# qianyizh/ElasticReconstruction

Measured on AMD Instinct MI355X. Metric: depth frames/sec into 512^3 TSDF (640x480), higher is better.
Workload: dtype f32; 1 GPU; configs[1]; frames_per_gpu=91800, volume_units_touched=122, warp=True, inputs=hbm_resident, parallelism=single GPU

## Files before the change

### elasticreconstruction_amd/_ffi.py

```python
import ctypes as C
import os

_HERE = os.path.dirname(os.path.abspath(__file__))
LIB_PATH = os.environ.get("ER_HIP_LIB") or os.path.join(_HERE, "liber_hip.so")

SYMBOLS = [
    "er_last_error", "er_device_count", "er_abi_version", "er_request_hw_queues", "er_host_alloc", "er_host_free", "er_host_copy_h2d", "er_device_alloc", "er_device_free", "er_device_copy_d2h",
    "er_tsdf_create", "er_tsdf_destroy", "er_tsdf_set_stream", "er_tsdf_synchronize",
    "er_tsdf_wait_event", "er_tsdf_reset", "er_tsdf_status", "er_tsdf_set_unit_shard", "er_unit_owner",
    "er_tsdf_scale_depth", "er_tsdf_reproject", "er_tsdf_integrate", "er_tsdf_integrate_frames", "er_tsdf_prepass_trace",
    "er_tsdf_unit_count", "er_tsdf_unit_keys", "er_tsdf_read_unit", "er_tsdf_sum_weight",
    "er_tsdf_extract_world", "er_tsdf_extract_surface", "er_tsdf_extract_oriented", "er_tsdf_extract_mesh", "er_mc_table", "er_tsdf_extract_mesh_indexed", "er_tsdf_import_world", "er_raycast_params_default", "er_tsdf_raycast", "er_tsdf_raycast_batch", "er_tsdf_export_weighted", "er_tsdf_import_weighted",
    "er_tsdf_export_raw", "er_tsdf_import_raw",
    "er_tsdf_color_enable", "er_tsdf_read_unit_color", "er_tsdf_write_unit_color", "er_tsdf_color_frames", "er_tsdf_reproject_color", "er_tsdf_sample_colors",
    "er_tsdf_band_sizes", "er_tsdf_export_band", "er_tsdf_merge_band", "er_tsdf_import_band", "er_tsdf_drop_units",
    "er_tsdf_set_profiling", "er_tsdf_get_profile",
    "er_comm_unique_id", "er_comm_create", "er_comm_create_local", "er_comm_create_loopback", "er_comm_destroy", "er_comm_rank", "er_comm_world",
    "er_tsdf_allreduce", "er_comm_merge_stats", "er_comm_merge_stats_owner", "er_frame_block",
    "er_cloud_create", "er_cloud_create_batch", "er_cloud_create_from_tsdf", "er_cloud_destroy", "er_cloud_size",
    "er_icp_count_inliers", "er_icp_align", "er_icp_align_trace", "er_find_correspondence",
    "er_icp_count_inliers_batch", "er_icp_align_batch", "er_find_correspondence_batch", "er_icp_release_workspaces", "er_registration_batch", "er_ransac_fitness_batch", "er_ransac_inliers",
    "er_features_create", "er_features_destroy", "er_features_size", "er_feature_knn", "er_ransac_hypotheses", "er_ransac_params_default", "er_ransac_align", "er_ransac_align_batch",
    "er_odom_params_default", "er_odom_create", "er_odom_destroy", "er_odom_align_pairs", "er_odom_track", "er_frame_to_model_align", "er_frames_to_models_align", "er_odom_linearize", "er_odom_read_maps", "er_odom_tables",
    "er_cloud_read", "er_cloud_voxel_grid", "er_cloud_estimate_normals", "er_fpfh_estimate", "er_features_dim", "er_features_read",
    "er_frag_params_default", "er_frag_create", "er_frag_destroy", "er_frag_lane_bytes", "er_frag_build", "er_frag_count", "er_frag_read",
    "er_pgo_create", "er_pgo_destroy", "er_pgo_optimize", "er_pgo_set_state", "er_pgo_get_state", "er_pgo_linearize", "er_pgo_trial", "er_pgo_set_profiling", "er_pgo_get_profile",
    "er_fopt_create", "er_fopt_destroy", "er_fopt_set_cloud", "er_fopt_cloud_size", "er_fopt_get_points", "er_fopt_update_pose",
    "er_fopt_update_point_pn", "er_fopt_set_correspondences", "er_fopt_set_correspondences_dev", "er_fopt_group_count", "er_fopt_group_info", "er_fopt_update_normals", "er_fopt_assemble_rigid", "er_fopt_assemble_slac",
    "er_fopt_assemble_nonrigid", "er_fopt_factor_slac", "er_fopt_factor_nonrigid", "er_fopt_solve", "er_fopt_debug_shift_diagonal",
]


class ErWarp(C.Structure):
    _fields_ = [
        ("ctr", C.POINTER(C.c_float)),
        ("num_grids", C.c_int),
        ("resolution", C.c_int),
        ("length", C.c_float),
        ("grid_index", C.POINTER(C.c_int)),
        ("seg", C.POINTER(C.c_double)),
        ("madj", C.POINTER(C.c_double)),
    ]


class ErRansacParams(C.Structure):
    _fields_ = [("max_iterations", C.c_int), ("nr_samples", C.c_int), ("k_correspondences", C.c_int), ("similarity", C.c_float),
                ("max_corr_dist", C.c_float), ("inlier_fraction", C.c_float), ("inlier_number", C.c_int), ("angle_diff", C.c_float),
                ("seed", C.c_uint), ("chunk_iterations", C.c_int)]


class ErRansacStats(C.Structure):
    _fields_ = [("iterations", C.c_longlong), ("polygon_rejections", C.c_longlong), ("normal_rejections", C.c_longlong), ("scored", C.c_longlong)]


class ErOdomParams(C.Structure):
    _fields_ = [("levels", C.c_int), ("iterations", C.c_int * 4), ("bilateral", C.c_int), ("max_depth_mm", C.c_int), ("min_valid", C.c_int),
                ("dist_thresh", C.c_float), ("angle_thresh", C.c_float)]


class ErRaycastParams(C.Structure):
    _fields_ = [("t_min", C.c_float), ("t_max", C.c_float), ("step", C.c_float)]


class ErFragParams(C.Structure):
    _fields_ = [("interval", C.c_int), ("lanes", C.c_int), ("max_units", C.c_int), ("length", C.c_float), ("raycast", ErRaycastParams)]


class ErError(RuntimeError):
    pass


_lib = None


def lib():
    global _lib
    if _lib is not None:
        return _lib
    if not os.path.exists(LIB_PATH):
        raise ErError(
            "liber_hip.so not found at %s -- build it with `python -c 'import __graft_entry__ as g; g.build()'` "
            "or `make -C elasticreconstruction_amd/csrc`; there is no CPU fallback." % LIB_PATH)
    L = C.CDLL(LIB_PATH, mode=C.RTLD_GLOBAL)
    vp, ip, dp, fp = C.c_void_p, C.POINTER(C.c_int), C.POINTER(C.c_double), C.POINTER(C.c_float)
    u16p = C.POINTER(C.c_uint16)
    L.er_last_error.restype = C.c_char_p
    L.er_last_error.argtypes = []
    L.er_device_count.argtypes = []
    L.er_abi_version.argtypes = []
    L.er_host_alloc.restype = vp
    L.er_host_alloc.argtypes = [C.c_size_t]
    L.er_host_free.argtypes = [vp]
    L.er_host_copy_h2d.argtypes = [vp, vp, C.c_size_t]
    L.er_device_alloc.restype = vp
    L.er_device_alloc.argtypes = [C.c_size_t, C.c_int]
    L.er_device_free.argtypes = [vp]
    L.er_device_copy_d2h.argtypes = [vp, vp, C.c_size_t]
    L.er_tsdf_create.argtypes = [C.c_int, C.c_int, fp, C.c_int, C.c_int, C.POINTER(vp)]
    L.er_tsdf_destroy.argtypes = [vp]
    L.er_tsdf_set_stream.argtypes = [vp, vp]
    L.er_tsdf_synchronize.argtypes = [vp]
    L.er_tsdf_wait_event.argtypes = [vp, vp]
    L.er_tsdf_reset.argtypes = [vp]
    L.er_tsdf_status.argtypes = [vp, ip, C.POINTER(C.c_long)]
    L.er_tsdf_set_unit_shard.argtypes = [vp, C.c_int, C.c_int]
    L.er_unit_owner.argtypes = [C.c_int, C.c_int]
    L.er_tsdf_scale_depth.argtypes = [vp, vp, vp]
    L.er_tsdf_reproject.argtypes = [vp, vp, vp, C.c_int, C.c_float, vp, vp]
    L.er_tsdf_integrate.argtypes = [vp, vp, vp]
    L.er_tsdf_integrate_frames.argtypes = [vp, C.c_int, vp, C.c_int, vp, C.POINTER(ErWarp)]
    if hasattr(L, "er_tsdf_prepass_trace"):
        L.er_tsdf_prepass_trace.argtypes = [vp, C.c_int, vp, C.c_int, vp, C.POINTER(ErWarp), vp, ip, vp, vp, vp, vp, vp, C.c_int, ip]
    L.er_tsdf_unit_count.argtypes = [vp, ip]
    L.er_tsdf_unit_keys.argtypes = [vp, vp]
    L.er_tsdf_read_unit.argtypes = [vp, C.c_int, vp, vp]
    L.er_tsdf_sum_weight.argtypes = [vp, dp]
    L.er_tsdf_extract_world.argtypes = [vp, vp, C.c_long, C.POINTER(C.c_long)]
    L.er_tsdf_extract_surface.argtypes = [vp, vp, C.c_long, C.POINTER(C.c_long)]
    if hasattr(L, "er_tsdf_extract_oriented"):
        L.er_tsdf_extract_oriented.argtypes = [vp, vp, vp, C.c_long, C.POINTER(C.c_long)]
    L.er_tsdf_extract_mesh.argtypes = [vp, vp, C.c_long, C.POINTER(C.c_long)]
    L.er_mc_table.argtypes = [vp]
    if hasattr(L, "er_tsdf_extract_mesh_indexed"):
        L.er_tsdf_extract_mesh_indexed.argtypes = [vp, vp, vp, C.c_long, vp, C.c_long, C.POINTER(C.c_long), C.POINTER(C.c_long)]
        L.er_tsdf_import_world.argtypes = [vp, vp, C.c_long, ip]
    if hasattr(L, "er_tsdf_raycast"):
        L.er_raycast_params_default.argtypes = [C.POINTER(ErRaycastParams)]
        L.er_tsdf_raycast.argtypes = [vp, C.c_int, C.c_int, vp, vp, C.POINTER(ErRaycastParams), vp, vp, C.c_int]
    if hasattr(L, "er_tsdf_raycast_batch"):
        L.er_tsdf_raycast_batch.argtypes = [C.c_int, vp, vp, vp, vp, vp, vp, vp, vp]
    if hasattr(L, "er_frag_create"):
        L.er_frag_params_default.argtypes = [C.POINTER(ErFragParams)]
        L.er_frag_create.argtypes = [C.c_int, C.c_int, vp, C.POINTER(ErOdomParams), C.POINTER(ErFragParams), C.c_int, C.POINTER(vp)]
        L.er_frag_destroy.argtypes = [vp]
        L.er_frag_lane_bytes.argtypes = [vp, C.POINTER(C.c_size_t)]
        L.er_frag_build.argtypes = [vp, C.c_int, vp, C.c_int, vp, C.c_int, vp, vp]
        L.er_frag_count.argtypes = [vp, ip]
        L.er_frag_read.argtypes = [vp, C.c_int, vp, vp, C.c_long, C.POINTER(C.c_long)]
    if hasattr(L, "er_tsdf_color_enable"):
        L.er_tsdf_color_enable.argtypes = [vp]
        L.er_tsdf_read_unit_color.argtypes = [vp, C.c_int, vp]
        L.er_tsdf_write_unit_color.argtypes = [vp, C.c_int, vp]
        L.er_tsdf_color_frames.argtypes = [vp, C.c_int, vp, vp, C.c_int, vp, C.POINTER(ErWarp), vp]
        L.er_tsdf_sample_colors.argtypes = [vp, vp, C.c_long, vp, vp]
        L.er_tsdf_reproject_color.argtypes = [vp, vp, vp, vp, C.c_int, C.c_float, vp, vp]
    L.er_request_hw_queues.argtypes = [C.c_int]
    L.er_tsdf_export_weighted.argtypes = [vp, vp, C.c_int, vp]
    L.er_tsdf_import_weighted.argtypes = [vp, vp, C.c_int, vp]
    L.er_tsdf_export_raw.argtypes = [vp, vp, C.c_int, vp]
    L.er_tsdf_import_raw.argtypes = [vp, vp, C.c_int, vp]
    L.er_comm_unique_id.argtypes = [vp]
    L.er_comm_create.argtypes = [vp, C.c_int, C.c_int, C.c_int, C.POINTER(vp)]
    L.er_comm_create_local.argtypes = [C.c_int, vp, vp]
    L.er_comm_create_loopback.argtypes = [C.c_int, C.c_int, vp]
    L.er_comm_destroy.argtypes = [vp]
    L.er_comm_rank.argtypes = [vp]
    L.er_comm_world.argtypes = [vp]
    L.er_tsdf_allreduce.argtypes = [vp, vp, C.c_int, ip]
    L.er_comm_merge_stats.argtypes = [vp, vp]
    L.er_comm_merge_stats_owner.argtypes = [vp, vp]
    L.er_tsdf_band_sizes.argtypes = [vp, vp, C.c_int, vp]
    L.er_tsdf_export_band.argtypes = [vp, vp, vp, C.c_int, vp]
    L.er_tsdf_merge_band.argtypes = [vp, vp, C.c_int, vp, vp, vp]
    L.er_tsdf_import_band.argtypes = [vp, vp, C.c_int, vp]
    L.er_tsdf_drop_units.argtypes = [vp, vp, C.c_int]
    L.er_frame_block.restype = None
    L.er_frame_block.argtypes = [C.c_int, C.c_int, C.c_int, ip, ip]
    L.er_tsdf_set_profiling.argtypes = [vp, C.c_int]
    L.er_tsdf_get_profile.argtypes = [vp, dp, C.POINTER(C.c_long), C.POINTER(C.c_long), C.POINTER(C.c_long)]
    if hasattr(L, "er_cloud_create"):
        L.er_cloud_create.argtypes = [vp, vp, C.c_int, C.c_float, C.c_int, C.POINTER(vp)]
        L.er_cloud_create_batch.argtypes = [C.c_int, vp, vp, vp, C.c_float, C.c_int, vp]
        if hasattr(L, "er_cloud_create_from_tsdf"):
            L.er_cloud_create_from_tsdf.argtypes = [vp, C.c_float, C.c_float, C.POINTER(vp), ip]
        L.er_cloud_destroy.argtypes = [vp]
        L.er_cloud_size.argtypes = [vp]
        L.er_icp_count_inliers.argtypes = [vp, vp, vp, C.c_double, ip]
        L.er_icp_align.argtypes = [vp, vp, vp, C.c_double, C.c_int, C.c_double, C.c_int, vp, ip, ip, dp]
        if hasattr(L, "er_icp_align_trace"):
            L.er_icp_align_trace.argtypes = [vp, vp, vp, C.c_double, C.c_int, C.c_double, C.c_int, C.c_int, C.c_int, vp, vp, vp, vp, vp, vp, ip, vp, ip, ip]
        L.er_find_correspondence.argtypes = [vp, vp, vp, C.c_double, C.c_double, vp, C.c_int, ip, vp]
        L.er_icp_count_inliers_batch.argtypes = [C.c_int, vp, vp, vp, C.c_double, vp]
        L.er_icp_align_batch.argtypes = [C.c_int, vp, vp, vp, C.c_double, C.c_int, C.c_double, C.c_int, vp, vp, vp, vp]
        L.er_find_correspondence_batch.argtypes = [C.c_int, vp, vp, vp, C.c_double, C.c_double, vp, vp, vp, vp]
        L.er_icp_release_workspaces.argtypes = []
        L.er_registration_batch.argtypes = [C.c_int, vp, vp, vp, C.c_double, C.c_int, C.c_double, C.c_int, C.c_double, C.c_int, C.c_double, C.c_double,
                                            vp, vp, vp, vp, vp, vp, vp, vp, vp]
        L.er_ransac_fitness_batch.argtypes = [vp, vp, C.c_int, vp, C.c_float, vp, vp]
        L.er_ransac_inliers.argtypes = [vp, vp, vp, C.c_float, vp, C.c_int, ip, vp, vp, vp]
        if hasattr(L, "er_ransac_align"):
            L.er_features_create.argtypes = [vp, C.c_int, C.c_int, C.c_int, C.POINTER(vp)]
            L.er_features_destroy.argtypes = [vp]
            L.er_features_size.argtypes = [vp]
            L.er_feature_knn.argtypes = [vp, vp, C.c_int, vp, vp]
            L.er_ransac_hypotheses.argtypes = [vp, vp, C.c_int, C.c_int, vp, vp, C.c_float, C.c_float, vp, vp]
            L.er_ransac_params_default.argtypes = [C.POINTER(ErRansacParams)]
            L.er_ransac_align.argtypes = [vp, vp, vp, vp, C.POINTER(ErRansacParams), vp, ip, ip, dp, C.POINTER(ErRansacStats), vp, C.c_int, ip]
        if hasattr(L, "er_ransac_align_batch"):
            L.er_ransac_align_batch.argtypes = [C.c_int, vp, vp, vp, vp, C.POINTER(ErRansacParams), vp, C.c_int, vp, vp, vp, vp, vp, vp, vp]
        if hasattr(L, "er_fpfh_estimate"):
            L.er_cloud_read.argtypes = [vp, vp, vp]
            L.er_cloud_voxel_grid.argtypes = [vp, C.c_float, C.c_float, C.POINTER(vp), ip]
            L.er_cloud_estimate_normals.argtypes = [vp, C.c_float, C.POINTER(vp), vp]
            L.er_fpfh_estimate.argtypes = [vp, C.c_float, C.POINTER(vp), vp, vp]
            L.er_features_dim.argtypes = [vp]
            L.er_features_read.argtypes = [vp, vp]
    if hasattr(L, "er_odom_create"):
        L.er_odom_params_default.argtypes = [C.POINTER(ErOdomParams)]
        L.er_odom_create.argtypes = [C.c_int, C.c_int, fp, C.POINTER(ErOdomParams), C.c_int, C.POINTER(vp)]
        L.er_odom_destroy.argtypes = [vp]
        L.er_odom_align_pairs.argtypes = [vp, C.c_int, vp, C.c_int, C.c_int, vp, vp, vp, vp, vp, vp, vp, C.c_int]
        L.er_odom_track.argtypes = [vp, C.c_int, vp, C.c_int, vp, vp, C.c_int]
        if hasattr(L, "er_frame_to_model_align"):
            L.er_frame_to_model_align.argtypes = [vp, vp, C.c_int, vp, C.c_int, vp, vp, vp, vp, vp, C.c_int]
        if hasattr(L, "er_frames_to_models_align"):
            L.er_frames_to_models_align.argtypes = [vp, C.c_int, vp, C.c_int, vp, C.c_int, vp, vp, vp, vp, vp, vp, C.c_int]
        L.er_odom_linearize.argtypes = [vp, vp, C.c_int, C.c_int, vp, vp, ip]
        L.er_odom_read_maps.argtypes = [vp, vp, C.c_int, C.c_int, vp, vp, vp]
        L.er_odom_tables.argtypes = [vp, vp, ip]
    if hasattr(L, "er_pgo_create"):
        L.er_pgo_create.argtypes = [C.c_int, C.c_int, vp, vp, vp, vp, vp, C.c_int, C.POINTER(vp)]
        L.er_pgo_destroy.argtypes = [vp]
        L.er_pgo_optimize.argtypes = [vp, C.c_int, C.c_double, C.c_int, vp, vp, ip, ip, vp]
        L.er_pgo_set_state.argtypes = [vp, vp, vp]
        L.er_pgo_get_state.argtypes = [vp, vp, vp]
        L.er_pgo_linearize.argtypes = [vp, C.c_double, C.c_double, vp, vp, vp]
        L.er_pgo_trial.argtypes = [vp, C.c_double, C.c_double, vp, vp, dp, ip]
        L.er_pgo_set_profiling.argtypes = [vp, C.c_int]
        L.er_pgo_get_profile.argtypes = [vp, vp]
    if hasattr(L, "er_fopt_create"):
        L.er_fopt_create.argtypes = [C.c_int, C.c_int, C.c_float, C.c_int, C.POINTER(vp)]
        L.er_fopt_destroy.argtypes = [vp]
        L.er_fopt_set_cloud.argtypes = [vp, C.c_int, vp, vp, C.c_int, ip]
        L.er_fopt_cloud_size.argtypes = [vp, C.c_int]
        L.er_fopt_get_points.argtypes = [vp, C.c_int, vp, vp, vp, vp, vp]
        L.er_fopt_update_pose.argtypes = [vp, C.c_int, vp]
        L.er_fopt_update_point_pn.argtypes = [vp, C.c_int, vp]
        L.er_fopt_set_correspondences.argtypes = [vp, C.c_int, vp, vp, vp, vp]
        L.er_fopt_set_correspondences_dev.argtypes = [vp, C.c_int, vp, vp, vp, vp]
        L.er_fopt_group_count.argtypes = [vp]
        L.er_fopt_assemble_rigid.argtypes = [vp, vp, vp, vp]
        L.er_fopt_assemble_slac.argtypes = [vp, vp, vp, vp, vp]
        L.er_fopt_group_info.argtypes = [vp, vp]
        L.er_fopt_update_normals.argtypes = [vp, C.c_int, vp]
        L.er_fopt_assemble_nonrigid.argtypes = [vp, C.c_double, vp, vp]
        L.er_fopt_factor_slac.argtypes = [vp, vp, C.c_double, vp, vp]
        L.er_fopt_factor_nonrigid.argtypes = [vp, C.c_double]
        L.er_fopt_solve.argtypes = [vp, vp, C.c_int, vp]
        L.er_fopt_debug_shift_diagonal.argtypes = [vp, C.c_long, C.c_double]
    _lib = L
    return L


def check(rc, what):
    if rc != 0:
        msg = lib().er_last_error()
        raise ErError("%s failed: %s" % (what, msg.decode("utf-8", "replace") if msg else "unknown error"))


class PinnedArena:

    def __init__(self):
        self._lib, self._p, self._cap, self._off, self._old = lib(), None, 0, 0, []

    def reset(self, need_bytes):
        self._off = 0
        for p in self._old:
            self._lib.er_host_free(p)
        self._old = []
        if need_bytes > self._cap:
            if self._p:
                self._lib.er_host_free(self._p)
            self._cap = int(need_bytes * 1.25) + 4096
            self._p = self._lib.er_host_alloc(self._cap)
            if not self._p:
                self._cap = 0
                raise ErError("er_host_alloc: " + self._lib.er_last_error().decode())

    def take(self, shape, dtype):
        import numpy as np
        dt = np.dtype(dtype)
        n = int(np.prod(shape)) * dt.itemsize
        off = (self._off + 4095) & ~4095
        assert off + n <= self._cap, "PinnedArena.reset() was sized too small"
        self._off = off + n
        buf = (C.c_char * max(n, 1)).from_address(self._p + off)
        return np.frombuffer(buf, dtype=dt, count=int(np.prod(shape))).reshape(shape)

    def close(self):
        if self._p:
            self._lib.er_host_free(self._p)
            self._p, self._cap = None, 0

    def __del__(self):
        try:
            self.close()
        except Exception:
            pass


def ptr(a):
    return a.ctypes.data_as(C.c_void_p)
```

### elasticreconstruction_amd/csrc/er_tsdf.h

```cpp
#pragma once

#include "er_common.h"
#include "er_tsdf_math.h"

#include "../../include/er_hip.h"

#include <algorithm>
#include <cstdlib>
#include <utility>
#include <vector>

namespace er_tsdf_k {
using namespace er;

constexpr int kBlock = 256;
constexpr int kEmptyKey = -1;
constexpr uint32_t kZEmpty = 0xFFFFFFFFu;

enum { C_NUNITS = 0, C_NBATCH = 1 , C_POOL_OVERFLOW = 2, C_TABLE_FULL = 3, C_OUT_OF_RANGE = 4,
       C_NBATCH1 = 6, C_NBATCH2 = 7, C_ZERO_WRITE = 8 ,
       C_ZERO_WRITE1 = 10, C_COUNT = 12 };
constexpr int kDepth = 3;
constexpr int kAux = 2;

struct ReprojArgs {
  const uint16_t* depth;
  int n_frames, cols, rows;
  Camera cam;
  CameraInv cami;
  const double* seg12;
  const double* madj12;
  const int* grid_index;
  const float* ctr;
  int res;
  float grid_ul;
  int floats_per_grid;
  uint32_t* zbuf;
  uint32_t* lastzero;
  uint32_t* zfix;
  int* zero_flag;
};
__global__ void k_reproject_scatter(ReprojArgs A);

constexpr int kFixThreads = 64;
constexpr int kFixBlocks = 256;

constexpr int kScaledPad = 64;
constexpr int kTile = 32;
constexpr int kLoShift = 4;
constexpr int kLoSub = kTile >> kLoShift;
constexpr int kTileKeys = 96;

constexpr int kPrepThreads = 256;
constexpr int kPrepPix = kTile * kTile / kPrepThreads;

template <bool kWide>
__global__ __launch_bounds__(kPrepThreads) void k_prepare(
    const uint16_t* __restrict__ depth, uint32_t* __restrict__ zbuf, int n_frames, int cols, int rows,
    Camera cam, CameraInv cami, const float* __restrict__ lambda, const double* __restrict__ T12, float* __restrict__ scaled,
    int* __restrict__ ht_key, int* __restrict__ ht_slot, unsigned long long* __restrict__ ht_mask, int cap_mask,
    int hash_shift, int* __restrict__ batch, int* __restrict__ nbatch,
    int* __restrict__ counters, float* __restrict__ tile_max, float* __restrict__ tile_lo, float* __restrict__ tile_lo_fine, int2 shard,
    uint32_t* __restrict__ lastzero, uint32_t* __restrict__ zfix, const int* __restrict__ zero_flag);
extern template __global__ void k_prepare<true>(const uint16_t* __restrict__, uint32_t* __restrict__, int, int, int, Camera, CameraInv, const float* __restrict__, const double* __restrict__, float* __restrict__, int* __restrict__, int* __restrict__, unsigned long long* __restrict__, int, int, int* __restrict__, int* __restrict__, int* __restrict__, float* __restrict__, float* __restrict__, float* __restrict__, int2, uint32_t* __restrict__, uint32_t* __restrict__, const int* __restrict__);
extern template __global__ void k_prepare<false>(const uint16_t* __restrict__, uint32_t* __restrict__, int, int, int, Camera, CameraInv, const float* __restrict__, const double* __restrict__, float* __restrict__, int* __restrict__, int* __restrict__, unsigned long long* __restrict__, int, int, int* __restrict__, int* __restrict__, int* __restrict__, float* __restrict__, float* __restrict__, float* __restrict__, int2, uint32_t* __restrict__, uint32_t* __restrict__, const int* __restrict__);

constexpr int kRows = 4;
constexpr int kItemsPerUnit = 256;

struct Plan {
  int n_units;
  int next;
};

struct PlanRec {
  int key;
  int slot;
  unsigned long long mask;
};

constexpr int kIntMinBlocks = 5;

template <bool kSure>
__global__ __launch_bounds__(kBlock, kIntMinBlocks) void k_integrate(
    float2* __restrict__ pool, const PlanRec* __restrict__ plan_rec, Plan* __restrict__ plan,
    const FrameXform* __restrict__ frames, const float* __restrict__ scaled, const float* __restrict__ tile_max,
    const float* __restrict__ tile_lo, const float* __restrict__ tile_lo_fine, int tiles_x, int tiles_y, Camera cam, int cols, int rows);
extern template __global__ void k_integrate<true>(float2* __restrict__, const PlanRec* __restrict__, Plan* __restrict__, const FrameXform* __restrict__, const float* __restrict__, const float* __restrict__, const float* __restrict__, const float* __restrict__, int, int, Camera, int, int);
extern template __global__ void k_integrate<false>(float2* __restrict__, const PlanRec* __restrict__, Plan* __restrict__, const FrameXform* __restrict__, const float* __restrict__, const float* __restrict__, const float* __restrict__, const float* __restrict__, int, int, Camera, int, int);
}

struct er_tsdf_s {
  int device = 0, cols = 0, rows = 0, pixels = 0, max_units = 0;
  er::Camera cam{};
  er::CameraInv cami{};
  hipStream_t own_stream = nullptr, stream = nullptr;
  hipEvent_t caller_ev = nullptr;
  hipEvent_t voxel_done = nullptr;
  bool voxel_ahead = false;
  hipStream_t aux_stream[er_tsdf_k::kAux] = {};
  hipStream_t copy_stream = nullptr;
  hipEvent_t copy_done[er_tsdf_k::kDepth] = {};
  hipEvent_t consts_done[er_tsdf_k::kDepth] = {};
  int n_cu = 256;
  int shard_rank = 0, shard_world = 1;
  float2* pool = nullptr;
  int *ht_key = nullptr, *ht_slot = nullptr, *unit_key = nullptr, *counters = nullptr;
  unsigned long long* stats = nullptr;
  long batch_no = 0;
  bool used[er_tsdf_k::kDepth] = {};
  int* batch[er_tsdf_k::kDepth] = {};
  unsigned long long* ht_mask[er_tsdf_k::kDepth] = {};
  float *scaled[er_tsdf_k::kDepth] = {}, *tile_max[er_tsdf_k::kDepth] = {}, *tile_lo[er_tsdf_k::kDepth] = {}, *tile_lo_fine[er_tsdf_k::kDepth] = {};
  er::FrameXform* frames[er_tsdf_k::kDepth] = {};
  void* dstage[er_tsdf_k::kDepth] = {};
  hipEvent_t pre_done[er_tsdf_k::kDepth] = {}, int_done[er_tsdf_k::kDepth] = {};
  void* pinned[er_tsdf_k::kDepth] = {};
  int ht_cap = 0, ht_shift = 0;
  float *lambda = nullptr, *ctr = nullptr;
  float* ctr_pinned[2] = {nullptr, nullptr};
  float* ctr_dev[2] = {nullptr, nullptr};
  size_t ctr_pinned_cap[2] = {0, 0}, ctr_dev_cap[2] = {0, 0};
  hipEvent_t ctr_ev[2] = {nullptr, nullptr};
  hipEvent_t ctr_rd[2][er_tsdf_k::kAux] = {};
  bool ctr_rd_set[2] = {false, false};
  int ctr_parity = 0, ctr_cur = 0;
  uint16_t* depth_stage[er_tsdf_k::kDepth] = {};
  uint32_t *zbuf[er_tsdf_k::kAux] = {}, *lastzero[er_tsdf_k::kAux] = {}, *zfix[er_tsdf_k::kAux] = {};
  double *T12 = nullptr, *seg12 = nullptr, *madj12 = nullptr, *dsum = nullptr;
  int *grid_index = nullptr, *key_scratch = nullptr, *slot_scratch = nullptr;
  er_tsdf_k::PlanRec* plan_rec[er_tsdf_k::kDepth] = {};
  er_tsdf_k::Plan* plan[er_tsdf_k::kDepth] = {};
  bool reset_pending[er_tsdf_k::kDepth] = {};
  size_t key_scratch_cap = 0;
  int prof_stride = 0;
  long prof_tick = 0;
  std::vector<std::pair<hipEvent_t, hipEvent_t>> events;
  double ms_total = 0.0;
  long launches = 0, frames_done = 0;
  std::vector<int> dropped;
  void* band_scratch = nullptr;
  size_t band_scratch_cap = 0;
  unsigned long long* color = nullptr;
  void* color_scratch = nullptr;
  size_t color_scratch_cap = 0;
};

namespace er_tsdf_k {
__attribute__((visibility("hidden"))) int check_flags(er_tsdf_t h);
__attribute__((visibility("hidden"))) int resolve_slots(er_tsdf_t h, const int* keys_host, int n, bool allocate);
__attribute__((visibility("hidden"))) int sorted_units(er_tsdf_t h, std::vector<int>& keys, std::vector<int>& slots);
__attribute__((visibility("hidden"))) int reproject_single(er_tsdf_t h, const ReprojArgs& RA, uint16_t* z_dev, hipStream_t X);
__attribute__((visibility("hidden"))) int color_zero_slots(er_tsdf_t h, int n);
}
```

### elasticreconstruction_amd/csrc/er_tsdf.hip

```cpp
#include "er_tsdf_dev.h"

namespace {

using namespace er_tsdf_k;

constexpr int kNbatchSlot[3] = {C_NBATCH, C_NBATCH1, C_NBATCH2};
constexpr int kZeroFlagSlot[2] = {C_ZERO_WRITE, C_ZERO_WRITE1};

__global__ void k_lambda(float* __restrict__ lambda, int cols, int rows, Camera cam) {
  int p = blockIdx.x * blockDim.x + threadIdx.x;
  if (p >= cols * rows) return;
  lambda[p] = scale_lambda(p % cols, p / cols, cam);
}

__global__ void k_scale_depth(const uint16_t* __restrict__ depth, const float* __restrict__ lambda,
                              float* __restrict__ scaled, int pixels, float itrunc) {
  int p = blockIdx.x * blockDim.x + threadIdx.x;
  if (p >= pixels) return;
  scaled[p] = scale_depth_px(depth[p], lambda[p], itrunc);
}

__global__ __launch_bounds__(kFixThreads) __attribute__((amdgpu_num_vgpr(48))) void k_reproject_fix(ReprojArgs A) {
  const int fl0 = A.zero_flag[0], fl1 = A.zero_flag[1];
  if ((fl0 | fl1) == 0) return;
  const int pixels = A.cols * A.rows;
  for (int f = 0; f < A.n_frames; f++) {
    if ((((f < 32 ? fl0 : fl1) >> (f & 31)) & 1) == 0) continue;
    for (int p = blockIdx.x * kFixThreads + threadIdx.x; p < pixels; p += gridDim.x * kFixThreads) reproject_scatter_px(A, f, p % A.cols, p / A.cols, 1);
  }
}

__global__ void k_zbuf_to_depth(uint32_t* __restrict__ zbuf, uint16_t* __restrict__ depth, long total, uint32_t* __restrict__ lastzero,
                                uint32_t* __restrict__ zfix, const int* __restrict__ zero_flag) {
  long t = (long)blockIdx.x * blockDim.x + threadIdx.x;
  if (t >= total) return;
  uint32_t z = zbuf[t];
  zbuf[t] = kZEmpty;
  if (zero_flag[0] & 1) z = take_z(z, (size_t)t, lastzero, zfix);
  depth[t] = (z == kZEmpty) ? (uint16_t)0 : (uint16_t)z;
}


__device__ int unit_slot_acquire(int e, int key, int* __restrict__ ht_slot, int* __restrict__ unit_key, int max_units, int* __restrict__ counters) {
  int slot = __hip_atomic_load(&ht_slot[e], __ATOMIC_RELAXED, __HIP_MEMORY_SCOPE_AGENT);
  bool won = false;
  if (slot == -1) won = atomicCAS(&ht_slot[e], -1, -2) == -1;
  if (won) {
    const int s = atomicAdd(&counters[C_NUNITS], 1);
    if (s < max_units) {
      unit_key[s] = key;
      __threadfence();
      slot = s;
    } else {
      atomicOr(&counters[C_POOL_OVERFLOW], 1);
      slot = -3;
    }
    atomicExch(&ht_slot[e], slot);
  }
  if (!won && (slot == -1 || slot == -2)) {
    do {
      slot = __hip_atomic_load(&ht_slot[e], __ATOMIC_RELAXED, __HIP_MEMORY_SCOPE_AGENT);
      if (slot == -2) __builtin_amdgcn_s_sleep(8);
    } while (slot == -2);
  }
  return slot;
}

__global__ __launch_bounds__(256) void k_plan(const int* __restrict__ batch, const int* __restrict__ nbatch,
                                              const unsigned long long* __restrict__ ht_mask, const int* __restrict__ ht_key,
                                              int* __restrict__ ht_slot, int* __restrict__ unit_key, int max_units,
                                              int* __restrict__ counters, PlanRec* __restrict__ plan_rec, Plan* __restrict__ plan,
                                              int* __restrict__ zero_flag) {
  __shared__ int hist[65];
  __shared__ int start[66];
  const int n = *nbatch;
  for (int t = threadIdx.x; t < 65; t += blockDim.x) hist[t] = 0;
  __syncthreads();
  for (int t = threadIdx.x; t < n; t += blockDim.x) atomicAdd(&hist[__popcll(ht_mask[batch[t]])], 1);
  __syncthreads();
  if (threadIdx.x == 0) {
    int acc = 0;
    for (int c = 64; c >= 0; c--) {
      start[c] = acc;
      acc += hist[c];
    }
    plan->n_units = n;
    plan->next = 0;
    if (zero_flag) zero_flag[0] = zero_flag[1] = 0;
  }
  __syncthreads();
  for (int t = threadIdx.x; t < n; t += blockDim.x) {
    const int e = batch[t];
    const unsigned long long mask = ht_mask[e];
    const int key = ht_key[e];
    PlanRec r;
    r.key = key;
    r.slot = unit_slot_acquire(e, key, ht_slot, unit_key, max_units, counters);
    r.mask = mask;
    plan_rec[atomicAdd(&start[__popcll(mask)], 1)] = r;
  }
}

__global__ void k_reset(const int* __restrict__ batch, int* __restrict__ nbatch, unsigned long long* __restrict__ ht_mask,
                        unsigned long long* __restrict__ stats) {
  const int n = *nbatch;
  unsigned long long visits = 0;
  for (int t = threadIdx.x; t < n; t += blockDim.x) {
    const int e = batch[t];
    visits += (unsigned long long)__popcll(ht_mask[e]);
    ht_mask[e] = 0ull;
  }
  if (visits) atomicAdd(&stats[0], visits);
  __syncthreads();
  if (threadIdx.x == 0) *nbatch = 0;
}

__global__ void k_sum_weight(const float2* __restrict__ pool, long n_vox, double* __restrict__ out) {
  double s = 0.0;
  for (long t = (long)blockIdx.x * blockDim.x + threadIdx.x; t < n_vox; t += (long)gridDim.x * blockDim.x)
    s += (double)pool[t].y;
  for (int off = 32; off > 0; off >>= 1) s += __shfl_down(s, off);
  __shared__ double part[kBlock / 64];
  if ((threadIdx.x & 63) == 0) part[threadIdx.x >> 6] = s;
  __syncthreads();
  if (threadIdx.x == 0) {
    double b = 0.0;
    for (int w = 0; w < kBlock / 64; w++) b += part[w];
    atomicAdd(out, b);
  }
}

__global__ void k_ensure_units(const int* __restrict__ keys, int n, int* __restrict__ ht_key, int* __restrict__ ht_slot,
                               int cap_mask, int hash_shift, int* __restrict__ unit_key, int max_units,
                               int* __restrict__ counters, int* __restrict__ slots_out, int allocate) {
  const int t = blockIdx.x * blockDim.x + threadIdx.x;
  if (t >= n) return;
  const int key = keys[t];
  int slot = -1;
  if (allocate) {
    const int e = ht_find_or_insert(ht_key, cap_mask, hash_shift, key);
    if (e < 0) {
      atomicOr(&counters[C_TABLE_FULL], 1);
    } else {
      slot = ht_slot[e];
      if (slot < 0) {
        const int s = atomicAdd(&counters[C_NUNITS], 1);
        if (s < max_units) {
          ht_slot[e] = s;
          unit_key[s] = key;
          slot = s;
        } else {
          atomicOr(&counters[C_POOL_OVERFLOW], 1);
        }
      }
    }
  } else {
    unsigned h = hash_unit_key(key, hash_shift);
    for (int probe = 0; probe <= cap_mask; ++probe) {
      const int e = (int)((h + (unsigned)probe) & (unsigned)cap_mask);
      const int k = ht_key[e];
      if (k == key) { slot = ht_slot[e]; break; }
      if (k == kEmptyKey) break;
    }
  }
  slots_out[t] = slot;
}

}

hipStream_t er::tsdf_stream(er_tsdf_s* h) { return h->stream; }
int er::tsdf_device(er_tsdf_s* h) { return h->device; }

static int launch_reproject(er_tsdf_t h, const ReprojArgs& RA, int n, hipStream_t X);

namespace {

int drain_events(er_tsdf_t h) {
  for (auto& ev : h->events) {
    float ms = 0.f;
    ER_HIP_TRY(hipEventSynchronize(ev.second));
    ER_HIP_TRY(hipEventElapsedTime(&ms, ev.first, ev.second));
    h->ms_total += ms;
    h->launches += 1;
    (void)hipEventDestroy(ev.first);
    (void)hipEventDestroy(ev.second);
  }
  h->events.clear();
  return 0;
}

int join_voxel(er_tsdf_t h) {
  if (h->voxel_ahead) {
    ER_HIP_TRY(hipStreamWaitEvent(h->stream, h->voxel_done, 0));
    h->voxel_ahead = false;
  }
  return 0;
}

int ensure_key_scratch(er_tsdf_t h, size_t n) {
  if (n <= h->key_scratch_cap) return 0;
  if (h->key_scratch) (void)hipFree(h->key_scratch);
  if (h->slot_scratch) (void)hipFree(h->slot_scratch);
  h->key_scratch = h->slot_scratch = nullptr;
  size_t cap = std::max<size_t>(n, 1024);
  ER_HIP_TRY(hipMalloc(&h->key_scratch, cap * sizeof(int)));
  ER_HIP_TRY(hipMalloc(&h->slot_scratch, cap * sizeof(int)));
  h->key_scratch_cap = cap;
  return 0;
}

}

namespace er_tsdf_k {

int check_flags(er_tsdf_t h) {
  int c[C_COUNT];
  if (join_voxel(h)) return 1;
  ER_HIP_TRY(hipMemcpyAsync(c, h->counters, sizeof c, hipMemcpyDeviceToHost, h->stream));
  ER_HIP_TRY(hipStreamSynchronize(h->stream));
  if (c[C_POOL_OVERFLOW])
    return er::fail("TSDF unit pool exhausted: %d units requested, capacity %d (raise max_units)", c[C_NUNITS], h->max_units);
  if (c[C_TABLE_FULL]) return er::fail("TSDF unit hash table full (capacity %d)", h->ht_cap);
  return 0;
}

int resolve_slots(er_tsdf_t h, const int* keys_host, int n, bool allocate) {
  if (join_voxel(h) || ensure_key_scratch(h, (size_t)n)) return 1;
  ER_HIP_TRY(hipMemcpyAsync(h->key_scratch, keys_host, (size_t)n * sizeof(int), hipMemcpyHostToDevice, h->stream));
  hipLaunchKernelGGL(k_ensure_units, dim3((n + kBlock - 1) / kBlock), dim3(kBlock), 0, h->stream, h->key_scratch, n,
                     h->ht_key, h->ht_slot, h->ht_cap - 1, h->ht_shift, h->unit_key, h->max_units, h->counters,
                     h->slot_scratch, allocate ? 1 : 0);
  ER_HIP_TRY(hipGetLastError());
  return 0;
}

int sorted_units(er_tsdf_t h, std::vector<int>& keys, std::vector<int>& slots) {
  if (check_flags(h)) return 1;
  int n = 0;
  ER_HIP_TRY(hipMemcpy(&n, h->counters + C_NUNITS, sizeof(int), hipMemcpyDeviceToHost));
  n = std::min(n, h->max_units);
  std::vector<int> uk((size_t)n);
  if (n) ER_HIP_TRY(hipMemcpy(uk.data(), h->unit_key, (size_t)n * sizeof(int), hipMemcpyDeviceToHost));
  std::vector<std::pair<int, int>> ks;
  ks.reserve((size_t)n);
  for (int s = 0; s < n; s++)
    if (!std::binary_search(h->dropped.begin(), h->dropped.end(), uk[(size_t)s])) ks.push_back(std::make_pair(uk[(size_t)s], s));
  std::sort(ks.begin(), ks.end());
  n = (int)ks.size();
  keys.resize((size_t)n);
  slots.resize((size_t)n);
  for (int s = 0; s < n; s++) {
    keys[(size_t)s] = ks[(size_t)s].first;
    slots[(size_t)s] = ks[(size_t)s].second;
  }
  return 0;
}

}

namespace {

struct Staging {
  er::FrameXform fx[ER_MAX_BATCH];
  float fxT[16][ER_MAX_BATCH];
  double t12[ER_MAX_BATCH * 12];
  double seg[ER_MAX_BATCH * 16];
  double madj[ER_MAX_BATCH * 12];
  int gi[ER_MAX_BATCH];
};

int flush_resets(er_tsdf_t h) {
  if (join_voxel(h)) return 1;
  for (int q = 0; q < kDepth; q++)
    if (h->reset_pending[q]) {
      hipLaunchKernelGGL(k_reset, dim3(1), dim3(kBlock), 0, h->stream, h->batch[q], h->counters + kNbatchSlot[q], h->ht_mask[q], h->stats);
      ER_HIP_TRY(hipGetLastError());
      ER_HIP_TRY(hipEventRecord(h->int_done[q], h->stream));
      h->reset_pending[q] = false;
    }
  return 0;
}

int sync_all(er_tsdf_t h) {
  if (flush_resets(h)) return 1;
  if (h->copy_stream) ER_HIP_TRY(hipStreamSynchronize(h->copy_stream));
  for (int a = 0; a < kAux; a++) ER_HIP_TRY(hipStreamSynchronize(h->aux_stream[a]));
  if (h->stream != h->own_stream) ER_HIP_TRY(hipStreamSynchronize(h->own_stream));
  ER_HIP_TRY(hipStreamSynchronize(h->stream));
  h->voxel_ahead = false;
  return 0;
}

int run_batch(er_tsdf_t h, int n, const uint16_t* depth_dev, const double* T, const er_warp* warp, int frame0) {
  const int p = (int)(h->batch_no % kDepth), a = (int)(h->batch_no % kAux);
  h->batch_no++;
  if (h->used[p]) ER_HIP_TRY(hipEventSynchronize(h->consts_done[p]));
  Staging* st = static_cast<Staging*>(h->pinned[p]);
  for (int f = 0; f < n; f++) {
    const double* Tf = T + (size_t)f * 16;
    double Tinv[16];
    if (!er::mat4_inverse(Tf, Tinv)) return er::fail("frame %d: singular pose matrix", frame0 + f);
    for (int q = 0; q < 12; q++) {
      st->fx[f].mi[q] = (float)Tinv[q];
      st->t12[f * 12 + q] = Tf[q];
    }
    st->fx[f].tx = (float)Tf[3];
    st->fx[f].ty = (float)Tf[7];
    st->fx[f].tz = (float)Tf[11];
    st->fx[f].pad = 0.f;
    for (int q = 0; q < 16; q++) st->fxT[q][f] = reinterpret_cast<const float*>(&st->fx[f])[q];
  }
  static_assert(offsetof(Staging, fxT) == sizeof(er::FrameXform) * ER_MAX_BATCH && sizeof(er::FrameXform) == 64, "fxT lies directly behind fx");
  hipStream_t X = h->aux_stream[a], S = h->own_stream;
  int* nbatch = h->counters + kNbatchSlot[p];

  constexpr int kIntBlocksPerCu = 3;
  const int wide_grid = h->n_cu * kIntBlocksPerCu;
  uint32_t* zsrc = nullptr;
  char* dst = static_cast<char*>(h->dstage[p]);
  const double* dev_t12 = reinterpret_cast<const double*>(dst + offsetof(Staging, t12));
  const double* dev_seg = reinterpret_cast<const double*>(dst + offsetof(Staging, seg));
  const double* dev_madj = reinterpret_cast<const double*>(dst + offsetof(Staging, madj));
  const int* dev_gi = reinterpret_cast<const int*>(dst + offsetof(Staging, gi));
  if (warp) {
    for (int f = 0; f < n; f++) {
      for (int q = 0; q < 12; q++) {
        st->seg[f * 16 + q] = warp->seg[(size_t)(frame0 + f) * 16 + q];
        st->madj[f * 12 + q] = warp->madj[(size_t)(frame0 + f) * 16 + q];
      }
      er::cube_coord_deltas(&st->seg[f * 16], h->cam, h->cols, h->rows, &st->seg[f * 16 + 12]);
      st->seg[f * 16 + 15] = 0.0;
      const int g = warp->grid_index[frame0 + f];
      if (g < 0 || g >= warp->num_grids) return er::fail("frame %d: control grid index %d out of [0,%d)", frame0 + f, g, warp->num_grids);
      st->gi[f] = g;
    }
  }
  if (h->used[p]) ER_HIP_TRY(hipStreamWaitEvent(X, h->int_done[p], 0));
  if (h->reset_pending[p]) {
    hipLaunchKernelGGL(k_reset, dim3(1), dim3(kBlock), 0, X, h->batch[p], nbatch, h->ht_mask[p], h->stats);
    ER_HIP_TRY(hipGetLastError());
    h->reset_pending[p] = false;
  }
  ER_HIP_TRY(hipMemcpyAsync(h->dstage[p], st, sizeof(Staging), hipMemcpyHostToDevice, X));
  ER_HIP_TRY(hipEventRecord(h->consts_done[p], X));
  if (warp) {
    const int verts = (warp->resolution + 1) * (warp->resolution + 1) * (warp->resolution + 1);
    const float grid_ul = warp->length / (float)warp->resolution;
    const ReprojArgs RA{depth_dev, n, h->cols, h->rows, h->cam, h->cami, dev_seg, dev_madj, dev_gi, h->ctr, warp->resolution, grid_ul,
                        verts * 3, h->zbuf[a], h->lastzero[a], h->zfix[a], h->counters + kZeroFlagSlot[a]};
    if (launch_reproject(h, RA, n, X)) return 1;
    zsrc = h->zbuf[a];
  }

  const bool wide = h->cols % 4 == 0 && (zsrc || reinterpret_cast<uintptr_t>(depth_dev) % 8 == 0);
  hipLaunchKernelGGL(wide ? k_prepare<true> : k_prepare<false>, dim3((h->cols + kTile - 1) / kTile, (h->rows + kTile - 1) / kTile, n), dim3(kPrepThreads), 0, X,
                     depth_dev, zsrc, n, h->cols, h->rows, h->cam, h->cami, h->lambda, dev_t12, h->scaled[p], h->ht_key, h->ht_slot,
                     h->ht_mask[p], h->ht_cap - 1, h->ht_shift, h->batch[p], nbatch, h->counters,
                     h->tile_max[p], h->tile_lo[p], h->tile_lo_fine[p], make_int2(h->shard_rank, h->shard_world), h->lastzero[a], h->zfix[a],
                     h->counters + kZeroFlagSlot[a]);
  hipLaunchKernelGGL(k_plan, dim3(1), dim3(256), 0, X, h->batch[p], nbatch, h->ht_mask[p], h->ht_key, h->ht_slot, h->unit_key, h->max_units,
                     h->counters, h->plan_rec[p], h->plan[p], warp ? h->counters + kZeroFlagSlot[a] : (int*)nullptr);
  ER_HIP_TRY(hipGetLastError());
  ER_HIP_TRY(hipEventRecord(h->pre_done[p], X));

  ER_HIP_TRY(hipStreamWaitEvent(S, h->pre_done[p], 0));
  hipEvent_t e0 = nullptr, e1 = nullptr;
  const bool timed = h->prof_stride > 0 && (h->prof_tick++ % h->prof_stride) == 0;
  if (timed) {
    ER_HIP_TRY(hipEventCreate(&e0));
    ER_HIP_TRY(hipEventCreate(&e1));
    ER_HIP_TRY(hipEventRecord(e0, S));
  }
  const bool sure = h->cam.integration_trunc < 64.0f;
  hipLaunchKernelGGL(sure ? k_integrate<true> : k_integrate<false>, dim3(wide_grid), dim3(kBlock), 0, S, h->pool, h->plan_rec[p], h->plan[p],
                     h->frames[p], h->scaled[p], h->tile_max[p], h->tile_lo[p], h->tile_lo_fine[p], (h->cols + kTile - 1) / kTile, (h->rows + kTile - 1) / kTile,
                     h->cam, h->cols, h->rows);
  if (timed) {
    ER_HIP_TRY(hipEventRecord(e1, S));
    h->events.emplace_back(e0, e1);
  }
  ER_HIP_TRY(hipGetLastError());
  ER_HIP_TRY(hipEventRecord(h->int_done[p], S));
  h->reset_pending[p] = true;
  h->used[p] = true;
  h->frames_done += n;
  return 0;
}

}

static hipError_t aux_create(hipStream_t* s) {
  return hipStreamCreateWithFlags(s, hipStreamNonBlocking);
}

extern "C" {

int er_tsdf_create(int cols, int rows, const float cam6[6], int max_units, int device, er_tsdf_t* out) {
  if (!out) return er::fail("er_tsdf_create: out is NULL");
  *out = nullptr;
  if (cols <= 0 || rows <= 0 || max_units <= 0) return er::fail("er_tsdf_create: bad dimensions");
  if ((long)cols * rows >= (1L << 30)) return er::fail("er_tsdf_create: image of %d x %d pixels is too large", cols, rows);
  int ndev = 0;
  if (hipGetDeviceCount(&ndev) != hipSuccess || ndev <= 0)
    return er::fail("er_tsdf_create: no HIP device available (liber_hip has no CPU fallback)");
  if (device < 0 || device >= ndev) return er::fail("er_tsdf_create: device %d out of range [0,%d)", device, ndev);
  ER_HIP_TRY(hipSetDevice(device));
  er_tsdf_t h = new er_tsdf_s();
  h->device = device;
  h->cols = cols;
  h->rows = rows;
  h->pixels = cols * rows;
  h->max_units = max_units;
  if (cam6) {
    h->cam = er::Camera{cam6[0], cam6[1], cam6[2], cam6[3], cam6[4], cam6[5]};
  } else {
    h->cam = er::Camera{525.0f, 525.0f, 319.5f, 239.5f, 2.5f, 2.5f};
  }
  h->cami.inv_fx = 1.0 / (double)h->cam.fx;
  h->cami.inv_fy = 1.0 / (double)h->cam.fy;
  h->cami.pp_small = (std::fabs((double)h->cam.cx) < 1e6 && std::fabs((double)h->cam.cy) < 1e6) ? 1 : 0;
  h->cami.pad = 0;
  hipDeviceProp_t prop;
  if (hipGetDeviceProperties(&prop, device) == hipSuccess && prop.multiProcessorCount > 0) h->n_cu = prop.multiProcessorCount;
  int cap = 1024, lg = 10;
  while (cap < 4 * max_units) { cap <<= 1; lg++; }
  h->ht_cap = cap;
  h->ht_shift = 32 - lg;
  const size_t px = (size_t)h->pixels, B = ER_MAX_BATCH;
#define ER_ALLOC(ptr, bytes)                                                                         \
  do {                                                                                               \
    hipError_t e_ = hipMalloc((void**)&(ptr), (bytes));                                              \
    if (e_ != hipSuccess) {                                                                          \
      er::fail("er_tsdf_create: hipMalloc(%zu bytes) for " #ptr " failed: %s", (size_t)(bytes), hipGetErrorString(e_)); \
      er_tsdf_destroy(h);                                                                            \
      return 1;                                                                                      \
    }                                                                                                \
  } while (0)
  if (hipStreamCreateWithFlags(&h->own_stream, hipStreamNonBlocking) != hipSuccess ||
      aux_create(&h->aux_stream[0]) != hipSuccess || (kAux > 1 && aux_create(&h->aux_stream[kAux - 1]) != hipSuccess) ||
      false) {
    delete h;
    return er::fail("er_tsdf_create: hipStreamCreate failed");
  }
  h->stream = h->own_stream;
  if (hipEventCreateWithFlags(&h->caller_ev, hipEventDisableTiming) != hipSuccess ||
      hipEventCreateWithFlags(&h->voxel_done, hipEventDisableTiming) != hipSuccess) {
    er_tsdf_destroy(h);
    return er::fail("er_tsdf_create: event allocation failed");
  }
  for (int q = 0; q < kDepth; q++) {
    if (hipEventCreateWithFlags(&h->pre_done[q], hipEventDisableTiming) != hipSuccess ||
        hipEventCreateWithFlags(&h->int_done[q], hipEventDisableTiming) != hipSuccess ||
        hipEventCreateWithFlags(&h->copy_done[q], hipEventDisableTiming) != hipSuccess ||
        hipEventCreateWithFlags(&h->consts_done[q], hipEventDisableTiming) != hipSuccess ||
        hipHostMalloc(&h->pinned[q], sizeof(Staging), hipHostMallocDefault) != hipSuccess) {
      er_tsdf_destroy(h);
      return er::fail("er_tsdf_create: event / pinned staging allocation failed");
    }
  }
  ER_ALLOC(h->pool, (size_t)max_units * er::kUnitVox * sizeof(float2));
  ER_ALLOC(h->ht_key, (size_t)cap * sizeof(int));
  ER_ALLOC(h->ht_slot, (size_t)cap * sizeof(int));
  for (int q = 0; q < kDepth; q++) ER_ALLOC(h->ht_mask[q], (size_t)cap * sizeof(unsigned long long));
  ER_ALLOC(h->unit_key, (size_t)max_units * sizeof(int));
  ER_ALLOC(h->counters, C_COUNT * sizeof(int));
  ER_ALLOC(h->stats, 4 * sizeof(unsigned long long));
  for (int q = 0; q < kDepth; q++) ER_ALLOC(h->batch[q], (size_t)cap * sizeof(int));
  ER_ALLOC(h->lambda, px * sizeof(float));
  for (int q = 0; q < kDepth; q++) ER_ALLOC(h->scaled[q], B * (px + kScaledPad) * sizeof(float));
  for (int q = 0; q < kDepth; q++) ER_ALLOC(h->depth_stage[q], B * px * sizeof(uint16_t));
  for (int q = 0; q < kAux; q++) ER_ALLOC(h->zbuf[q], B * px * sizeof(uint32_t));
  for (int q = 0; q < kAux; q++) ER_ALLOC(h->lastzero[q], B * px * sizeof(uint32_t));
  for (int q = 0; q < kAux; q++) ER_ALLOC(h->zfix[q], B * px * sizeof(uint32_t));
  for (int q = 0; q < kDepth; q++) ER_ALLOC(h->dstage[q], sizeof(Staging));
  for (int q = 0; q < kDepth; q++) h->frames[q] = reinterpret_cast<er::FrameXform*>(reinterpret_cast<char*>(h->dstage[q]) + offsetof(Staging, fx));
  ER_ALLOC(h->T12, B * 12 * sizeof(double));
  ER_ALLOC(h->seg12, B * 16 * sizeof(double));
  ER_ALLOC(h->madj12, B * 12 * sizeof(double));
  ER_ALLOC(h->grid_index, B * sizeof(int));
  ER_ALLOC(h->dsum, sizeof(double));
  for (int q = 0; q < kDepth; q++) ER_ALLOC(h->tile_max[q], B * (size_t)((cols + kTile - 1) / kTile) * ((rows + kTile - 1) / kTile) * sizeof(float));
  for (int q = 0; q < kDepth; q++) ER_ALLOC(h->tile_lo[q], B * (size_t)((cols + kTile - 1) / kTile) * ((rows + kTile - 1) / kTile) * sizeof(float));
  for (int q = 0; q < kDepth; q++)
    ER_ALLOC(h->tile_lo_fine[q], B * (size_t)((cols + (1 << kLoShift) - 1) >> kLoShift) * ((rows + (1 << kLoShift) - 1) >> kLoShift) * sizeof(float));
  for (int q = 0; q < kDepth; q++) ER_ALLOC(h->plan_rec[q], (size_t)cap * sizeof(PlanRec));
  for (int q = 0; q < kDepth; q++) ER_ALLOC(h->plan[q], sizeof(Plan));
#undef ER_ALLOC
  hipStream_t s = h->stream;
  bool ok = hipMemsetAsync(h->pool, 0, (size_t)max_units * er::kUnitVox * sizeof(float2), s) == hipSuccess &&
            hipMemsetAsync(h->ht_key, 0xFF, (size_t)cap * sizeof(int), s) == hipSuccess &&
            hipMemsetAsync(h->ht_slot, 0xFF, (size_t)cap * sizeof(int), s) == hipSuccess &&
            hipMemsetAsync(h->counters, 0, C_COUNT * sizeof(int), s) == hipSuccess &&
            hipMemsetAsync(h->stats, 0, 4 * sizeof(unsigned long long), s) == hipSuccess;
  for (int q = 0; q < kDepth; q++)
    ok = ok && hipMemsetAsync(h->ht_mask[q], 0, (size_t)cap * sizeof(unsigned long long), s) == hipSuccess &&
         hipMemsetAsync(h->scaled[q], 0, B * (px + kScaledPad) * sizeof(float), s) == hipSuccess;
  for (int q = 0; q < kAux; q++)
    ok = ok && hipMemsetAsync(h->lastzero[q], 0, B * px * sizeof(uint32_t), s) == hipSuccess &&
         hipMemsetAsync(h->zbuf[q], 0xFF, B * px * sizeof(uint32_t), s) == hipSuccess &&
         hipMemsetAsync(h->zfix[q], 0xFF, B * px * sizeof(uint32_t), s) == hipSuccess;
  if (ok) {
    hipLaunchKernelGGL(k_lambda, dim3((h->pixels + kBlock - 1) / kBlock), dim3(kBlock), 0, s, h->lambda, cols, rows, h->cam);
    ok = hipGetLastError() == hipSuccess && hipStreamSynchronize(s) == hipSuccess;
  }
  if (!ok) {
    er_tsdf_destroy(h);
    return er::fail("er_tsdf_create: device initialisation failed: %s", hipGetErrorString(hipGetLastError()));
  }
  *out = h;
  return 0;
}

int er_tsdf_destroy(er_tsdf_t h) {
  if (!h) return 0;
  (void)hipSetDevice(h->device);
  if (h->stream) (void)hipStreamSynchronize(h->stream);
  if (h->own_stream && h->own_stream != h->stream) (void)hipStreamSynchronize(h->own_stream);
  if (h->caller_ev) (void)hipEventDestroy(h->caller_ev);
  if (h->voxel_done) (void)hipEventDestroy(h->voxel_done);
  for (auto& ev : h->events) {
    (void)hipEventDestroy(ev.first);
    (void)hipEventDestroy(ev.second);
  }
  for (int a = 0; a < kAux; a++)
    if (h->aux_stream[a]) (void)hipStreamSynchronize(h->aux_stream[a]);
  std::vector<void*> ptrs = {h->pool, h->ht_key, h->ht_slot, h->unit_key, h->counters, h->stats, h->lambda, h->T12, h->seg12, h->madj12,
                             h->grid_index, h->dsum, h->ctr_dev[0], h->ctr_dev[1], h->key_scratch,
                             h->slot_scratch, h->band_scratch, h->color, h->color_scratch};
  for (int q = 0; q < kDepth; q++)
    for (void* x : {(void*)h->ht_mask[q], (void*)h->batch[q], (void*)h->scaled[q], (void*)h->depth_stage[q], h->dstage[q], (void*)h->tile_max[q], (void*)h->tile_lo[q], (void*)h->tile_lo_fine[q],
                    (void*)h->plan_rec[q], (void*)h->plan[q]})
      ptrs.push_back(x);
  for (int q = 0; q < kAux; q++) {
    ptrs.push_back(h->zbuf[q]);
    ptrs.push_back(h->lastzero[q]);
    ptrs.push_back(h->zfix[q]);
  }
  for (int q = 0; q < kDepth; q++) {
    if (h->pre_done[q]) (void)hipEventDestroy(h->pre_done[q]);
    if (h->int_done[q]) (void)hipEventDestroy(h->int_done[q]);
    if (h->copy_done[q]) (void)hipEventDestroy(h->copy_done[q]);
    if (h->consts_done[q]) (void)hipEventDestroy(h->consts_done[q]);
    if (h->pinned[q]) (void)hipHostFree(h->pinned[q]);
  }
  for (int a = 0; a < kAux; a++)
    if (h->aux_stream[a]) (void)hipStreamDestroy(h->aux_stream[a]);
  if (h->copy_stream) {
    (void)hipStreamSynchronize(h->copy_stream);
    (void)hipStreamDestroy(h->copy_stream);
  }
  for (int q = 0; q < 2; q++) {
    if (h->ctr_ev[q]) (void)hipEventDestroy(h->ctr_ev[q]);
    for (int a = 0; a < kAux; a++)
      if (h->ctr_rd[q][a]) (void)hipEventDestroy(h->ctr_rd[q][a]);
    if (h->ctr_pinned[q]) (void)hipHostFree(h->ctr_pinned[q]);
  }
  for (void* p : ptrs)
    if (p) (void)hipFree(p);
  if (h->own_stream) (void)hipStreamDestroy(h->own_stream);
  delete h;
  return 0;
}

int er_tsdf_set_stream(er_tsdf_t h, void* hip_stream) {
  if (!h) return er::fail("er_tsdf_set_stream: NULL handle");
  ER_HIP_TRY(hipSetDevice(h->device));
  if (sync_all(h)) return 1;
  h->stream = hip_stream ? (hipStream_t)hip_stream : h->own_stream;
  return 0;
}

int er_tsdf_synchronize(er_tsdf_t h) {
  if (!h) return er::fail("er_tsdf_synchronize: NULL handle");
  ER_HIP_TRY(hipSetDevice(h->device));
  return sync_all(h);
}

int er_tsdf_scale_depth(er_tsdf_t h, const uint16_t* depth_host, float* scaled_host) {
  if (!h || !depth_host || !scaled_host) return er::fail("er_tsdf_scale_depth: NULL argument");
  ER_HIP_TRY(hipSetDevice(h->device));
  if (sync_all(h)) return 1;
  const size_t px = (size_t)h->pixels;
  ER_HIP_TRY(hipMemcpyAsync(h->depth_stage[0], depth_host, px * sizeof(uint16_t), hipMemcpyHostToDevice, h->stream));
  hipLaunchKernelGGL(k_scale_depth, dim3((h->pixels + kBlock - 1) / kBlock), dim3(kBlock), 0, h->stream, h->depth_stage[0],
                     h->lambda, h->scaled[0], h->pixels, h->cam.integration_trunc);
  ER_HIP_TRY(hipGetLastError());
  ER_HIP_TRY(hipMemcpyAsync(scaled_host, h->scaled[0], px * sizeof(float), hipMemcpyDeviceToHost, h->stream));
  ER_HIP_TRY(hipStreamSynchronize(h->stream));
  return 0;
}

static int upload_ctr(er_tsdf_t h, const float* ctr, int res, int num_grids, hipStream_t also) {
  const size_t verts = (size_t)(res + 1) * (res + 1) * (res + 1);
  const size_t floats = verts * 3 * (size_t)num_grids;
  const int q = h->ctr_parity;
  h->ctr_parity ^= 1;
  if (floats > h->ctr_dev_cap[q]) {
    if (sync_all(h)) return 1;
    if (h->ctr_dev[q]) (void)hipFree(h->ctr_dev[q]);
    h->ctr_dev[q] = nullptr;
    h->ctr_dev_cap[q] = 0;
    ER_HIP_TRY(hipMalloc((void**)&h->ctr_dev[q], floats * sizeof(float)));
    h->ctr_dev_cap[q] = floats;
  }
  if (!h->ctr_ev[q]) {
    ER_HIP_TRY(hipEventCreateWithFlags(&h->ctr_ev[q], hipEventDisableTiming));
    for (int a = 0; a < kAux; a++) ER_HIP_TRY(hipEventCreateWithFlags(&h->ctr_rd[q][a], hipEventDisableTiming));
  } else {
    ER_HIP_TRY(hipEventSynchronize(h->ctr_ev[q]));
  }
  if (floats > h->ctr_pinned_cap[q]) {
    if (h->ctr_pinned[q]) (void)hipHostFree(h->ctr_pinned[q]);
    h->ctr_pinned[q] = nullptr;
    h->ctr_pinned_cap[q] = 0;
    ER_HIP_TRY(hipHostMalloc((void**)&h->ctr_pinned[q], floats * sizeof(float), hipHostMallocDefault));
    h->ctr_pinned_cap[q] = floats;
  }
  memcpy(h->ctr_pinned[q], ctr, floats * sizeof(float));
  const int a0 = (int)(h->batch_no % kAux);
  hipStream_t C = h->aux_stream[a0];
  if (h->ctr_rd_set[q])
    for (int a = 0; a < kAux; a++)
      if (a != a0) ER_HIP_TRY(hipStreamWaitEvent(C, h->ctr_rd[q][a], 0));
  ER_HIP_TRY(hipMemcpyAsync(h->ctr_dev[q], h->ctr_pinned[q], floats * sizeof(float), hipMemcpyHostToDevice, C));
  ER_HIP_TRY(hipEventRecord(h->ctr_ev[q], C));
  for (int a = 0; a < kAux; a++)
    if (a != a0) ER_HIP_TRY(hipStreamWaitEvent(h->aux_stream[a], h->ctr_ev[q], 0));
  if (also) ER_HIP_TRY(hipStreamWaitEvent(also, h->ctr_ev[q], 0));
  h->ctr = h->ctr_dev[q];
  h->ctr_cur = q;
  return 0;
}

static int launch_reproject(er_tsdf_t h, const ReprojArgs& RA, int n, hipStream_t X) {
  hipLaunchKernelGGL(k_reproject_scatter, dim3((h->cols + 63) / 64, (h->rows + 3) / 4, n), dim3(kBlock), 0, X, RA);
  hipLaunchKernelGGL(k_reproject_fix, dim3(kFixBlocks), dim3(kFixThreads), 0, X, RA);
  ER_HIP_TRY(hipGetLastError());
  return 0;
}

int er_tsdf_reproject(er_tsdf_t h, uint16_t* depth_inout_host, const float* ctr_host, int resolution, float length,
                      const double seg[16], const double madj[16]) {
  if (!h || !depth_inout_host || !ctr_host || !seg || !madj) return er::fail("er_tsdf_reproject: NULL argument");
  if (resolution <= 0) return er::fail("er_tsdf_reproject: bad resolution");
  ER_HIP_TRY(hipSetDevice(h->device));
  const size_t px = (size_t)h->pixels;
  const int verts = (resolution + 1) * (resolution + 1) * (resolution + 1);
  if (sync_all(h)) return 1;
  if (upload_ctr(h, ctr_host, resolution, 1, h->stream)) return 1;
  const int gi = 0;
  ER_HIP_TRY(hipMemcpyAsync(h->depth_stage[0], depth_inout_host, px * sizeof(uint16_t), hipMemcpyHostToDevice, h->stream));
  double seg16[16] = {0};
  memcpy(seg16, seg, 12 * sizeof(double));
  er::cube_coord_deltas(seg16, h->cam, h->cols, h->rows, seg16 + 12);
  ER_HIP_TRY(hipMemcpyAsync(h->seg12, seg16, 16 * sizeof(double), hipMemcpyHostToDevice, h->stream));
  ER_HIP_TRY(hipMemcpyAsync(h->madj12, madj, 12 * sizeof(double), hipMemcpyHostToDevice, h->stream));
  ER_HIP_TRY(hipMemcpyAsync(h->grid_index, &gi, sizeof(int), hipMemcpyHostToDevice, h->stream));
  const float grid_ul = length / (float)resolution;
  const long total = (long)px;
  const ReprojArgs RA{h->depth_stage[0], 1, h->cols, h->rows, h->cam, h->cami, h->seg12, h->madj12, h->grid_index, h->ctr, resolution, grid_ul,
                      verts * 3, h->zbuf[0], h->lastzero[0], h->zfix[0], h->counters + kZeroFlagSlot[0]};
  if (launch_reproject(h, RA, 1, h->stream)) return 1;
  hipLaunchKernelGGL(k_zbuf_to_depth, dim3((int)((total + kBlock - 1) / kBlock)), dim3(kBlock), 0, h->stream, h->zbuf[0],
                     h->depth_stage[0], total, h->lastzero[0], h->zfix[0], h->counters + kZeroFlagSlot[0]);
  ER_HIP_TRY(hipGetLastError());
  ER_HIP_TRY(hipMemsetAsync(h->counters + kZeroFlagSlot[0], 0, 2 * sizeof(int), h->stream));
  ER_HIP_TRY(hipMemcpyAsync(depth_inout_host, h->depth_stage[0], px * sizeof(uint16_t), hipMemcpyDeviceToHost, h->stream));
  ER_HIP_TRY(hipStreamSynchronize(h->stream));
  return 0;
}

int er_tsdf_integrate_frames(er_tsdf_t h, int n, const uint16_t* depth, int depth_on_device, const double* T,
                             const er_warp* warp) {
  if (!h || !depth || !T) return er::fail("er_tsdf_integrate_frames: NULL argument");
  if (n < 0) return er::fail("er_tsdf_integrate_frames: negative frame count");
  ER_HIP_TRY(hipSetDevice(h->device));
  if (n > 0) h->dropped.clear();
  if (warp) {
    if (!warp->ctr || !warp->grid_index || !warp->seg || !warp->madj || warp->num_grids <= 0 || warp->resolution <= 0)
      return er::fail("er_tsdf_integrate_frames: incomplete er_warp");
    if (upload_ctr(h, warp->ctr, warp->resolution, warp->num_grids, nullptr)) return 1;
  }
  const size_t px = (size_t)h->pixels;
  const int launches = (n + ER_MAX_BATCH - 1) / ER_MAX_BATCH;
  const int per = launches > 0 ? (n + launches - 1) / launches : 0;
  const bool joined = h->stream != h->own_stream && n > 0;
  if (joined) {
    ER_HIP_TRY(hipEventRecord(h->caller_ev, h->stream));
    ER_HIP_TRY(hipStreamWaitEvent(h->own_stream, h->caller_ev, 0));
  }
  for (int start = 0; start < n; start += per) {
    const int nb = std::min(per, n - start);
    const uint16_t* ddev;
    if (depth_on_device) {
      ddev = depth + (size_t)start * px;
    } else {
      const int p = (int)(h->batch_no % kDepth);
      if (!h->copy_stream) ER_HIP_TRY(hipStreamCreateWithFlags(&h->copy_stream, hipStreamNonBlocking));
      if (h->used[p]) ER_HIP_TRY(hipStreamWaitEvent(h->copy_stream, h->pre_done[p], 0));
      ER_HIP_TRY(hipMemcpyAsync(h->depth_stage[p], depth + (size_t)start * px, (size_t)nb * px * sizeof(uint16_t),
                                hipMemcpyHostToDevice, h->copy_stream));
      ER_HIP_TRY(hipEventRecord(h->copy_done[p], h->copy_stream));
      ER_HIP_TRY(hipStreamWaitEvent(h->aux_stream[h->batch_no % kAux], h->copy_done[p], 0));
      ddev = h->depth_stage[p];
    }
    if (run_batch(h, nb, ddev, T + (size_t)start * 16, warp, start)) return 1;
  }
  if (joined) {
    ER_HIP_TRY(hipEventRecord(h->voxel_done, h->own_stream));
    h->voxel_ahead = true;
  }
  if (warp) {
    for (int a = 0; a < kAux; a++) ER_HIP_TRY(hipEventRecord(h->ctr_rd[h->ctr_cur][a], h->aux_stream[a]));
    h->ctr_rd_set[h->ctr_cur] = true;
  }
  if (!depth_on_device && n > 0) ER_HIP_TRY(hipStreamSynchronize(h->copy_stream));
  return 0;
}

int er_tsdf_integrate(er_tsdf_t h, const uint16_t* depth_host, const double T[16]) {
  return er_tsdf_integrate_frames(h, 1, depth_host, 0, T, nullptr);
}

int er_tsdf_prepass_trace(er_tsdf_t h, int n, const uint16_t* depth, int depth_on_device, const double* T, const er_warp* warp,
                          float* scaled, int* scaled_pad, float* tile_max, float* tile_lo, float* tile_lo_fine,
                          int* keys, unsigned long long* masks, int keys_cap, int* n_keys) {
  if (!h) return er::fail("er_tsdf_prepass_trace: NULL handle");
  if (n < 1 || n > ER_MAX_BATCH) return er::fail("er_tsdf_prepass_trace: %d frames outside 1..%d (one batch)", n, ER_MAX_BATCH);
  ER_HIP_TRY(hipSetDevice(h->device));
  if (sync_all(h)) return 1;
  const int p = (int)(h->batch_no % kDepth);
  if (er_tsdf_integrate_frames(h, n, depth, depth_on_device, T, warp)) return 1;
  if (sync_all(h)) return 1;
  const size_t B = ER_MAX_BATCH, px = (size_t)h->pixels;
  const size_t tiles = (size_t)((h->cols + kTile - 1) / kTile) * ((h->rows + kTile - 1) / kTile);
  const size_t fine = (size_t)((h->cols + (1 << kLoShift) - 1) >> kLoShift) * ((h->rows + (1 << kLoShift) - 1) >> kLoShift);
  if (scaled_pad) *scaled_pad = kScaledPad;
  if (scaled) ER_HIP_TRY(hipMemcpy(scaled, h->scaled[p], (size_t)n * (px + kScaledPad) * sizeof(float), hipMemcpyDeviceToHost));
  if (tile_max) ER_HIP_TRY(hipMemcpy(tile_max, h->tile_max[p], tiles * B * sizeof(float), hipMemcpyDeviceToHost));
  if (tile_lo) ER_HIP_TRY(hipMemcpy(tile_lo, h->tile_lo[p], tiles * B * sizeof(float), hipMemcpyDeviceToHost));
  if (tile_lo_fine) ER_HIP_TRY(hipMemcpy(tile_lo_fine, h->tile_lo_fine[p], fine * B * sizeof(float), hipMemcpyDeviceToHost));
  Plan plan{};
  ER_HIP_TRY(hipMemcpy(&plan, h->plan[p], sizeof plan, hipMemcpyDeviceToHost));
  if (plan.n_units < 0 || plan.n_units > h->ht_cap) return er::fail("er_tsdf_prepass_trace: the batch lists %d units", plan.n_units);
  if (n_keys) *n_keys = plan.n_units;
  if (keys || masks) {
    std::vector<PlanRec> rec((size_t)plan.n_units);
    if (plan.n_units > 0) ER_HIP_TRY(hipMemcpy(rec.data(), h->plan_rec[p], rec.size() * sizeof(PlanRec), hipMemcpyDeviceToHost));
    std::sort(rec.begin(), rec.end(), [](const PlanRec& a, const PlanRec& b) { return a.key < b.key; });
    for (int i = 0; i < plan.n_units && i < keys_cap; i++) {
      if (keys) keys[i] = rec[(size_t)i].key;
      if (masks) masks[i] = rec[(size_t)i].mask;
    }
  }
  return 0;
}

int er_tsdf_wait_event(er_tsdf_t h, void* hip_event) {
  if (!h || !hip_event) return er::fail("er_tsdf_wait_event: NULL argument");
  ER_HIP_TRY(hipSetDevice(h->device));
  for (int a = 0; a < kAux; a++) ER_HIP_TRY(hipStreamWaitEvent(h->aux_stream[a], (hipEvent_t)hip_event, 0));
  if (h->copy_stream) ER_HIP_TRY(hipStreamWaitEvent(h->copy_stream, (hipEvent_t)hip_event, 0));
  return 0;
}

int er_tsdf_reset(er_tsdf_t h) {
  if (!h) return er::fail("er_tsdf_reset: NULL handle");
  ER_HIP_TRY(hipSetDevice(h->device));
  if (sync_all(h)) return 1;
  int n = 0;
  ER_HIP_TRY(hipMemcpy(&n, h->counters + C_NUNITS, sizeof(int), hipMemcpyDeviceToHost));
  n = std::min(std::max(n, 0), h->max_units);
  hipStream_t s = h->stream;
  if (n > 0) ER_HIP_TRY(hipMemsetAsync(h->pool, 0, (size_t)n * er::kUnitVox * sizeof(float2), s));
  if (n > 0 && h->color) ER_HIP_TRY(hipMemsetAsync(h->color, 0, (size_t)n * er::kUnitVox * 16, s));
  ER_HIP_TRY(hipMemsetAsync(h->ht_key, 0xFF, (size_t)h->ht_cap * sizeof(int), s));
  ER_HIP_TRY(hipMemsetAsync(h->ht_slot, 0xFF, (size_t)h->ht_cap * sizeof(int), s));
  for (int q = 0; q < kDepth; q++) ER_HIP_TRY(hipMemsetAsync(h->ht_mask[q], 0, (size_t)h->ht_cap * sizeof(unsigned long long), s));
  ER_HIP_TRY(hipMemsetAsync(h->counters, 0, C_COUNT * sizeof(int), s));
  ER_HIP_TRY(hipStreamSynchronize(s));
  for (int q = 0; q < kDepth; q++) h->used[q] = h->reset_pending[q] = false;
  h->batch_no = 0;
  h->dropped.clear();
  return 0;
}

int er_tsdf_set_unit_shard(er_tsdf_t h, int rank, int world) {
  if (!h) return er::fail("er_tsdf_set_unit_shard: NULL handle");
  if (world < 1 || rank < 0 || rank >= world) return er::fail("er_tsdf_set_unit_shard: rank %d not in [0,%d)", rank, world);
  ER_HIP_TRY(hipSetDevice(h->device));
  int n = 0;
  ER_HIP_TRY(hipMemcpy(&n, h->counters + C_NUNITS, sizeof(int), hipMemcpyDeviceToHost));
  if (n != 0) return er::fail("er_tsdf_set_unit_shard: the volume already holds %d units (set the shard before the first frame)", n);
  h->shard_rank = rank;
  h->shard_world = world;
  return 0;
}

int er_unit_owner(int key, int world) { return er::unit_owner(key, world); }

int er_tsdf_status(er_tsdf_t h, int* flags, long* out_of_range_pixels) {
  if (!h) return er::fail("er_tsdf_status: NULL handle");
  ER_HIP_TRY(hipSetDevice(h->device));
  int c[C_COUNT];
  ER_HIP_TRY(hipMemcpy(c, h->counters, sizeof c, hipMemcpyDeviceToHost));
  if (flags) *flags = (c[C_POOL_OVERFLOW] ? ER_STATUS_POOL_EXHAUSTED : 0) | (c[C_TABLE_FULL] ? ER_STATUS_TABLE_FULL : 0);
  if (out_of_range_pixels) *out_of_range_pixels = c[C_OUT_OF_RANGE];
  return 0;
}

int er_tsdf_unit_count(er_tsdf_t h, int* count) {
  if (!h || !count) return er::fail("er_tsdf_unit_count: NULL argument");
  ER_HIP_TRY(hipSetDevice(h->device));
  if (check_flags(h)) return 1;
  ER_HIP_TRY(hipMemcpy(count, h->counters + C_NUNITS, sizeof(int), hipMemcpyDeviceToHost));
  *count -= (int)h->dropped.size();
  return 0;
}

int er_tsdf_unit_keys(er_tsdf_t h, int* keys_host) {
  if (!h || !keys_host) return er::fail("er_tsdf_unit_keys: NULL argument");
  ER_HIP_TRY(hipSetDevice(h->device));
  std::vector<int> keys, slots;
  if (sorted_units(h, keys, slots)) return 1;
  std::copy(keys.begin(), keys.end(), keys_host);
  return 0;
}

int er_tsdf_read_unit(er_tsdf_t h, int key, float* sdf_host, float* weight_host) {
  if (!h) return er::fail("er_tsdf_read_unit: NULL handle");
  ER_HIP_TRY(hipSetDevice(h->device));
  if (check_flags(h)) return 1;
  if (std::binary_search(h->dropped.begin(), h->dropped.end(), key)) return er::fail("er_tsdf_read_unit: unit %d was handed to its owner by the last merge", key);
  if (resolve_slots(h, &key, 1, false)) return 1;
  int slot = -1;
  ER_HIP_TRY(hipMemcpyAsync(&slot, h->slot_scratch, sizeof(int), hipMemcpyDeviceToHost, h->stream));
  ER_HIP_TRY(hipStreamSynchronize(h->stream));
  if (slot < 0) return er::fail("er_tsdf_read_unit: no unit with key %d", key);
  std::vector<float2> tmp((size_t)er::kUnitVox);
  ER_HIP_TRY(hipMemcpyAsync(tmp.data(), h->pool + (size_t)slot * er::kUnitVox, tmp.size() * sizeof(float2),
                            hipMemcpyDeviceToHost, h->stream));
  ER_HIP_TRY(hipStreamSynchronize(h->stream));
  for (int l = 0; l < er::kUnitVox; l++) {
    if (sdf_host) sdf_host[l] = tmp[(size_t)l].x;
    if (weight_host) weight_host[l] = tmp[(size_t)l].y;
  }
  return 0;
}

int er_tsdf_sum_weight(er_tsdf_t h, double* sum) {
  if (!h || !sum) return er::fail("er_tsdf_sum_weight: NULL argument");
  ER_HIP_TRY(hipSetDevice(h->device));
  if (check_flags(h)) return 1;
  int n = 0;
  ER_HIP_TRY(hipMemcpy(&n, h->counters + C_NUNITS, sizeof(int), hipMemcpyDeviceToHost));
  ER_HIP_TRY(hipMemsetAsync(h->dsum, 0, sizeof(double), h->stream));
  if (n > 0) {
    hipLaunchKernelGGL(k_sum_weight, dim3(h->n_cu * 8), dim3(kBlock), 0, h->stream, h->pool, (long)n * er::kUnitVox, h->dsum);
    ER_HIP_TRY(hipGetLastError());
  }
  ER_HIP_TRY(hipMemcpyAsync(sum, h->dsum, sizeof(double), hipMemcpyDeviceToHost, h->stream));
  ER_HIP_TRY(hipStreamSynchronize(h->stream));
  return 0;
}

int er_tsdf_set_profiling(er_tsdf_t h, int enable) {
  if (!h) return er::fail("er_tsdf_set_profiling: NULL handle");
  ER_HIP_TRY(hipSetDevice(h->device));
  if (flush_resets(h) || drain_events(h)) return 1;
  h->prof_stride = enable > 0 ? enable : 0;
  h->prof_tick = 0;
  h->ms_total = 0.0;
  h->launches = 0;
  h->frames_done = 0;
  ER_HIP_TRY(hipMemsetAsync(h->stats, 0, 4 * sizeof(unsigned long long), h->stream));
  return 0;
}

int er_tsdf_get_profile(er_tsdf_t h, double* integrate_ms_total, long* integrate_launches, long* frames,
                        long* unit_visits) {
  if (!h) return er::fail("er_tsdf_get_profile: NULL handle");
  ER_HIP_TRY(hipSetDevice(h->device));
  if (flush_resets(h)) return 1;
  ER_HIP_TRY(hipStreamSynchronize(h->stream));
  if (drain_events(h)) return 1;
  unsigned long long st[4] = {0, 0, 0, 0};
  ER_HIP_TRY(hipMemcpy(st, h->stats, sizeof st, hipMemcpyDeviceToHost));
  if (integrate_ms_total) *integrate_ms_total = h->ms_total;
  if (integrate_launches) *integrate_launches = h->launches;
  if (frames) *frames = h->frames_done;
  if (unit_visits) *unit_visits = (long)st[0];
  return 0;
}


}

namespace er_tsdf_k {

int reproject_single(er_tsdf_t h, const ReprojArgs& RA, uint16_t* z_dev, hipStream_t X) {
  if (launch_reproject(h, RA, 1, X)) return 1;
  const long total = (long)RA.cols * RA.rows;
  hipLaunchKernelGGL(k_zbuf_to_depth, dim3((int)((total + kBlock - 1) / kBlock)), dim3(kBlock), 0, X, RA.zbuf, z_dev, total, RA.lastzero, RA.zfix,
                     RA.zero_flag);
  ER_HIP_TRY(hipGetLastError());
  ER_HIP_TRY(hipMemsetAsync(RA.zero_flag, 0, 2 * sizeof(int), X));
  return 0;
}

}
```

### elasticreconstruction_amd/csrc/er_tsdf_color.hip

```cpp
#include "er_tsdf_dev.h"

#include <cmath>

namespace {

using namespace er_tsdf_k;

constexpr int kColorBatch = 64;
constexpr double kLatticeLo = -(256.0 * 64.0), kLatticeHi = 256.0 * 64.0;

__global__ __launch_bounds__(kBlock) void k_color_splat(const uint16_t* __restrict__ depth, const uint8_t* __restrict__ rgb, int pixels, int cols,
                                                        Camera cam, const double* __restrict__ T16, const int* __restrict__ ht_key,
                                                        const int* __restrict__ ht_slot, int cap_mask, int shift, int max_units,
                                                        unsigned long long* __restrict__ color, unsigned long long* __restrict__ stats) {
  const int p = blockIdx.x * kBlock + threadIdx.x;
  const int f = blockIdx.y;
  int verdict = 0;
  if (p < pixels) {
    const size_t o = (size_t)f * (size_t)pixels + (size_t)p;
    const uint16_t d = depth[o];
    const int v = p / cols, u = p - v * cols;
    if (d != 0 && scale_depth_px(d, scale_lambda(u, v, cam), cam.integration_trunc) > 0.001f) {
      const double* T = T16 + (size_t)f * 16;
      double x, y, z;
      uvd2xyz(u, v, d, cam, x, y, z);
      const double p0 = ((T[0] * x + T[1] * y) + T[2] * z) + T[3];
      const double p1 = ((T[4] * x + T[5] * y) + T[6] * z) + T[7];
      const double p2 = ((T[8] * x + T[9] * y) + T[10] * z) + T[11];
      const double g0 = floor(p0 / kUnitLength + 0.5), g1 = floor(p1 / kUnitLength + 0.5), g2 = floor(p2 / kUnitLength + 0.5);
      if (!(g0 >= kLatticeLo && g0 < kLatticeHi && g1 >= kLatticeLo && g1 < kLatticeHi && g2 >= kLatticeLo && g2 < kLatticeHi)) {
        verdict = 3;
      } else {
        const int a0 = (int)g0 + 256 * 64, a1 = (int)g1 + 256 * 64, a2 = (int)g2 + 256 * 64;
        const int key = (a0 >> 6) << 18 | (a1 >> 6) << 9 | (a2 >> 6);
        const int slot = ht_lookup_slot(ht_key, ht_slot, cap_mask, shift, key);
        if ((unsigned)slot >= (unsigned)max_units) {
          verdict = 2;
        } else {
          const size_t l = (size_t)slot * kUnitVox + (size_t)((a0 & 63) * 4096 + (a1 & 63) * 64 + (a2 & 63));
          const uint8_t* c = rgb + o * 3;
          const unsigned long long rg = (unsigned long long)c[0] | (unsigned long long)c[1] << 32;
          const unsigned long long bn = (unsigned long long)c[2] | 1ull << 32;
          (void)__hip_atomic_fetch_add(&color[2 * l], rg, __ATOMIC_RELAXED, __HIP_MEMORY_SCOPE_AGENT);
          (void)__hip_atomic_fetch_add(&color[2 * l + 1], bn, __ATOMIC_RELAXED, __HIP_MEMORY_SCOPE_AGENT);
          verdict = 1;
        }
      }
    }
  }
  const unsigned long long b1 = __ballot(verdict == 1), b2 = __ballot(verdict == 2), b3 = __ballot(verdict == 3);
  if ((threadIdx.x & 63) == 0) {
    if (b1) atomicAdd(&stats[0], (unsigned long long)__popcll(b1));
    if (b2) atomicAdd(&stats[1], (unsigned long long)__popcll(b2));
    if (b3) atomicAdd(&stats[2], (unsigned long long)__popcll(b3));
  }
}

__device__ __forceinline__ void color_gather(const unsigned long long* __restrict__ color, const int* __restrict__ ht_key, const int* __restrict__ ht_slot,
                                             int cap_mask, int shift, int max_units, int gx, int gy, int gz, int* key, int* slot, unsigned long long s[4]) {
  if ((unsigned)gx >= 512u * 64u || (unsigned)gy >= 512u * 64u || (unsigned)gz >= 512u * 64u) return;
  const int k = (gx >> 6) << 18 | (gy >> 6) << 9 | (gz >> 6);
  if (k != *key) {
    *key = k;
    *slot = ht_lookup_slot(ht_key, ht_slot, cap_mask, shift, k);
  }
  if ((unsigned)*slot >= (unsigned)max_units) return;
  const size_t l = (size_t)*slot * kUnitVox + (size_t)((gx & 63) * 4096 + (gy & 63) * 64 + (gz & 63));
  const unsigned long long rg = color[2 * l], bn = color[2 * l + 1];
  s[0] += rg & 0xFFFFFFFFull;
  s[1] += rg >> 32;
  s[2] += bn & 0xFFFFFFFFull;
  s[3] += bn >> 32;
}

__global__ __launch_bounds__(kBlock) void k_color_sample(const unsigned long long* __restrict__ color, const int* __restrict__ ht_key,
                                                         const int* __restrict__ ht_slot, int cap_mask, int shift, int max_units,
                                                         const float4* __restrict__ pts, long n, uchar4* __restrict__ out,
                                                         unsigned long long* __restrict__ counts) {
  const long r = (long)blockIdx.x * kBlock + threadIdx.x;
  int level = -1;
  if (r < n) {
    const float4 p = pts[r];
    const double v0 = rint((double)p.x / kUnitLength), v1 = rint((double)p.y / kUnitLength), v2 = rint((double)p.z / kUnitLength);
    unsigned long long s[4] = {0, 0, 0, 0};
    if (v0 >= kLatticeLo && v0 < kLatticeHi && v1 >= kLatticeLo && v1 < kLatticeHi && v2 >= kLatticeLo && v2 < kLatticeHi) {
      const int gx = (int)v0 + 256 * 64, gy = (int)v1 + 256 * 64, gz = (int)v2 + 256 * 64;
      int key = -2, slot = -1;
      color_gather(color, ht_key, ht_slot, cap_mask, shift, max_units, gx, gy, gz, &key, &slot, s);
      if (s[3] > 0) {
        level = 0;
      } else {
        for (int dx = -1; dx <= 1; dx++)
          for (int dy = -1; dy <= 1; dy++)
            for (int dz = -1; dz <= 1; dz++) color_gather(color, ht_key, ht_slot, cap_mask, shift, max_units, gx + dx, gy + dy, gz + dz, &key, &slot, s);
        if (s[3] > 0) level = 1;
      }
    }
    uchar4 c = make_uchar4(0, 0, 0, 0);
    if (level >= 0) {
      const unsigned long long d = 2 * s[3];
      c = make_uchar4((unsigned char)((2 * s[0] + s[3]) / d), (unsigned char)((2 * s[1] + s[3]) / d), (unsigned char)((2 * s[2] + s[3]) / d), 255);
    }
    out[r] = c;
  }
  const unsigned long long b0 = __ballot(level == 0), b1 = __ballot(level == 1);
  if ((threadIdx.x & 63) == 0) {
    if (b0) atomicAdd(&counts[0], (unsigned long long)__popcll(b0));
    if (b1) atomicAdd(&counts[1], (unsigned long long)__popcll(b1));
  }
}

__global__ __launch_bounds__(kBlock) void k_color_warp(ReprojArgs A, const uint16_t* __restrict__ Z, uint32_t* __restrict__ win) {
  const int p = blockIdx.x * kBlock + threadIdx.x;
  if (p >= A.cols * A.rows) return;
  const uint16_t d = A.depth[p];
  if (d == 0) return;
  const int v = p / A.cols, u = p - v * A.cols;
  int cell;
  uint16_t dd;
  if (!reproject_px(u, v, d, A.cam, A.cami, A.cols, A.rows, A.seg12, A.madj12, A.ctr + (size_t)A.grid_index[0] * A.floats_per_grid, A.res, A.grid_ul,
                    cell, dd))
    return;
  if (dd != 0 && dd == Z[cell]) atomicMin(&win[cell], (uint32_t)p);
}

__global__ __launch_bounds__(kBlock) void k_color_gather(const uint8_t* __restrict__ rgb, uint32_t* __restrict__ win, uint8_t* __restrict__ out, int pixels) {
  const int c = blockIdx.x * kBlock + threadIdx.x;
  if (c >= pixels) return;
  const uint32_t w = win[c];
  win[c] = kZEmpty;
  const bool has = w < (uint32_t)pixels;
  const uint8_t* s = rgb + (size_t)(has ? w : 0u) * 3;
  out[(size_t)c * 3 + 0] = has ? s[0] : (uint8_t)0;
  out[(size_t)c * 3 + 1] = has ? s[1] : (uint8_t)0;
  out[(size_t)c * 3 + 2] = has ? s[2] : (uint8_t)0;
}

__global__ __launch_bounds__(256) void k_zero_unit_colors(unsigned long long* __restrict__ color, const int* __restrict__ slots, int max_units) {
  const int slot = slots[blockIdx.y];
  if ((unsigned)slot >= (unsigned)max_units) return;
  uint4* __restrict__ u = reinterpret_cast<uint4*>(color + (size_t)slot * kUnitVox * 2);
  u[blockIdx.x * 256 + threadIdx.x] = make_uint4(0u, 0u, 0u, 0u);
}

size_t round256(size_t x) { return (x + 255) & ~(size_t)255; }

int ensure_color_scratch(er_tsdf_t h, size_t bytes) {
  if (bytes <= h->color_scratch_cap) return 0;
  if (h->color_scratch) (void)hipFree(h->color_scratch);
  h->color_scratch = nullptr;
  h->color_scratch_cap = 0;
  if (hipMalloc(&h->color_scratch, bytes) != hipSuccess) {
    (void)hipGetLastError();
    return er::fail("colour staging: cannot allocate %zu bytes of device memory", bytes);
  }
  h->color_scratch_cap = bytes;
  return 0;
}

int color_ready(er_tsdf_t h, const char* who) {
  if (!h->color) return er::fail("%s: colour is not enabled on this volume (er_tsdf_color_enable)", who);
  if (h->shard_world > 1) return er::fail("%s: colour is not carried across GPUs (er_tsdf_set_unit_shard has world = %d)", who, h->shard_world);
  return 0;
}

int unit_slot(er_tsdf_t h, const char* who, int key, int* slot) {
  if (check_flags(h)) return 1;
  if (std::binary_search(h->dropped.begin(), h->dropped.end(), key)) return er::fail("%s: unit %d was handed to its owner by the last merge", who, key);
  if (resolve_slots(h, &key, 1, false)) return 1;
  *slot = -1;
  ER_HIP_TRY(hipMemcpyAsync(slot, h->slot_scratch, sizeof(int), hipMemcpyDeviceToHost, h->stream));
  ER_HIP_TRY(hipStreamSynchronize(h->stream));
  if (*slot < 0 || *slot >= h->max_units) return er::fail("%s: no unit with key %d", who, key);
  return 0;
}

int color_run(er_tsdf_t h, const char* who, int n, const uint16_t* depth, const uint8_t* rgb, int on_device, const double* T, const er_warp* warp,
              uint16_t* z_host, uint8_t* c_host, long stats[3]) {
  if (warp && (!warp->ctr || !warp->grid_index || !warp->seg || !warp->madj || warp->num_grids <= 0 || warp->resolution <= 0))
    return er::fail("%s: incomplete er_warp", who);
  if (check_flags(h)) return 1;
  if (stats) stats[0] = stats[1] = stats[2] = 0;
  if (n == 0) return 0;
  const size_t px = (size_t)h->pixels;
  const int nb_max = std::min(n, kColorBatch);
  const size_t verts = warp ? (size_t)(warp->resolution + 1) * (warp->resolution + 1) * (warp->resolution + 1) : 0;
  const size_t ctr_floats = warp ? verts * 3 * (size_t)warp->num_grids : 0;
  size_t off = 0;
  auto take = [&off](size_t bytes) { const size_t o = off; off += round256(bytes); return o; };
  const size_t o_stats = take(3 * sizeof(unsigned long long)), o_flag = take(2 * sizeof(int)), o_T = take((size_t)n * 16 * sizeof(double));
  const size_t o_d = take(on_device ? 0 : (size_t)nb_max * px * sizeof(uint16_t)), o_c = take(on_device ? 0 : (size_t)nb_max * px * 3);
  const size_t o_seg = take(warp ? (size_t)n * 16 * sizeof(double) : 0), o_madj = take(warp ? (size_t)n * 12 * sizeof(double) : 0);
  const size_t o_gi = take(warp ? (size_t)n * sizeof(int) : 0), o_ctr = take(ctr_floats * sizeof(float));
  const size_t o_zbuf = take(warp ? px * 4 : 0), o_lz = take(warp ? px * 4 : 0), o_zfix = take(warp ? px * 4 : 0), o_win = take(warp ? px * 4 : 0);
  const size_t o_Z = take(warp ? px * sizeof(uint16_t) : 0), o_C = take(warp ? px * 3 : 0);
  if (ensure_color_scratch(h, off)) return 1;
  char* S = static_cast<char*>(h->color_scratch);
  hipStream_t X = h->stream;
  unsigned long long* d_stats = reinterpret_cast<unsigned long long*>(S + o_stats);
  double* d_T = reinterpret_cast<double*>(S + o_T);
  ER_HIP_TRY(hipMemsetAsync(d_stats, 0, 3 * sizeof(unsigned long long), X));
  if (T) ER_HIP_TRY(hipMemcpyAsync(d_T, T, (size_t)n * 16 * sizeof(double), hipMemcpyHostToDevice, X));
  std::vector<double> seg16, madj12;
  if (warp) {
    seg16.assign((size_t)n * 16, 0.0);
    madj12.resize((size_t)n * 12);
    for (int f = 0; f < n; f++) {
      memcpy(&seg16[(size_t)f * 16], warp->seg + (size_t)f * 16, 12 * sizeof(double));
      memcpy(&madj12[(size_t)f * 12], warp->madj + (size_t)f * 16, 12 * sizeof(double));
      er::cube_coord_deltas(&seg16[(size_t)f * 16], h->cam, h->cols, h->rows, &seg16[(size_t)f * 16 + 12]);
      const int g = warp->grid_index[f];
      if (g < 0 || g >= warp->num_grids) return er::fail("%s: frame %d: control grid index %d out of [0,%d)", who, f, g, warp->num_grids);
    }
    ER_HIP_TRY(hipMemcpyAsync(S + o_seg, seg16.data(), seg16.size() * sizeof(double), hipMemcpyHostToDevice, X));
    ER_HIP_TRY(hipMemcpyAsync(S + o_madj, madj12.data(), madj12.size() * sizeof(double), hipMemcpyHostToDevice, X));
    ER_HIP_TRY(hipMemcpyAsync(S + o_gi, warp->grid_index, (size_t)n * sizeof(int), hipMemcpyHostToDevice, X));
    ER_HIP_TRY(hipMemcpyAsync(S + o_ctr, warp->ctr, ctr_floats * sizeof(float), hipMemcpyHostToDevice, X));
    ER_HIP_TRY(hipMemsetAsync(S + o_flag, 0, 2 * sizeof(int), X));
    ER_HIP_TRY(hipMemsetAsync(S + o_zbuf, 0xFF, px * 4, X));
    ER_HIP_TRY(hipMemsetAsync(S + o_lz, 0, px * 4, X));
    ER_HIP_TRY(hipMemsetAsync(S + o_zfix, 0xFF, px * 4, X));
    ER_HIP_TRY(hipMemsetAsync(S + o_win, 0xFF, px * 4, X));
  }
  const unsigned blocks = (unsigned)((px + kBlock - 1) / kBlock);
  for (int start = 0; start < n; start += kColorBatch) {
    const int nb = std::min(kColorBatch, n - start);
    const uint16_t* dd = depth + (size_t)start * px;
    const uint8_t* dc = rgb + (size_t)start * px * 3;
    if (!on_device) {
      ER_HIP_TRY(hipMemcpyAsync(S + o_d, dd, (size_t)nb * px * sizeof(uint16_t), hipMemcpyHostToDevice, X));
      ER_HIP_TRY(hipMemcpyAsync(S + o_c, dc, (size_t)nb * px * 3, hipMemcpyHostToDevice, X));
      dd = reinterpret_cast<const uint16_t*>(S + o_d);
      dc = reinterpret_cast<const uint8_t*>(S + o_c);
    }
    if (!warp) {
      hipLaunchKernelGGL(k_color_splat, dim3(blocks, (unsigned)nb), dim3(kBlock), 0, X, dd, dc, h->pixels, h->cols, h->cam, d_T + (size_t)start * 16,
                         h->ht_key, h->ht_slot, h->ht_cap - 1, h->ht_shift, h->max_units, h->color, d_stats);
      ER_HIP_TRY(hipGetLastError());
      continue;
    }
    uint16_t* Z = reinterpret_cast<uint16_t*>(S + o_Z);
    uint8_t* Cw = reinterpret_cast<uint8_t*>(S + o_C);
    uint32_t* win = reinterpret_cast<uint32_t*>(S + o_win);
    for (int f = 0; f < nb; f++) {
      const size_t F = (size_t)(start + f);
      const ReprojArgs RA{dd + (size_t)f * px, 1, h->cols, h->rows, h->cam, h->cami, reinterpret_cast<const double*>(S + o_seg) + F * 16,
                          reinterpret_cast<const double*>(S + o_madj) + F * 12, reinterpret_cast<const int*>(S + o_gi) + F,
                          reinterpret_cast<const float*>(S + o_ctr), warp->resolution, warp->length / (float)warp->resolution, (int)(verts * 3),
                          reinterpret_cast<uint32_t*>(S + o_zbuf), reinterpret_cast<uint32_t*>(S + o_lz), reinterpret_cast<uint32_t*>(S + o_zfix),
                          reinterpret_cast<int*>(S + o_flag)};
      if (reproject_single(h, RA, Z, X)) return 1;
      hipLaunchKernelGGL(k_color_warp, dim3(blocks), dim3(kBlock), 0, X, RA, Z, win);
      hipLaunchKernelGGL(k_color_gather, dim3(blocks), dim3(kBlock), 0, X, dc + (size_t)f * px * 3, win, Cw, h->pixels);
      ER_HIP_TRY(hipGetLastError());
      if (z_host) {
        ER_HIP_TRY(hipMemcpyAsync(z_host, Z, px * sizeof(uint16_t), hipMemcpyDeviceToHost, X));
        ER_HIP_TRY(hipMemcpyAsync(c_host, Cw, px * 3, hipMemcpyDeviceToHost, X));
      } else {
        hipLaunchKernelGGL(k_color_splat, dim3(blocks, 1u), dim3(kBlock), 0, X, Z, Cw, h->pixels, h->cols, h->cam, d_T + F * 16, h->ht_key, h->ht_slot,
                           h->ht_cap - 1, h->ht_shift, h->max_units, h->color, d_stats);
        ER_HIP_TRY(hipGetLastError());
      }
    }
  }
  unsigned long long st[3] = {0, 0, 0};
  ER_HIP_TRY(hipMemcpyAsync(st, d_stats, sizeof st, hipMemcpyDeviceToHost, X));
  ER_HIP_TRY(hipStreamSynchronize(X));
  if (stats)
    for (int k = 0; k < 3; k++) stats[k] = (long)st[k];
  return 0;
}

}

namespace er_tsdf_k {

int color_zero_slots(er_tsdf_t h, int n) {
  if (!h->color || n <= 0) return 0;
  hipLaunchKernelGGL(k_zero_unit_colors, dim3(kUnitVox / 256, n), dim3(256), 0, h->stream, h->color, h->slot_scratch, h->max_units);
  ER_HIP_TRY(hipGetLastError());
  return 0;
}

}

extern "C" {

int er_tsdf_color_enable(er_tsdf_t h) {
  if (!h) return er::fail("er_tsdf_color_enable: NULL handle");
  if (h->shard_world > 1) return er::fail("er_tsdf_color_enable: colour is not carried across GPUs (er_tsdf_set_unit_shard has world = %d)", h->shard_world);
  if (h->color) return 0;
  ER_HIP_TRY(hipSetDevice(h->device));
  const size_t bytes = (size_t)h->max_units * kUnitVox * 16;
  unsigned long long* c = nullptr;
  if (hipMalloc(&c, bytes) != hipSuccess) {
    (void)hipGetLastError();
    return er::fail("er_tsdf_color_enable: cannot allocate %zu bytes of device memory for the colour of %d units", bytes, h->max_units);
  }
  if (hipMemsetAsync(c, 0, bytes, h->stream) != hipSuccess || hipStreamSynchronize(h->stream) != hipSuccess) {
    (void)hipGetLastError();
    (void)hipFree(c);
    return er::fail("er_tsdf_color_enable: cannot zero %zu bytes of device memory", bytes);
  }
  h->color = c;
  return 0;
}

int er_tsdf_read_unit_color(er_tsdf_t h, int key, uint32_t* rgbn_host) {
  if (!h || !rgbn_host) return er::fail("er_tsdf_read_unit_color: NULL argument");
  ER_HIP_TRY(hipSetDevice(h->device));
  int slot;
  if (color_ready(h, "er_tsdf_read_unit_color") || unit_slot(h, "er_tsdf_read_unit_color", key, &slot)) return 1;
  ER_HIP_TRY(hipMemcpyAsync(rgbn_host, h->color + (size_t)slot * kUnitVox * 2, (size_t)kUnitVox * 16, hipMemcpyDeviceToHost, h->stream));
  ER_HIP_TRY(hipStreamSynchronize(h->stream));
  return 0;
}

int er_tsdf_write_unit_color(er_tsdf_t h, int key, const uint32_t* rgbn_host) {
  if (!h || !rgbn_host) return er::fail("er_tsdf_write_unit_color: NULL argument");
  ER_HIP_TRY(hipSetDevice(h->device));
  int slot;
  if (color_ready(h, "er_tsdf_write_unit_color") || unit_slot(h, "er_tsdf_write_unit_color", key, &slot)) return 1;
  ER_HIP_TRY(hipMemcpyAsync(h->color + (size_t)slot * kUnitVox * 2, rgbn_host, (size_t)kUnitVox * 16, hipMemcpyHostToDevice, h->stream));
  ER_HIP_TRY(hipStreamSynchronize(h->stream));
  return 0;
}

int er_tsdf_color_frames(er_tsdf_t h, int n, const uint16_t* depth, const uint8_t* rgb, int on_device, const double* T, const er_warp* warp,
                         long stats[3]) {
  if (!h) return er::fail("er_tsdf_color_frames: NULL handle");
  if (n < 0) return er::fail("er_tsdf_color_frames: negative frame count");
  if (n > 0 && (!depth || !rgb || !T)) return er::fail("er_tsdf_color_frames: NULL argument");
  ER_HIP_TRY(hipSetDevice(h->device));
  if (color_ready(h, "er_tsdf_color_frames")) return 1;
  return color_run(h, "er_tsdf_color_frames", n, depth, rgb, on_device, T, warp, nullptr, nullptr, stats);
}

int er_tsdf_reproject_color(er_tsdf_t h, uint16_t* depth_inout_host, uint8_t* rgb_inout_host, const float* ctr_host, int resolution, float length,
                            const double seg[16], const double madj[16]) {
  if (!h || !depth_inout_host || !rgb_inout_host || !ctr_host || !seg || !madj) return er::fail("er_tsdf_reproject_color: NULL argument");
  if (resolution <= 0) return er::fail("er_tsdf_reproject_color: bad resolution");
  ER_HIP_TRY(hipSetDevice(h->device));
  int gi = 0;
  const er_warp w{ctr_host, 1, resolution, length, &gi, seg, madj};
  return color_run(h, "er_tsdf_reproject_color", 1, depth_inout_host, rgb_inout_host, 0, nullptr, &w, depth_inout_host, rgb_inout_host, nullptr);
}

int er_tsdf_sample_colors(er_tsdf_t h, const float* points_host, long n, uint8_t* rgba_host, long counts[2]) {
  if (!h) return er::fail("er_tsdf_sample_colors: NULL handle");
  if (n < 0) return er::fail("er_tsdf_sample_colors: negative point count");
  if (n > 0 && (!points_host || !rgba_host)) return er::fail("er_tsdf_sample_colors: NULL argument");
  if (n > 0x7FFFFFFFL) return er::fail("er_tsdf_sample_colors: %ld points are more than the 2^31 - 1 a call takes", n);
  ER_HIP_TRY(hipSetDevice(h->device));
  if (color_ready(h, "er_tsdf_sample_colors")) return 1;
  if (check_flags(h)) return 1;
  if (counts) counts[0] = counts[1] = 0;
  if (n == 0) return 0;
  const size_t off_p = 256, off_o = off_p + round256((size_t)n * 16);
  if (ensure_color_scratch(h, off_o + round256((size_t)n * 4))) return 1;
  char* S = static_cast<char*>(h->color_scratch);
  unsigned long long* d_counts = reinterpret_cast<unsigned long long*>(S);
  ER_HIP_TRY(hipMemsetAsync(d_counts, 0, 2 * sizeof(unsigned long long), h->stream));
  ER_HIP_TRY(hipMemcpyAsync(S + off_p, points_host, (size_t)n * 16, hipMemcpyHostToDevice, h->stream));
  hipLaunchKernelGGL(k_color_sample, dim3((unsigned)((n + kBlock - 1) / kBlock)), dim3(kBlock), 0, h->stream, h->color, h->ht_key, h->ht_slot,
                     h->ht_cap - 1, h->ht_shift, h->max_units, reinterpret_cast<const float4*>(S + off_p), n, reinterpret_cast<uchar4*>(S + off_o), d_counts);
  ER_HIP_TRY(hipGetLastError());
  unsigned long long ct[2] = {0, 0};
  ER_HIP_TRY(hipMemcpyAsync(rgba_host, S + off_o, (size_t)n * 4, hipMemcpyDeviceToHost, h->stream));
  ER_HIP_TRY(hipMemcpyAsync(ct, d_counts, sizeof ct, hipMemcpyDeviceToHost, h->stream));
  ER_HIP_TRY(hipStreamSynchronize(h->stream));
  if (counts) {
    counts[0] = (long)ct[0];
    counts[1] = (long)ct[1];
  }
  return 0;
}

}
```

### elasticreconstruction_amd/csrc/er_tsdf_dev.h

```cpp
#pragma once

#include "er_tsdf.h"

namespace er_tsdf_k {
namespace {

__device__ __forceinline__ unsigned hash_unit_key(int key, int shift) { return ((unsigned)key * 2654435761u) >> shift; }

__device__ int ht_find_or_insert(int* __restrict__ ht_key, int cap_mask, int shift, int key) {
  unsigned h = hash_unit_key(key, shift);
  for (int probe = 0; probe <= cap_mask; ++probe) {
    int e = (int)((h + (unsigned)probe) & (unsigned)cap_mask);
    int k = __hip_atomic_load(&ht_key[e], __ATOMIC_RELAXED, __HIP_MEMORY_SCOPE_AGENT);
    if (k == key) return e;
    if (k == kEmptyKey) {
      int old = atomicCAS(&ht_key[e], kEmptyKey, key);
      if (old == kEmptyKey || old == key) return e;
    }
  }
  return -1;
}

__device__ __forceinline__ int ht_lookup_slot(const int* __restrict__ ht_key, const int* __restrict__ ht_slot, int cap_mask, int shift, int key) {
  unsigned h = hash_unit_key(key, shift);
  for (int probe = 0; probe <= cap_mask; ++probe) {
    const int e = (int)((h + (unsigned)probe) & (unsigned)cap_mask);
    const int k = ht_key[e];
    if (k == key) return ht_slot[e];
    if (k == kEmptyKey) return -1;
  }
  return -1;
}

__device__ __forceinline__ void scatter_px(const ReprojArgs& A, int f, int p, int cell, uint16_t dd, int replay) {
  const size_t o = (size_t)f * ((size_t)A.cols * A.rows) + cell;
  if (!replay) {
    if (dd != 0) {
      atomicMin(&A.zbuf[o], (uint32_t)dd);
    } else {
      atomicMax(&A.lastzero[o], (uint32_t)p + 1u);
      atomicOr(&A.zero_flag[f >> 5], 1 << (f & 31));
    }
  } else {
    const uint32_t lz = A.lastzero[o];
    if (dd != 0 && lz > 0 && (uint32_t)p + 1u > lz) atomicMin(&A.zfix[o], (uint32_t)dd);
  }
}

__device__ __forceinline__ void reproject_scatter_px(const ReprojArgs& A, int f, int u, int v, int replay) {
  const int pixels = A.cols * A.rows;
  const int p = v * A.cols + u;
  const uint16_t d = A.depth[(size_t)f * pixels + p];
  if (d == 0) return;
  int cell;
  uint16_t dd;
  if (!reproject_px(u, v, d, A.cam, A.cami, A.cols, A.rows, A.seg12 + f * 16, A.madj12 + f * 12,
                    A.ctr + (size_t)A.grid_index[f] * A.floats_per_grid, A.res, A.grid_ul, cell, dd))
    return;
  scatter_px(A, f, p, cell, dd, replay);
}

__device__ __forceinline__ uint32_t take_z(uint32_t z, size_t o, uint32_t* __restrict__ lastzero, uint32_t* __restrict__ zfix) {
  if (lastzero[o] == 0) return z;
  const uint32_t r = zfix[o];
  zfix[o] = kZEmpty;
  lastzero[o] = 0;
  return r;
}

}
}
```

### elasticreconstruction_amd/csrc/er_tsdf_pre.hip

```cpp
#include "er_tsdf_dev.h"

namespace er_tsdf_k {

__global__ void k_reproject_scatter(ReprojArgs A) {
  const int f = blockIdx.z;
  const int u = blockIdx.x * 64 + (threadIdx.x & 63);
  const int v = blockIdx.y * 4 + (threadIdx.x >> 6);
  if (u >= A.cols || v >= A.rows) return;
  reproject_scatter_px(A, f, u, v, 0);
}

namespace {

__device__ void touch_unit(int key, int f, int* __restrict__ ht_key, int* __restrict__ ht_slot,
                           unsigned long long* __restrict__ ht_mask, int cap_mask, int hash_shift,
                           int* __restrict__ batch, int* __restrict__ nbatch, int* __restrict__ counters, int2 shard) {
  if (shard.y > 1 && unit_owner(key, shard.y) != shard.x) return;
  const int e = ht_find_or_insert(ht_key, cap_mask, hash_shift, key);
  if (e < 0) {
    atomicOr(&counters[C_TABLE_FULL], 1);
    return;
  }
  const unsigned long long bit = 1ull << f;
  const unsigned long long seen = __hip_atomic_load(&ht_mask[e], __ATOMIC_RELAXED, __HIP_MEMORY_SCOPE_AGENT);
  if (seen & bit) return;
  const unsigned long long old = atomicOr(&ht_mask[e], bit);
  if (old != 0ull) return;
  batch[atomicAdd(nbatch, 1)] = e;
}

}

namespace {

template <int kCtrl>
__device__ __forceinline__ int dpp_mov(int v) {
  return __builtin_amdgcn_update_dpp(v, v, kCtrl, 0xF, 0xF, false);
}
constexpr int kDppQuadXor1 = 0xB1;
constexpr int kDppQuadXor2 = 0x4E;
constexpr int kDppRowShr1 = 0x111;
constexpr int kDppRowRor4 = 0x124;
constexpr int kDppRowRor8 = 0x128;

template <int kCtrl>
__device__ __forceinline__ float dpp_movf(float v) {
  return __int_as_float(dpp_mov<kCtrl>(__float_as_int(v)));
}

struct FMin { __device__ __forceinline__ float operator()(float a, float b) const { return fminf(a, b); } };
struct FMax { __device__ __forceinline__ float operator()(float a, float b) const { return fmaxf(a, b); } };

template <class Op>
__device__ __forceinline__ float across_rows(float v, Op op) {
  const unsigned u = (unsigned)__float_as_int(v);
  const auto s16 = __builtin_amdgcn_permlane16_swap(u, u, false, false);
  v = op(__int_as_float((int)s16[0]), __int_as_float((int)s16[1]));
  const unsigned w = (unsigned)__float_as_int(v);
  const auto s32 = __builtin_amdgcn_permlane32_swap(w, w, false, false);
  return op(__int_as_float((int)s32[0]), __int_as_float((int)s32[1]));
}

template <class Op>
__device__ __forceinline__ float reduce_half_columns(float v, Op op) {
  v = op(v, dpp_movf<kDppQuadXor1>(v));
  v = op(v, dpp_movf<kDppQuadXor2>(v));
  v = op(v, dpp_movf<kDppRowRor8>(v));
  return across_rows(v, op);
}

template <class Op>
__device__ __forceinline__ float reduce_wave(float v, Op op) {
  v = op(v, dpp_movf<kDppQuadXor1>(v));
  v = op(v, dpp_movf<kDppQuadXor2>(v));
  v = op(v, dpp_movf<kDppRowRor4>(v));
  v = op(v, dpp_movf<kDppRowRor8>(v));
  return across_rows(v, op);
}

}

static_assert(kTile == 32 && kPrepPix == 4 && kPrepThreads == 256, "k_prepare: 8 column groups x 32 rows of 4 pixels; a wave is 8 rows of the tile");
static_assert(kLoShift == 4 && kLoSub == 2, "k_prepare: a sub-tile is 4 threads (one quad) wide and 2 waves high; lane bit 2 is its column");
constexpr int kPrepCols = kTile / kPrepPix;
constexpr int kPrepWaveRows = 64 / kPrepCols;
constexpr int kPrepSubWaves = (1 << kLoShift) / kPrepWaveRows;

template <bool kWide>
__global__ __launch_bounds__(kPrepThreads) void k_prepare(
    const uint16_t* __restrict__ depth, uint32_t* __restrict__ zbuf, int n_frames, int cols, int rows,
    Camera cam, CameraInv cami, const float* __restrict__ lambda, const double* __restrict__ T12, float* __restrict__ scaled,
    int* __restrict__ ht_key, int* __restrict__ ht_slot, unsigned long long* __restrict__ ht_mask, int cap_mask,
    int hash_shift, int* __restrict__ batch, int* __restrict__ nbatch,
    int* __restrict__ counters, float* __restrict__ tile_max, float* __restrict__ tile_lo, float* __restrict__ tile_lo_fine, int2 shard,
    uint32_t* __restrict__ lastzero, uint32_t* __restrict__ zfix, const int* __restrict__ zero_flag) {
  __shared__ int s_keys[kTileKeys];
  __shared__ int s_n;
  __shared__ float s_wmax[kPrepThreads / 64], s_wlo[kLoSub][kLoSub][kPrepSubWaves];
  const int pixels = cols * rows;
  const int f = blockIdx.z;
  const bool replayed = zbuf && ((zero_flag[f >> 5] >> (f & 31)) & 1);
  const int c = threadIdx.x & (kPrepCols - 1), r = threadIdx.x / kPrepCols;
  const int x0 = blockIdx.x * kTile + c * kPrepPix, y = blockIdx.y * kTile + r;
  if (threadIdx.x == 0) s_n = 0;
  __syncthreads();
  const int p = y * cols + x0;
  const size_t o = (size_t)f * pixels + p;
  float* __restrict__ const sc_out = scaled + ((size_t)f * (pixels + kScaledPad) + p);
  uint16_t d[kPrepPix];
  float lam[kPrepPix];
  bool in[kPrepPix];
#pragma unroll
  for (int j = 0; j < kPrepPix; j++) {
    d[j] = 0;
    lam[j] = 0.0f;
    in[j] = y < rows && x0 + (kWide ? 0 : j) < cols;
  }
  if constexpr (kWide) {
    if (in[0]) {
      if (zbuf) {
        const uint4 zv = *reinterpret_cast<const uint4*>(zbuf + o);
        *reinterpret_cast<uint4*>(zbuf + o) = make_uint4(kZEmpty, kZEmpty, kZEmpty, kZEmpty);
        uint32_t z[kPrepPix] = {zv.x, zv.y, zv.z, zv.w};
        if (replayed) {
#pragma unroll
          for (int j = 0; j < kPrepPix; j++) z[j] = take_z(z[j], o + j, lastzero, zfix);
        }
#pragma unroll
        for (int j = 0; j < kPrepPix; j++) d[j] = (z[j] == kZEmpty) ? (uint16_t)0 : (uint16_t)z[j];
      } else {
        uint2 dv;
        __builtin_memcpy(&dv, __builtin_assume_aligned(depth + o, 8), 8);
        d[0] = (uint16_t)dv.x;
        d[1] = (uint16_t)(dv.x >> 16);
        d[2] = (uint16_t)dv.y;
        d[3] = (uint16_t)(dv.y >> 16);
      }
      const float4 lv = *reinterpret_cast<const float4*>(lambda + p);
      lam[0] = lv.x;
      lam[1] = lv.y;
      lam[2] = lv.z;
      lam[3] = lv.w;
    }
  } else {
#pragma unroll
    for (int j = 0; j < kPrepPix; j++) {
      if (in[j]) {
        if (zbuf) {
          uint32_t z = zbuf[o + j];
          zbuf[o + j] = kZEmpty;
          if (replayed) z = take_z(z, o + j, lastzero, zfix);
          d[j] = (z == kZEmpty) ? (uint16_t)0 : (uint16_t)z;
        } else {
          d[j] = depth[o + j];
        }
        lam[j] = lambda[p + j];
      }
    }
  }
  float wmax = 0.0f, vlo = 3.0e38f, sc[kPrepPix];
  int key[kPrepPix];
#pragma unroll
  for (int j = 0; j < kPrepPix; j++) {
    key[j] = -1;
    sc[j] = 0.0f;
    if (in[j]) {
      sc[j] = scale_depth_px(d[j], lam[j], cam.integration_trunc);
      if constexpr (!kWide) sc_out[j] = sc[j];
      wmax = fmaxf(wmax, sc[j]);
      vlo = fminf(vlo, sc[j] > 0.001f ? sc[j] : 0.0f);
      if (d[j] > 0) {
        key[j] = touch_key(x0 + j, y, d[j], cam, cami, T12 + f * 12);
        if (key[j] < 0) atomicAdd(&counters[C_OUT_OF_RANGE], 1);
      }
    }
  }
  if constexpr (kWide) {
    if (in[0]) *reinterpret_cast<float4*>(sc_out) = make_float4(sc[0], sc[1], sc[2], sc[3]);
  }
  const int left = dpp_mov<kDppRowShr1>(key[kPrepPix - 1]);
#pragma unroll
  for (int j = 0; j < kPrepPix; j++) {
    const bool leader = key[j] >= 0 && (j == 0 ? (c == 0 || left != key[0]) : key[j - 1] != key[j]);
    if (leader) {
      const int slot = atomicAdd(&s_n, 1);
      if (slot < kTileKeys) {
        s_keys[slot] = key[j];
      } else {
        touch_unit(key[j], f, ht_key, ht_slot, ht_mask, cap_mask, hash_shift, batch, nbatch, counters, shard);
      }
    }
  }
  const int lane = threadIdx.x & 63, wave = threadIdx.x >> 6;
  wmax = reduce_wave(wmax, FMax());
  vlo = reduce_half_columns(vlo, FMin());
  if (lane == 0) s_wmax[wave] = wmax;
  if ((lane & ~4) == 0) s_wlo[wave / kPrepSubWaves][lane >> 2][wave % kPrepSubWaves] = vlo;
  __syncthreads();
  if (threadIdx.x == 0) {
    float m = 0.0f, lo = 3.0e38f;
    for (int w = 0; w < kPrepThreads / 64; w++) m = fmaxf(m, s_wmax[w]);
    for (int e = 0; e < kLoSub * kLoSub * kPrepSubWaves; e++) lo = fminf(lo, (&s_wlo[0][0][0])[e]);
    const size_t t = ((size_t)blockIdx.y * gridDim.x + blockIdx.x) * ER_MAX_BATCH + f;
    tile_max[t] = m;
    tile_lo[t] = lo;
  }
  if ((int)threadIdx.x < kLoSub * kLoSub) {
    const int sr = threadIdx.x / kLoSub, sg = threadIdx.x % kLoSub;
    float lo = 3.0e38f;
    for (int w = 0; w < kPrepSubWaves; w++) lo = fminf(lo, s_wlo[sr][sg][w]);
    const int lx = blockIdx.x * kLoSub + sg, ly = blockIdx.y * kLoSub + sr;
    const int lo_tx = (cols + (1 << kLoShift) - 1) >> kLoShift, lo_ty = (rows + (1 << kLoShift) - 1) >> kLoShift;
    if (lx < lo_tx && ly < lo_ty) tile_lo_fine[((size_t)ly * lo_tx + lx) * ER_MAX_BATCH + f] = lo;
  }
  const int n = min(s_n, kTileKeys);
  if ((int)threadIdx.x < n) {
    const int k = s_keys[threadIdx.x];
    bool dup = false;
    for (int j = 0; j < (int)threadIdx.x; j++) dup = dup || (s_keys[j] == k);
    if (!dup) touch_unit(k, f, ht_key, ht_slot, ht_mask, cap_mask, hash_shift, batch, nbatch, counters, shard);
  }
}

#define ER_PREPARE_INST(W) \
  template __global__ void k_prepare<W>(const uint16_t* __restrict__, uint32_t* __restrict__, int, int, int, Camera, CameraInv, const float* __restrict__, \
                                        const double* __restrict__, float* __restrict__, int* __restrict__, int* __restrict__,                             \
                                        unsigned long long* __restrict__, int, int, int* __restrict__, int* __restrict__, int* __restrict__,               \
                                        float* __restrict__, float* __restrict__, float* __restrict__, int2, uint32_t* __restrict__,                       \
                                        uint32_t* __restrict__, const int* __restrict__);
ER_PREPARE_INST(true)
ER_PREPARE_INST(false)
#undef ER_PREPARE_INST

}
```

### elasticreconstruction_amd/tsdf.py

```python
import ctypes as C
import os

import numpy as np

from . import _ffi
from . import formats

UNIT_VOX = 64 * 64 * 64


def mat4_mul(A, B):
    A = np.asarray(A, np.float64)
    B = np.asarray(B, np.float64)
    out = np.empty((4, 4), np.float64)
    for r in range(4):
        for c in range(4):
            out[r, c] = ((A[r, 0] * B[0, c] + A[r, 1] * B[1, c]) + A[r, 2] * B[2, c]) + A[r, 3] * B[3, c]
    return out


class TSDFVolume:

    def __init__(self, cols=640, rows=480, camera=None, max_units=1024, device=0):
        self._lib = _ffi.lib()
        self.cols_, self.rows_ = int(cols), int(rows)
        cam = None if camera is None else np.ascontiguousarray(camera, dtype=np.float32)
        self.camera_ = formats.load_camera(None) if cam is None else cam
        self.max_units = int(max_units)
        self.device = int(device)
        h = C.c_void_p()
        _ffi.check(self._lib.er_tsdf_create(self.cols_, self.rows_,
                                            self.camera_.ctypes.data_as(C.POINTER(C.c_float)),
                                            self.max_units, self.device, C.byref(h)), "er_tsdf_create")
        self._h = h
        self.color_enabled_ = False

    def close(self):
        if getattr(self, "_h", None):
            self._lib.er_tsdf_destroy(self._h)
            self._h = None

    def __del__(self):
        try:
            self.close()
        except Exception:
            pass

    def set_stream(self, hip_stream_ptr):
        _ffi.check(self._lib.er_tsdf_set_stream(self._h, C.c_void_p(hip_stream_ptr)), "er_tsdf_set_stream")

    def synchronize(self):
        _ffi.check(self._lib.er_tsdf_synchronize(self._h), "er_tsdf_synchronize")

    def wait_event(self, hip_event_ptr):
        _ffi.check(self._lib.er_tsdf_wait_event(self._h, C.c_void_p(hip_event_ptr)), "er_tsdf_wait_event")

    def reset(self):
        _ffi.check(self._lib.er_tsdf_reset(self._h), "er_tsdf_reset")

    def set_unit_shard(self, rank, world):
        _ffi.check(self._lib.er_tsdf_set_unit_shard(self._h, int(rank), int(world)), "er_tsdf_set_unit_shard")

    def status(self):
        f, n = C.c_int(0), C.c_long(0)
        _ffi.check(self._lib.er_tsdf_status(self._h, C.byref(f), C.byref(n)), "er_tsdf_status")
        return f.value, n.value

    def ScaleDepth(self, depth):
        d = np.ascontiguousarray(depth, dtype=np.uint16).reshape(-1)
        assert d.size == self.cols_ * self.rows_
        out = np.empty(d.size, dtype=np.float32)
        _ffi.check(self._lib.er_tsdf_scale_depth(self._h, _ffi.ptr(d), _ffi.ptr(out)), "er_tsdf_scale_depth")
        return out

    def Reproject(self, depth, ctr, resolution, length, seg, madj):
        d = np.array(depth, dtype=np.uint16).reshape(-1)
        g = np.ascontiguousarray(ctr, dtype=np.float32).reshape(-1)
        s = np.ascontiguousarray(seg, dtype=np.float64).reshape(16)
        m = np.ascontiguousarray(madj, dtype=np.float64).reshape(16)
        _ffi.check(self._lib.er_tsdf_reproject(self._h, _ffi.ptr(d), _ffi.ptr(g), int(resolution), C.c_float(length),
                                               _ffi.ptr(s), _ffi.ptr(m)), "er_tsdf_reproject")
        return d

    def Integrate(self, depth, transformation):
        d = np.ascontiguousarray(depth, dtype=np.uint16).reshape(-1)
        T = np.ascontiguousarray(transformation, dtype=np.float64).reshape(16)
        _ffi.check(self._lib.er_tsdf_integrate(self._h, _ffi.ptr(d), _ffi.ptr(T)), "er_tsdf_integrate")

    @staticmethod
    def _warp_ref(warp, n):
        if warp is None:
            return None, []
        ctr = np.ascontiguousarray(warp["ctr"], dtype=np.float32)
        gi = np.ascontiguousarray(warp["grid_index"], dtype=np.int32).reshape(-1)
        seg = np.ascontiguousarray(warp["seg"], dtype=np.float64).reshape(-1, 16)
        madj = np.ascontiguousarray(warp["madj"], dtype=np.float64).reshape(-1, 16)
        assert gi.size == n and seg.shape[0] == n and madj.shape[0] == n
        res = int(warp["resolution"])
        num = ctr.size // (3 * (res + 1) ** 3)
        w = _ffi.ErWarp(ctr.ctypes.data_as(C.POINTER(C.c_float)), num, res, C.c_float(warp["length"]),
                        gi.ctypes.data_as(C.POINTER(C.c_int)), seg.ctypes.data_as(C.POINTER(C.c_double)),
                        madj.ctypes.data_as(C.POINTER(C.c_double)))
        return C.byref(w), [ctr, gi, seg, madj, w]

    def IntegrateFrames(self, depth, transformations, warp=None, device_ptr=None):
        T = np.ascontiguousarray(transformations, dtype=np.float64).reshape(-1, 16)
        n = T.shape[0]
        w_ref, keep = self._warp_ref(warp, n)
        if device_ptr is not None:
            _ffi.check(self._lib.er_tsdf_integrate_frames(self._h, n, C.c_void_p(device_ptr), 1, _ffi.ptr(T), w_ref),
                       "er_tsdf_integrate_frames")
        else:
            d = np.ascontiguousarray(depth, dtype=np.uint16).reshape(n, -1)
            assert d.shape[1] == self.cols_ * self.rows_
            _ffi.check(self._lib.er_tsdf_integrate_frames(self._h, n, _ffi.ptr(d), 0, _ffi.ptr(T), w_ref),
                       "er_tsdf_integrate_frames")
        del keep

    def prepass_trace(self, depth, transformations, warp=None, device_ptr=None):
        T = np.ascontiguousarray(transformations, dtype=np.float64).reshape(-1, 16)
        n = T.shape[0]
        w_ref, keep = self._warp_ref(warp, n)
        px = self.cols_ * self.rows_
        if device_ptr is not None:
            src, on_dev = C.c_void_p(device_ptr), 1
        else:
            d = np.ascontiguousarray(depth, dtype=np.uint16).reshape(n, -1)
            assert d.shape[1] == px
            src, on_dev = _ffi.ptr(d), 0
        B = 64
        tx, ty = (self.cols_ + 31) // 32, (self.rows_ + 31) // 32
        fx, fy = (self.cols_ + 15) // 16, (self.rows_ + 15) // 16
        pad, nk = C.c_int(0), C.c_int(0)
        pad_floats = 64
        scaled = np.empty((n, px + pad_floats), np.float32)
        tmax, tlo = np.empty((ty, tx, B), np.float32), np.empty((ty, tx, B), np.float32)
        fine = np.empty((fy, fx, B), np.float32)
        cap = 1 << 16
        keys, masks = np.empty(cap, np.int32), np.empty(cap, np.uint64)
        _ffi.check(self._lib.er_tsdf_prepass_trace(self._h, n, src, on_dev, _ffi.ptr(T), w_ref, _ffi.ptr(scaled), C.byref(pad), _ffi.ptr(tmax),
                                                   _ffi.ptr(tlo), _ffi.ptr(fine), _ffi.ptr(keys), _ffi.ptr(masks), cap, C.byref(nk)),
                   "er_tsdf_prepass_trace")
        del keep
        assert pad.value == pad_floats and nk.value <= cap
        return dict(scaled=scaled, pad=pad.value, tile_max=tmax[:, :, :n].copy(), tile_lo=tlo[:, :, :n].copy(),
                    tile_lo_fine=fine[:, :, :n].copy(), keys=keys[:nk.value].copy(), masks=masks[:nk.value].copy())

    def unit_count(self):
        n = C.c_int(0)
        _ffi.check(self._lib.er_tsdf_unit_count(self._h, C.byref(n)), "er_tsdf_unit_count")
        return n.value

    def unit_keys(self):
        n = self.unit_count()
        keys = np.empty(n, dtype=np.int32)
        if n:
            _ffi.check(self._lib.er_tsdf_unit_keys(self._h, _ffi.ptr(keys)), "er_tsdf_unit_keys")
        return keys

    def read_unit(self, key):
        sdf = np.empty(UNIT_VOX, dtype=np.float32)
        w = np.empty(UNIT_VOX, dtype=np.float32)
        _ffi.check(self._lib.er_tsdf_read_unit(self._h, int(key), _ffi.ptr(sdf), _ffi.ptr(w)), "er_tsdf_read_unit")
        return sdf, w

    def sum_weight(self):
        s = C.c_double(0)
        _ffi.check(self._lib.er_tsdf_sum_weight(self._h, C.byref(s)), "er_tsdf_sum_weight")
        return s.value

    def extract_world(self):
        n = C.c_long(0)
        _ffi.check(self._lib.er_tsdf_extract_world(self._h, None, 0, C.byref(n)), "er_tsdf_extract_world")
        out = np.empty((n.value, 4), dtype=np.float32)
        if n.value:
            _ffi.check(self._lib.er_tsdf_extract_world(self._h, _ffi.ptr(out), n.value, C.byref(n)), "er_tsdf_extract_world")
        return out

    def extract_surface(self):
        n = C.c_long(0)
        _ffi.check(self._lib.er_tsdf_extract_surface(self._h, None, 0, C.byref(n)), "er_tsdf_extract_surface")
        out = np.empty((n.value, 4), dtype=np.float32)
        if n.value:
            _ffi.check(self._lib.er_tsdf_extract_surface(self._h, _ffi.ptr(out), n.value, C.byref(n)), "er_tsdf_extract_surface")
        return out

    def extract_oriented(self):
        n = C.c_long(0)
        _ffi.check(self._lib.er_tsdf_extract_oriented(self._h, None, None, 0, C.byref(n)), "er_tsdf_extract_oriented")
        pts = np.empty((n.value, 4), dtype=np.float32)
        nrm = np.empty((n.value, 4), dtype=np.float32)
        if n.value:
            _ffi.check(self._lib.er_tsdf_extract_oriented(self._h, _ffi.ptr(pts), _ffi.ptr(nrm), n.value, C.byref(n)), "er_tsdf_extract_oriented")
        return pts, np.ascontiguousarray(nrm[:, :3])

    def raycast(self, T, cols=None, rows=None, cam=None, levels=1, params=None, device=False):
        cols = self.cols_ if cols is None else int(cols)
        rows = self.rows_ if rows is None else int(rows)
        cam4 = np.ascontiguousarray(np.asarray(self.camera_ if cam is None else cam, np.float32).reshape(-1)[:4])
        levels = int(levels)
        if levels < 1 or cols % (1 << (levels - 1)) or rows % (1 << (levels - 1)):
            raise ValueError("raycast: %d x %d is not divisible by 2^(levels-1), levels = %d" % (cols, rows, levels))
        T = np.ascontiguousarray(T, dtype=np.float64).reshape(16)
        P = None
        if params is not None:
            P = C.byref(_ffi.ErRaycastParams(*[float(np.float32(x)) for x in params]))
        if device:
            import torch
            dev = torch.device("cuda", self.device)
            torch.cuda.current_stream(dev).synchronize()
        out = []
        for l in range(levels):
            c, r = cols >> l, rows >> l
            k = np.ascontiguousarray(cam4 / np.float32(1 << l))
            if device:
                rec = torch.empty((r, c, 2, 4), dtype=torch.float32, device=dev)
                dep = torch.empty((r, c), dtype=torch.uint16, device=dev)
                rp, dp = C.c_void_p(rec.data_ptr()), C.c_void_p(dep.data_ptr())
            else:
                rec, dep = np.empty((r, c, 2, 4), np.float32), np.empty((r, c), np.uint16)
                rp, dp = _ffi.ptr(rec), _ffi.ptr(dep)
            _ffi.check(self._lib.er_tsdf_raycast(self._h, c, r, _ffi.ptr(k), _ffi.ptr(T), P, rp, dp, 1 if device else 0), "er_tsdf_raycast")
            if device:
                out.append((dep, rec[:, :, 0, :3], rec[:, :, 1, :3]))
            else:
                out.append((dep, np.ascontiguousarray(rec[:, :, 0, :3]), np.ascontiguousarray(rec[:, :, 1, :3])))
        return out

    def SaveFragment(self, filename, length=3.0):
        pts, nrm = self.extract_oriented()
        x = pts[:, :3]
        inside = ((x >= np.float32(0.0)) & (x < np.float32(length))).all(axis=1)
        formats.save_pcd_xyzn(filename, np.ascontiguousarray(x[inside]), np.ascontiguousarray(nrm[inside]))
        return int(inside.sum())

    def extract_mesh(self):
        n = C.c_long(0)
        _ffi.check(self._lib.er_tsdf_extract_mesh(self._h, None, 0, C.byref(n)), "er_tsdf_extract_mesh")
        out = np.empty((n.value, 3, 3), dtype=np.float32)
        if n.value:
            _ffi.check(self._lib.er_tsdf_extract_mesh(self._h, _ffi.ptr(out), n.value, C.byref(n)), "er_tsdf_extract_mesh")
        return out

    def SaveWorld(self, filename):
        pts = self.extract_world()
        formats.save_pcd_xyzi(filename, pts)
        return pts.shape[0]

    def extract_indexed_mesh(self, colors=False):
        nv, nt = C.c_long(0), C.c_long(0)
        _ffi.check(self._lib.er_tsdf_extract_mesh_indexed(self._h, None, None, 0, None, 0, C.byref(nv), C.byref(nt)), "er_tsdf_extract_mesh_indexed")
        verts = np.empty((nv.value, 4), dtype=np.float32)
        nrm = np.empty((nv.value, 4), dtype=np.float32)
        tris = np.empty((nt.value, 3), dtype=np.int32)
        if nv.value:
            _ffi.check(self._lib.er_tsdf_extract_mesh_indexed(self._h, _ffi.ptr(verts), _ffi.ptr(nrm), nv.value, _ffi.ptr(tris), nt.value,
                                                              C.byref(nv), C.byref(nt)), "er_tsdf_extract_mesh_indexed")
        if colors:
            return verts, np.ascontiguousarray(nrm[:, :3]), tris, self.sample_colors(verts)
        return verts, np.ascontiguousarray(nrm[:, :3]), tris

    def SaveMesh(self, filename, normals=True, binary=True, colors=None):
        if colors is None:
            colors = self.color_enabled_
        if colors:
            verts, nrm, tris, rgba = self.extract_indexed_mesh(colors=True)
        else:
            (verts, nrm, tris), rgba = self.extract_indexed_mesh(), None
        formats.save_ply(filename, verts, tris, nrm if normals else None, binary, colors=rgba)
        return verts.shape[0], tris.shape[0]

    def enable_color(self):
        _ffi.check(self._lib.er_tsdf_color_enable(self._h), "er_tsdf_color_enable")
        self.color_enabled_ = True

    def ColorFrames(self, depth, rgb, transformations, warp=None, device_ptrs=None):
        T = np.ascontiguousarray(transformations, dtype=np.float64).reshape(-1, 16)
        n = T.shape[0]
        w_ref, keep = self._warp_ref(warp, n)
        st = (C.c_long * 3)(0, 0, 0)
        if device_ptrs is not None:
            dp, cp, on_dev = C.c_void_p(device_ptrs[0]), C.c_void_p(device_ptrs[1]), 1
        else:
            d = np.ascontiguousarray(depth, dtype=np.uint16).reshape(-1)
            c = np.ascontiguousarray(rgb, dtype=np.uint8).reshape(-1)
            if d.size != n * self.cols_ * self.rows_ or c.size != 3 * d.size:
                raise ValueError("ColorFrames: %d depth pixels and %d colour bytes are not %d frames of a %d x %d image"
                                 % (d.size, c.size, n, self.cols_, self.rows_))
            dp, cp, on_dev = _ffi.ptr(d), _ffi.ptr(c), 0
        _ffi.check(self._lib.er_tsdf_color_frames(self._h, n, dp, cp, on_dev, _ffi.ptr(T), w_ref, st), "er_tsdf_color_frames")
        del keep
        return st[0], st[1], st[2]

    def ReprojectColor(self, depth, rgb, ctr, resolution, length, seg, madj):
        d = np.array(depth, dtype=np.uint16).reshape(-1)
        c = np.array(rgb, dtype=np.uint8).reshape(-1, 3)
        assert d.size == self.cols_ * self.rows_ and c.shape[0] == d.size
        g = np.ascontiguousarray(ctr, dtype=np.float32).reshape(-1)
        s = np.ascontiguousarray(seg, dtype=np.float64).reshape(16)
        m = np.ascontiguousarray(madj, dtype=np.float64).reshape(16)
        _ffi.check(self._lib.er_tsdf_reproject_color(self._h, _ffi.ptr(d), _ffi.ptr(c), _ffi.ptr(g), int(resolution), C.c_float(length),
                                                     _ffi.ptr(s), _ffi.ptr(m)), "er_tsdf_reproject_color")
        return d, c

    def read_unit_color(self, key):
        a = np.empty((UNIT_VOX, 4), dtype=np.uint32)
        _ffi.check(self._lib.er_tsdf_read_unit_color(self._h, int(key), _ffi.ptr(a)), "er_tsdf_read_unit_color")
        return a

    def write_unit_color(self, key, rgbn):
        a = np.ascontiguousarray(rgbn, dtype=np.uint32).reshape(UNIT_VOX, 4)
        _ffi.check(self._lib.er_tsdf_write_unit_color(self._h, int(key), _ffi.ptr(a)), "er_tsdf_write_unit_color")

    def sample_colors(self, points, counts=False):
        p = np.asarray(points, np.float32)
        if p.ndim != 2 or p.shape[1] not in (3, 4):
            raise ValueError("sample_colors: points must be [n, 3] or [n, 4], not %s" % (p.shape,))
        if p.shape[1] == 3:
            p = np.concatenate([p, np.zeros((p.shape[0], 1), np.float32)], axis=1)
        p = np.ascontiguousarray(p)
        out = np.zeros((p.shape[0], 4), dtype=np.uint8)
        ct = (C.c_long * 2)(0, 0)
        _ffi.check(self._lib.er_tsdf_sample_colors(self._h, _ffi.ptr(p), p.shape[0], _ffi.ptr(out), ct), "er_tsdf_sample_colors")
        return (out, (ct[0], ct[1])) if counts else out

    def LoadWorld(self, path_or_array):
        if isinstance(path_or_array, (str, bytes, os.PathLike)):
            f = formats.load_pcd(path_or_array)
            a = np.stack([np.asarray(f[k], np.float32).reshape(-1) for k in ("x", "y", "z", "intensity")], axis=1)
        else:
            a = np.asarray(path_or_array, np.float32)
        a = np.ascontiguousarray(a, dtype=np.float32).reshape(-1, 4)
        nu = C.c_int(0)
        _ffi.check(self._lib.er_tsdf_import_world(self._h, _ffi.ptr(a), a.shape[0], C.byref(nu)), "er_tsdf_import_world")
        return nu.value

    def export_weighted(self, keys, dev_ptr):
        k = np.ascontiguousarray(keys, dtype=np.int32)
        _ffi.check(self._lib.er_tsdf_export_weighted(self._h, _ffi.ptr(k), k.size, C.c_void_p(dev_ptr)), "er_tsdf_export_weighted")

    def import_weighted(self, keys, dev_ptr):
        k = np.ascontiguousarray(keys, dtype=np.int32)
        _ffi.check(self._lib.er_tsdf_import_weighted(self._h, _ffi.ptr(k), k.size, C.c_void_p(dev_ptr)), "er_tsdf_import_weighted")

    def export_raw(self, keys, dev_ptr):
        k = np.ascontiguousarray(keys, dtype=np.int32)
        _ffi.check(self._lib.er_tsdf_export_raw(self._h, _ffi.ptr(k), k.size, C.c_void_p(dev_ptr)), "er_tsdf_export_raw")

    def import_raw(self, keys, dev_ptr):
        k = np.ascontiguousarray(keys, dtype=np.int32)
        _ffi.check(self._lib.er_tsdf_import_raw(self._h, _ffi.ptr(k), k.size, C.c_void_p(dev_ptr)), "er_tsdf_import_raw")

    def band_sizes(self, keys):
        k = np.ascontiguousarray(keys, dtype=np.int32)
        out = np.zeros(k.size, np.int32)
        _ffi.check(self._lib.er_tsdf_band_sizes(self._h, _ffi.ptr(k), k.size, _ffi.ptr(out)), "er_tsdf_band_sizes")
        return out

    def export_band(self, keys, counts, dev_ptr):
        k, c = np.ascontiguousarray(keys, dtype=np.int32), np.ascontiguousarray(counts, dtype=np.int32)
        _ffi.check(self._lib.er_tsdf_export_band(self._h, _ffi.ptr(k), _ffi.ptr(c), k.size, C.c_void_p(dev_ptr)), "er_tsdf_export_band")

    def import_band(self, keys, rec_ptrs):
        k = np.ascontiguousarray(keys, dtype=np.int32)
        r = (C.c_void_p * k.size)(*[int(p) for p in rec_ptrs])
        _ffi.check(self._lib.er_tsdf_import_band(self._h, _ffi.ptr(k), k.size, r), "er_tsdf_import_band")

    def merge_band(self, keys, srcs, self_pos):
        k = np.ascontiguousarray(keys, dtype=np.int32)
        ns = np.asarray([len(x) for x in srcs], np.int32)
        sp = np.ascontiguousarray(self_pos, dtype=np.int32)
        r = (C.c_void_p * (16 * k.size))()
        for u, x in enumerate(srcs):
            for q, ptr in enumerate(x[:16]):
                r[16 * u + q] = int(ptr)
        _ffi.check(self._lib.er_tsdf_merge_band(self._h, _ffi.ptr(k), k.size, _ffi.ptr(ns), _ffi.ptr(sp), r), "er_tsdf_merge_band")

    def drop_units(self, keys):
        k = np.ascontiguousarray(keys, dtype=np.int32)
        _ffi.check(self._lib.er_tsdf_drop_units(self._h, _ffi.ptr(k), k.size), "er_tsdf_drop_units")

    def set_profiling(self, enable):
        _ffi.check(self._lib.er_tsdf_set_profiling(self._h, int(enable)), "er_tsdf_set_profiling")

    def get_profile(self):
        ms, ln, fr, uv = C.c_double(0), C.c_long(0), C.c_long(0), C.c_long(0)
        _ffi.check(self._lib.er_tsdf_get_profile(self._h, C.byref(ms), C.byref(ln), C.byref(fr), C.byref(uv)), "er_tsdf_get_profile")
        return {"integrate_ms": ms.value, "launches": ln.value, "frames": fr.value, "unit_visits": uv.value}


def raycast_batch(jobs, depth=True):
    import torch
    lib = _ffi.lib()
    keys = ("volume", "T", "cols", "rows", "cam", "params")
    jobs = [j if isinstance(j, dict) else dict(zip(keys, j)) for j in jobs]
    n = len(jobs)
    if n == 0:
        _ffi.check(lib.er_tsdf_raycast_batch(0, None, None, None, None, None, None, None, None), "er_tsdf_raycast_batch")
        return []
    dev = torch.device("cuda", jobs[0]["volume"].device)
    vols = (C.c_void_p * n)(*[j["volume"]._h.value for j in jobs])
    cols = np.array([int(j["cols"]) for j in jobs], np.int32)
    rows = np.array([int(j["rows"]) for j in jobs], np.int32)
    cam = np.ascontiguousarray([np.asarray(j["cam"], np.float32).reshape(-1)[:4] for j in jobs], dtype=np.float32)
    T = np.ascontiguousarray([np.asarray(j["T"], np.float64).reshape(16) for j in jobs], dtype=np.float64)
    P = None
    if any(j.get("params") is not None for j in jobs):
        d = _ffi.ErRaycastParams()
        _ffi.check(lib.er_raycast_params_default(C.byref(d)), "er_raycast_params_default")
        P = (_ffi.ErRaycastParams * n)()
        for q, j in enumerate(jobs):
            P[q] = d if j.get("params") is None else _ffi.ErRaycastParams(*[float(np.float32(x)) for x in j["params"]])
    recs = [torch.empty((max(int(r), 0), max(int(c), 0), 2, 4), dtype=torch.float32, device=dev) for c, r in zip(cols, rows)]
    deps = [torch.empty((max(int(r), 0), max(int(c), 0)), dtype=torch.uint16, device=dev) if depth else None for c, r in zip(cols, rows)]
    torch.cuda.current_stream(dev).synchronize()
    rp = (C.c_void_p * n)(*[t.data_ptr() for t in recs])
    dp = (C.c_void_p * n)(*[t.data_ptr() for t in deps]) if depth else None
    _ffi.check(lib.er_tsdf_raycast_batch(n, vols, _ffi.ptr(cols), _ffi.ptr(rows), _ffi.ptr(cam), _ffi.ptr(T), P, rp, dp), "er_tsdf_raycast_batch")
    return [(deps[q], recs[q][:, :, 0, :3], recs[q][:, :, 1, :3]) for q in range(n)]


class IntegrateApp:

    def __init__(self, cols=640, rows=480, max_units=1024, device=0, batch=64):
        self.cols_, self.rows_ = cols, rows
        self.traj_filename_ = ""
        self.pose_filename_ = ""
        self.seg_filename_ = ""
        self.camera_filename_ = ""
        self.ctr_filename_ = ""
        self.pcd_filename_ = "world.pcd"
        self.ctr_num_ = 0
        self.ctr_resolution_ = 8
        self.ctr_interval_ = 50
        self.ctr_length_ = 3.0
        self.start_from_ = -1
        self.end_at_ = 100000000
        self.exit_ = False
        self.frame_id_ = 0
        self.traj_ = []
        self.seg_traj_ = []
        self.pose_traj_ = []
        self.grids_ = None
        self.volume_ = None
        self._max_units, self._device, self._batch = max_units, device, int(batch)
        self._q_depth, self._q_T, self._q_gi, self._q_seg, self._q_madj = [], [], [], [], []
        self._q_color = []
        self.frames_integrated = 0

    def Init(self):
        import os
        camera = formats.load_camera(self.camera_filename_ if os.path.exists(self.camera_filename_ or "") else None)
        self.volume_ = TSDFVolume(self.cols_, self.rows_, camera, self._max_units, self._device)
        if self.ctr_num_ > 0 and os.path.exists(self.ctr_filename_ or "") and os.path.exists(self.seg_filename_ or ""):
            self.grids_ = formats.load_ctr(self.ctr_filename_, self.ctr_num_, self.ctr_resolution_)
        else:
            self.ctr_num_ = 0
        if os.path.exists(self.traj_filename_ or ""):
            self.traj_ = formats.load_log(self.traj_filename_)
        if os.path.exists(self.seg_filename_ or ""):
            self.seg_traj_ = formats.load_log(self.seg_filename_)
            if os.path.exists(self.pose_filename_ or ""):
                self.pose_traj_ = formats.load_log(self.pose_filename_)
                self.traj_ = []
                for i in range(len(self.pose_traj_)):
                    for j in range(self.ctr_interval_):
                        idx = i * self.ctr_interval_ + j
                        self.traj_.append(formats.FramedTransformation(
                            idx, idx, idx + 1, mat4_mul(self.pose_traj_[i].T, self.seg_traj_[idx].T)))

    def Execute(self, frame_id, depth, color=None):
        self.frame_id_ = frame_id
        if self.traj_[frame_id - 1].frame == -1:
            return
        if frame_id >= len(self.traj_):
            self.exit_ = True
            return
        if frame_id < self.start_from_ or frame_id > self.end_at_:
            if frame_id > self.end_at_:
                self.exit_ = True
            return
        T = self.traj_[frame_id - 1].T
        if self.ctr_num_ > 0:
            if frame_id > self.ctr_interval_ * self.ctr_num_:
                self.exit_ = True
                return
            chunk = (frame_id - 1) // self.ctr_interval_
            madj = mat4_mul(mat4_mul(_inverse(T), self.traj_[0].T), _inverse(self.seg_traj_[0].T))
            self._q_gi.append(chunk)
            self._q_seg.append(self.seg_traj_[frame_id - 1].T.copy())
            self._q_madj.append(madj)
        self._q_depth.append(np.ascontiguousarray(depth, dtype=np.uint16).reshape(-1))
        if color is not None:
            self._q_color.append(np.ascontiguousarray(color, dtype=np.uint8).reshape(-1, 3))
        self._q_T.append(T.copy())
        if len(self._q_depth) >= self._batch:
            self.Flush()

    def Flush(self):
        if not self._q_depth:
            return
        warp = None
        if self.ctr_num_ > 0:
            warp = dict(ctr=self.grids_, resolution=self.ctr_resolution_, length=np.float32(self.ctr_length_),
                        grid_index=np.array(self._q_gi, np.int32), seg=np.array(self._q_seg), madj=np.array(self._q_madj))
        self.volume_.IntegrateFrames(np.stack(self._q_depth), np.array(self._q_T), warp)
        if self._q_color:
            if len(self._q_color) != len(self._q_depth):
                raise ValueError("IntegrateApp: %d of the %d queued frames carry colour" % (len(self._q_color), len(self._q_depth)))
            self.volume_.enable_color()
            self.volume_.ColorFrames(np.stack(self._q_depth), np.stack(self._q_color), np.array(self._q_T), warp)
        self.frames_integrated += len(self._q_depth)
        self._q_depth, self._q_T, self._q_gi, self._q_seg, self._q_madj = [], [], [], [], []
        self._q_color = []

    def Finish(self, save=True):
        self.Flush()
        if save:
            return self.volume_.SaveWorld(self.pcd_filename_)
        return None


def _inverse(T):
    m = np.asarray(T, np.float64).reshape(16)
    inv = np.empty(16, np.float64)
    inv[0] = m[5] * m[10] * m[15] - m[5] * m[11] * m[14] - m[9] * m[6] * m[15] + m[9] * m[7] * m[14] + m[13] * m[6] * m[11] - m[13] * m[7] * m[10]
    inv[4] = -m[4] * m[10] * m[15] + m[4] * m[11] * m[14] + m[8] * m[6] * m[15] - m[8] * m[7] * m[14] - m[12] * m[6] * m[11] + m[12] * m[7] * m[10]
    inv[8] = m[4] * m[9] * m[15] - m[4] * m[11] * m[13] - m[8] * m[5] * m[15] + m[8] * m[7] * m[13] + m[12] * m[5] * m[11] - m[12] * m[7] * m[9]
    inv[12] = -m[4] * m[9] * m[14] + m[4] * m[10] * m[13] + m[8] * m[5] * m[14] - m[8] * m[6] * m[13] - m[12] * m[5] * m[10] + m[12] * m[6] * m[9]
    inv[1] = -m[1] * m[10] * m[15] + m[1] * m[11] * m[14] + m[9] * m[2] * m[15] - m[9] * m[3] * m[14] - m[13] * m[2] * m[11] + m[13] * m[3] * m[10]
    inv[5] = m[0] * m[10] * m[15] - m[0] * m[11] * m[14] - m[8] * m[2] * m[15] + m[8] * m[3] * m[14] + m[12] * m[2] * m[11] - m[12] * m[3] * m[10]
    inv[9] = -m[0] * m[9] * m[15] + m[0] * m[11] * m[13] + m[8] * m[1] * m[15] - m[8] * m[3] * m[13] - m[12] * m[1] * m[11] + m[12] * m[3] * m[9]
    inv[13] = m[0] * m[9] * m[14] - m[0] * m[10] * m[13] - m[8] * m[1] * m[14] + m[8] * m[2] * m[13] + m[12] * m[1] * m[10] - m[12] * m[2] * m[9]
    inv[2] = m[1] * m[6] * m[15] - m[1] * m[7] * m[14] - m[5] * m[2] * m[15] + m[5] * m[3] * m[14] + m[13] * m[2] * m[7] - m[13] * m[3] * m[6]
    inv[6] = -m[0] * m[6] * m[15] + m[0] * m[7] * m[14] + m[4] * m[2] * m[15] - m[4] * m[3] * m[14] - m[12] * m[2] * m[7] + m[12] * m[3] * m[6]
    inv[10] = m[0] * m[5] * m[15] - m[0] * m[7] * m[13] - m[4] * m[1] * m[15] + m[4] * m[3] * m[13] + m[12] * m[1] * m[7] - m[12] * m[3] * m[5]
    inv[14] = -m[0] * m[5] * m[14] + m[0] * m[6] * m[13] + m[4] * m[1] * m[14] - m[4] * m[2] * m[13] - m[12] * m[1] * m[6] + m[12] * m[2] * m[5]
    inv[3] = -m[1] * m[6] * m[11] + m[1] * m[7] * m[10] + m[5] * m[2] * m[11] - m[5] * m[3] * m[10] - m[9] * m[2] * m[7] + m[9] * m[3] * m[6]
    inv[7] = m[0] * m[6] * m[11] - m[0] * m[7] * m[10] - m[4] * m[2] * m[11] + m[4] * m[3] * m[10] + m[8] * m[2] * m[7] - m[8] * m[3] * m[6]
    inv[11] = -m[0] * m[5] * m[11] + m[0] * m[7] * m[9] + m[4] * m[1] * m[11] - m[4] * m[3] * m[9] - m[8] * m[1] * m[7] + m[8] * m[3] * m[5]
    inv[15] = m[0] * m[5] * m[10] - m[0] * m[6] * m[9] - m[4] * m[1] * m[10] + m[4] * m[2] * m[9] + m[8] * m[1] * m[6] - m[8] * m[2] * m[5]
    det = m[0] * inv[0] + m[1] * inv[4] + m[2] * inv[8] + m[3] * inv[12]
    det = 1.0 / det
    return (inv * det).reshape(4, 4)


def reproject_matrix(traj_f, traj_0, seg_0):
    return mat4_mul(mat4_mul(_inverse(traj_f), traj_0), _inverse(seg_0))
```

### include/er_hip.h

```cpp
#ifndef ER_HIP_H_
#define ER_HIP_H_

#include <stddef.h>
#include <stdint.h>

#ifdef __cplusplus
extern "C" {
#endif

#define ER_UNIT_RES 64
#define ER_UNIT_VOX (64 * 64 * 64)
#define ER_MAX_BATCH 64

const char* er_last_error(void);
int er_device_count(void);
int er_abi_version(void);
int er_request_hw_queues(int n);

void* er_host_alloc(size_t bytes);
int er_host_free(void* p);
int er_host_copy_h2d(void* dev_dst, const void* host_src, size_t bytes);
void* er_device_alloc(size_t bytes, int device);
int er_device_free(void* p);
int er_device_copy_d2h(void* host_dst, const void* dev_src, size_t bytes);

typedef struct er_tsdf_s* er_tsdf_t;

typedef struct er_warp {
  const float* ctr;
  int num_grids;
  int resolution;
  float length;
  const int* grid_index;
  const double* seg;
  const double* madj;
} er_warp;

int er_tsdf_create(int cols, int rows, const float cam6[6], int max_units, int device, er_tsdf_t* out);
int er_tsdf_destroy(er_tsdf_t h);

int er_tsdf_set_stream(er_tsdf_t h, void* hip_stream);
int er_tsdf_synchronize(er_tsdf_t h);

int er_tsdf_scale_depth(er_tsdf_t h, const uint16_t* depth_host, float* scaled_host);

int er_tsdf_reproject(er_tsdf_t h, uint16_t* depth_inout_host, const float* ctr_host, int resolution, float length,
                      const double seg[16], const double madj[16]);

int er_tsdf_integrate(er_tsdf_t h, const uint16_t* depth_host, const double T[16]);

int er_tsdf_integrate_frames(er_tsdf_t h, int n, const uint16_t* depth, int depth_on_device, const double* T,
                             const er_warp* warp);

int er_tsdf_prepass_trace(er_tsdf_t h, int n, const uint16_t* depth, int depth_on_device, const double* T, const er_warp* warp,
                          float* scaled, int* scaled_pad, float* tile_max, float* tile_lo, float* tile_lo_fine,
                          int* keys, unsigned long long* masks, int keys_cap, int* n_keys);

int er_tsdf_wait_event(er_tsdf_t h, void* hip_event);

int er_tsdf_reset(er_tsdf_t h);

#define ER_STATUS_POOL_EXHAUSTED 1
#define ER_STATUS_TABLE_FULL 2
int er_tsdf_status(er_tsdf_t h, int* flags, long* out_of_range_pixels);

int er_tsdf_unit_count(er_tsdf_t h, int* count);
int er_tsdf_unit_keys(er_tsdf_t h, int* keys_host);
int er_tsdf_read_unit(er_tsdf_t h, int key, float* sdf_host, float* weight_host);

int er_tsdf_sum_weight(er_tsdf_t h, double* sum);

int er_tsdf_extract_world(er_tsdf_t h, float* out_host, long capacity, long* count);

int er_tsdf_extract_surface(er_tsdf_t h, float* out_host, long capacity, long* count);

int er_tsdf_extract_oriented(er_tsdf_t h, float* points_host, float* normals_host, long capacity, long* count);

int er_tsdf_extract_mesh(er_tsdf_t h, float* tri_host, long capacity_triangles, long* n_triangles);
int er_mc_table(unsigned char out[256 * 16]);

int er_tsdf_extract_mesh_indexed(er_tsdf_t h, float* verts_host, float* normals_host, long capacity_vertices, int* tri_host,
                                 long capacity_triangles, long* n_vertices, long* n_triangles);

int er_tsdf_import_world(er_tsdf_t h, const float* xyzi_host, long n, int* n_units);

int er_tsdf_color_enable(er_tsdf_t h);

int er_tsdf_read_unit_color(er_tsdf_t h, int key, uint32_t* rgbn_host);
int er_tsdf_write_unit_color(er_tsdf_t h, int key, const uint32_t* rgbn_host);

int er_tsdf_color_frames(er_tsdf_t h, int n, const uint16_t* depth, const uint8_t* rgb, int on_device, const double* T, const er_warp* warp,
                         long stats[3]);

int er_tsdf_reproject_color(er_tsdf_t h, uint16_t* depth_inout_host, uint8_t* rgb_inout_host, const float* ctr_host, int resolution, float length,
                            const double seg[16], const double madj[16]);

int er_tsdf_sample_colors(er_tsdf_t h, const float* points_host, long n, uint8_t* rgba_host, long counts[2]);

typedef struct er_raycast_params {
  float t_min, t_max, step;
} er_raycast_params;
int er_raycast_params_default(er_raycast_params* p);
int er_tsdf_raycast(er_tsdf_t h, int cols, int rows, const float cam4[4], const double T[16], const er_raycast_params* params,
                    void* rec_out , uint16_t* depth_out , int out_on_device);

int er_tsdf_raycast_batch(int n_jobs, const er_tsdf_t* vol, const int* cols, const int* rows, const float* cam4 ,
                          const double* T , const er_raycast_params* params ,
                          void* const* rec_out_dev, uint16_t* const* depth_out_dev);

int er_tsdf_export_weighted(er_tsdf_t h, const int* keys_host, int n_keys, float* dev_buf);
int er_tsdf_import_weighted(er_tsdf_t h, const int* keys_host, int n_keys, const float* dev_buf);
int er_tsdf_export_raw(er_tsdf_t h, const int* keys_host, int n_keys, float* dev_buf);
int er_tsdf_import_raw(er_tsdf_t h, const int* keys_host, int n_keys, const float* dev_buf);
int er_tsdf_band_sizes(er_tsdf_t h, const int* keys_host, int n_keys, int* words_host);
int er_tsdf_export_band(er_tsdf_t h, const int* keys_host, const int* words_host, int n_keys, void* dev_block);
int er_tsdf_merge_band(er_tsdf_t h, const int* keys_host, int n_keys, const int* nsrc, const int* self_pos, const void* const* recs);
int er_tsdf_import_band(er_tsdf_t h, const int* keys_host, int n_keys, const void* const* recs);
int er_tsdf_drop_units(er_tsdf_t h, const int* keys_host, int n_keys);

int er_tsdf_set_unit_shard(er_tsdf_t h, int rank, int world);
int er_unit_owner(int key, int world);

typedef struct er_comm_s* er_comm_t;
#define ER_COMM_ID_BYTES 128
int er_comm_unique_id(unsigned char id[ER_COMM_ID_BYTES]);
int er_comm_create(const unsigned char id[ER_COMM_ID_BYTES], int rank, int world, int device, er_comm_t* out);
int er_comm_create_local(int n, const int* devices, er_comm_t* out );
int er_comm_create_loopback(int n, int device, er_comm_t* out );
int er_comm_destroy(er_comm_t c);
int er_comm_rank(er_comm_t c);
int er_comm_world(er_comm_t c);
#define ER_MERGE_ALL (-1)
#define ER_MERGE_DISTRIBUTED (-2)
int er_tsdf_allreduce(er_tsdf_t h, er_comm_t c, int root, int* union_units);
int er_comm_merge_stats(er_comm_t c, long long stats[8]);
int er_comm_merge_stats_owner(er_comm_t c, long long stats[12]);
void er_frame_block(int n_frames, int rank, int world, int* lo, int* hi);

int er_tsdf_set_profiling(er_tsdf_t h, int enable);
int er_tsdf_get_profile(er_tsdf_t h, double* integrate_ms_total, long* integrate_launches, long* frames,
                        long* unit_visits);

typedef struct er_cloud_s* er_cloud_t;

int er_cloud_create(const float* xyz_host, const float* normal_host, int n, float grid_cell, int device,
                    er_cloud_t* out);
int er_cloud_create_batch(int n_clouds, const float* const* xyz_host, const float* const* normal_host, const int* counts, float grid_cell,
                          int device, er_cloud_t* out);
int er_cloud_create_from_tsdf(er_tsdf_t h, float cube_length, float grid_cell, er_cloud_t* out, int* n_points);
int er_cloud_destroy(er_cloud_t c);
int er_cloud_size(er_cloud_t c);

int er_icp_count_inliers(er_cloud_t src, er_cloud_t tgt, const double T[16], double max_dist, int* count);

int er_icp_align(er_cloud_t src, er_cloud_t tgt, const float guess[16], double max_dist, int max_iter,
                 double transformation_epsilon, int stop_rule, float out[16], int* iterations, int* converged,
                 double* fitness);

int er_find_correspondence(er_cloud_t src, er_cloud_t tgt, const double T[16], double dist, double normal_cos,
                           int* pairs_host, int capacity, int* n_pairs, double* info36);

int er_icp_align_trace(er_cloud_t src, er_cloud_t tgt, const float guess[16], double max_dist, int max_iter, double transformation_epsilon,
                       int stop_rule, int pts, int row_capacity, double* totals, float* fin, float* delta, int* state, double* prev_mse,
                       double* fx_scale, int* n_rows, float out[16], int* iterations, int* converged);

int er_icp_count_inliers_batch(int n, const er_cloud_t* src, const er_cloud_t* tgt, const double* T, double max_dist, int* counts);
int er_icp_align_batch(int n, const er_cloud_t* src, const er_cloud_t* tgt, const float* guess, double max_dist, int max_iter,
                       double transformation_epsilon, int stop_rule, float* out, int* iterations, int* converged,
                       double* fitness);
int er_find_correspondence_batch(int n, const er_cloud_t* src, const er_cloud_t* tgt, const double* T, double dist,
                                 double normal_cos, int* const* pairs_host, const int* capacity, int* n_pairs,
                                 double* info36);

int er_ransac_fitness_batch(er_cloud_t src, er_cloud_t tgt, int n_hyp, const float* M, float corr_dist_threshold,
                            int* inliers, double* fitness);

int er_ransac_inliers(er_cloud_t src, er_cloud_t tgt, const float* M16, float corr_dist_threshold, int* pairs_host, int capacity,
                      int* n_inliers, double* fitness, double* info_source36, double* info_target36);

typedef struct er_features_s* er_features_t;

int er_features_create(const float* feat_host, int n, int dim, int device, er_features_t* out);
int er_features_destroy(er_features_t f);
int er_features_size(er_features_t f);

int er_feature_knn(er_features_t src, er_features_t tgt, int k, int* idx_host, float* sqdist_host);

int er_ransac_hypotheses(er_cloud_t src, er_cloud_t tgt, int n_hyp, int nr_samples, const int* sample_idx, const int* corr_idx,
                         float similarity, float angle_diff, int* status, float* M);

typedef struct er_ransac_params {
  int max_iterations;
  int nr_samples;
  int k_correspondences;
  float similarity;
  float max_corr_dist;
  float inlier_fraction;
  int inlier_number;
  float angle_diff;
  unsigned int seed;
  int chunk_iterations;
} er_ransac_params;
typedef struct er_ransac_stats {
  long long iterations, polygon_rejections, normal_rejections, scored;
} er_ransac_stats;
typedef struct er_ransac_aux {
  int iteration, count;
  double error;
  float M[16];
} er_ransac_aux;
int er_ransac_params_default(er_ransac_params* p);

int er_ransac_align(er_cloud_t src, er_cloud_t tgt, er_features_t src_feat, er_features_t tgt_feat, const er_ransac_params* p,
                    float T_out[16], int* converged, int* n_inliers, double* error, er_ransac_stats* stats, er_ransac_aux* aux,
                    int aux_capacity, int* aux_count);

int er_ransac_align_batch(int n_pairs, const er_cloud_t* src, const er_cloud_t* tgt, const er_features_t* src_feat, const er_features_t* tgt_feat,
                          const er_ransac_params* p, const unsigned int* seeds, int max_concurrent, float* T_out, int* converged, int* n_inliers,
                          double* error, er_ransac_stats* stats, double* info_source36, double* info_target36);


int er_cloud_read(er_cloud_t c, float* xyz_host, float* normal_host);

int er_cloud_voxel_grid(er_cloud_t in, float leaf, float grid_cell, er_cloud_t* out, int* n_out);

int er_cloud_estimate_normals(er_cloud_t in, float radius, er_cloud_t* out, int* n_neighbours_host);

int er_fpfh_estimate(er_cloud_t c, float radius, er_features_t* out, int* spfh_counts_host, int* n_neighbours_host);

int er_features_dim(er_features_t f);
int er_features_read(er_features_t f, float* feat_host);

int er_icp_release_workspaces(void);

int er_registration_batch(int n, const er_cloud_t* src, const er_cloud_t* tgt, const double* T_guess, double reg_dist, int reg_num, double reg_ratio,
                          int max_iter, double transformation_epsilon, int stop_rule, double corr_dist, double normal_cos, int* counts,
                          int* accepted, float* T_final, int* iterations, int* converged, int* const* pairs_host, const int* capacity,
                          int* n_pairs, double* info36);

typedef struct er_odom_s* er_odom_t;
typedef struct er_odom_params {
  int levels;
  int iterations[4];
  int bilateral;
  int max_depth_mm;
  int min_valid;
  float dist_thresh;
  float angle_thresh;
} er_odom_params;
int er_odom_params_default(er_odom_params* p);

int er_odom_create(int cols, int rows, const float* cam4, const er_odom_params* params, int device, er_odom_t* out);
int er_odom_destroy(er_odom_t h);

#define ER_ODOM_OK 0
#define ER_ODOM_LOST 1
#define ER_ODOM_TRACE 17
int er_odom_align_pairs(er_odom_t h, int n_frames, const uint16_t* depth, int depth_on_device, int n_pairs, const int* model_idx,
                        const int* frame_idx, const double* guess, double* T_out, int* status, double* trace, double* sums, int window);

int er_odom_track(er_odom_t h, int n_frames, const uint16_t* depth, int depth_on_device, double* T_rel, int* status, int window);

int er_frame_to_model_align(er_odom_t h, const void* const* model_rec_dev , int n_frames, const uint16_t* depth,
                            int depth_on_device, const double* guess, double* T_out, int* status, double* trace, double* sums, int window);

int er_frames_to_models_align(er_odom_t h, int n_models, const void* const* model_rec_dev , int n_frames,
                              const uint16_t* depth, int depth_on_device, const int* model_of_frame , const double* guess,
                              double* T_out, int* status, double* trace, double* sums, int window);

int er_odom_linearize(er_odom_t h, const uint16_t* depth2, int on_device, int level, const double* T, double* sums, int* count);

int er_odom_read_maps(er_odom_t h, const uint16_t* depth1, int on_device, int level, uint16_t* depth_out, float* vmap_out, float* nmap_out);

#define ER_ODOM_DEPTH_W 512
int er_odom_tables(float* space, float* depth_w, int* n_depth_w);

typedef struct er_frag_s* er_frag_t;
typedef struct er_frag_params {
  int interval;
  int lanes;
  int max_units;
  float length;
  er_raycast_params raycast;
} er_frag_params;
int er_frag_params_default(er_frag_params* p);
int er_frag_create(int cols, int rows, const float cam6[6], const er_odom_params* odom_params, const er_frag_params* frag_params, int device,
                   er_frag_t* out);
int er_frag_destroy(er_frag_t h);
int er_frag_lane_bytes(er_frag_t h, size_t* bytes);
int er_frag_build(er_frag_t h, int n_frames, const uint16_t* depth, int depth_on_device, const double* T0, int n_T0, double* W_out, int* status);
int er_frag_count(er_frag_t h, int* n_fragments);
int er_frag_read(er_frag_t h, int fragment, float* xyz_out, float* normals_out, long capacity, long* count);

typedef struct er_pgo_s* er_pgo_t;
#define ER_PGO_SWITCHABLE 0
#define ER_PGO_EM 1

int er_pgo_create(int n_poses, int n_loops, const double* odo_T, const double* odo_info, const int* loop_ids, const double* loop_T,
                  const double* loop_info, int device, er_pgo_t* out);
int er_pgo_destroy(er_pgo_t h);

int er_pgo_optimize(er_pgo_t h, int method, double weight, int max_iteration, double* poses_out, double* switch_or_weight_out, int* iterations,
                    int* trials, double* chi2_trace);

int er_pgo_set_profiling(er_pgo_t h, int on);
int er_pgo_get_profile(er_pgo_t h, double* stage_ms5);

int er_pgo_set_state(er_pgo_t h, const double* poses, const double* switches);
int er_pgo_get_state(er_pgo_t h, double* poses, double* switches);
int er_pgo_linearize(er_pgo_t h, double weight, double lambda, double* H_out, double* b_out, double* chi2_out);
int er_pgo_trial(er_pgo_t h, double weight, double lambda, double* dx_out, double* ds_out, double* F_new_out, int* status_out);

typedef struct er_fopt_s* er_fopt_t;

int er_fopt_create(int num, int resolution, float length, int device, er_fopt_t* out);
int er_fopt_destroy(er_fopt_t h);

int er_fopt_set_cloud(er_fopt_t h, int frag, const float* xyz_host, const float* normal_host, int n, int* first_out_of_bound);
int er_fopt_cloud_size(er_fopt_t h, int frag);
int er_fopt_get_points(er_fopt_t h, int frag, int* idx0, float* val, float* nval, float* p, float* n);

int er_fopt_update_pose(er_fopt_t h, int frag, const float M[16]);
int er_fopt_update_point_pn(er_fopt_t h, int frag, const double* ctr_slice_host);

int er_fopt_set_correspondences(er_fopt_t h, int n_pairs, const int* frag_i, const int* frag_j, const int* const* pairs_host,
                                const int* counts);
int er_fopt_set_correspondences_dev(er_fopt_t h, int n_pairs, const int* frag_i, const int* frag_j, const int* const* pairs_dev,
                                    const int* counts);
int er_fopt_group_count(er_fopt_t h);
int er_fopt_group_info(er_fopt_t h, int* info4);
int er_fopt_update_normals(er_fopt_t h, int frag, const double* ctr_slice_host);

int er_fopt_assemble_rigid(er_fopt_t h, double* JJ, double* Jb, double* score);
int er_fopt_assemble_slac(er_fopt_t h, const double* pose_rot_t, double* JJ, double* Jb, double* score);

int er_fopt_assemble_nonrigid(er_fopt_t h, double weight, double* diag, double* offdiag);

int er_fopt_factor_slac(er_fopt_t h, const double* pose_rot_t, double default_weight, double* dataJb_host, double* score);
int er_fopt_factor_nonrigid(er_fopt_t h, double weight);
int er_fopt_solve(er_fopt_t h, const double* rhs_host, int add_data_jb, double* x_host);
int er_fopt_debug_shift_diagonal(er_fopt_t h, long index, double value);

#ifdef __cplusplus
}
#endif
#endif
```

Measured before the change: 193,600 frames/s.

## Epoch-tag z-buffer entries instead of clearing them; fold hash-mask reset into plan

Z-buffer cells now carry a 16-bit epoch tag in their high bits. Readers decode a cell as empty when its tag does not match the current epoch, so the prepare and zbuf_to_depth kernels no longer write kZEmpty back after reading. A full memset is issued only when the epoch counter wraps. Separately, the ht_mask clearing and nbatch reset from the standalone k_reset kernel move into k_plan, which removes one kernel launch and the deferred-reset bookkeeping per batch. The cost is a tag compare on every z read and a new API for setting the epoch.

New measurement: 196,100 frames/s (median of 6 runs). 1.3% higher.

```diff
diff --git a/elasticreconstruction_amd/_ffi.py b/elasticreconstruction_amd/_ffi.py
--- a/elasticreconstruction_amd/_ffi.py
+++ b/elasticreconstruction_amd/_ffi.py
@@ -8,7 +8,7 @@
     "er_last_error", "er_device_count", "er_abi_version", "er_request_hw_queues", "er_host_alloc", "er_host_free", "er_host_copy_h2d", "er_device_alloc", "er_device_free", "er_device_copy_d2h",
     "er_tsdf_create", "er_tsdf_destroy", "er_tsdf_set_stream", "er_tsdf_synchronize",
     "er_tsdf_wait_event", "er_tsdf_reset", "er_tsdf_status", "er_tsdf_set_unit_shard", "er_unit_owner",
-    "er_tsdf_scale_depth", "er_tsdf_reproject", "er_tsdf_integrate", "er_tsdf_integrate_frames", "er_tsdf_prepass_trace",
+    "er_tsdf_scale_depth", "er_tsdf_reproject", "er_tsdf_integrate", "er_tsdf_integrate_frames", "er_tsdf_prepass_trace", "er_tsdf_set_zbuf_epoch",
     "er_tsdf_unit_count", "er_tsdf_unit_keys", "er_tsdf_read_unit", "er_tsdf_sum_weight",
     "er_tsdf_extract_world", "er_tsdf_extract_surface", "er_tsdf_extract_oriented", "er_tsdf_extract_mesh", "er_mc_table", "er_tsdf_extract_mesh_indexed", "er_tsdf_import_world", "er_raycast_params_default", "er_tsdf_raycast", "er_tsdf_raycast_batch", "er_tsdf_export_weighted", "er_tsdf_import_weighted",
     "er_tsdf_export_raw", "er_tsdf_import_raw",
@@ -111,6 +111,8 @@
     L.er_tsdf_integrate_frames.argtypes = [vp, C.c_int, vp, C.c_int, vp, C.POINTER(ErWarp)]
     if hasattr(L, "er_tsdf_prepass_trace"):
         L.er_tsdf_prepass_trace.argtypes = [vp, C.c_int, vp, C.c_int, vp, C.POINTER(ErWarp), vp, ip, vp, vp, vp, vp, vp, C.c_int, ip]
+    if hasattr(L, "er_tsdf_set_zbuf_epoch"):
+        L.er_tsdf_set_zbuf_epoch.argtypes = [vp, C.c_int, C.c_uint]
     L.er_tsdf_unit_count.argtypes = [vp, ip]
     L.er_tsdf_unit_keys.argtypes = [vp, vp]
     L.er_tsdf_read_unit.argtypes = [vp, C.c_int, vp, vp]
diff --git a/elasticreconstruction_amd/csrc/er_tsdf.h b/elasticreconstruction_amd/csrc/er_tsdf.h
--- a/elasticreconstruction_amd/csrc/er_tsdf.h
+++ b/elasticreconstruction_amd/csrc/er_tsdf.h
@@ -16,12 +16,14 @@
 constexpr int kBlock = 256;
 constexpr int kEmptyKey = -1;
 constexpr uint32_t kZEmpty = 0xFFFFFFFFu;
+constexpr uint32_t kZEpochMax = 0xFFFFu;
 
 enum { C_NUNITS = 0, C_NBATCH = 1 , C_POOL_OVERFLOW = 2, C_TABLE_FULL = 3, C_OUT_OF_RANGE = 4,
        C_NBATCH1 = 6, C_NBATCH2 = 7, C_ZERO_WRITE = 8 ,
        C_ZERO_WRITE1 = 10, C_COUNT = 12 };
 constexpr int kDepth = 3;
 constexpr int kAux = 2;
+constexpr int kZColor = kAux;
 
 struct ReprojArgs {
   const uint16_t* depth;
@@ -39,6 +41,7 @@
   uint32_t* lastzero;
   uint32_t* zfix;
   int* zero_flag;
+  uint32_t ztag;
 };
 __global__ void k_reproject_scatter(ReprojArgs A);
 
@@ -61,9 +64,9 @@
     int* __restrict__ ht_key, int* __restrict__ ht_slot, unsigned long long* __restrict__ ht_mask, int cap_mask,
     int hash_shift, int* __restrict__ batch, int* __restrict__ nbatch,
     int* __restrict__ counters, float* __restrict__ tile_max, float* __restrict__ tile_lo, float* __restrict__ tile_lo_fine, int2 shard,
-    uint32_t* __restrict__ lastzero, uint32_t* __restrict__ zfix, const int* __restrict__ zero_flag);
-extern template __global__ void k_prepare<true>(const uint16_t* __restrict__, uint32_t* __restrict__, int, int, int, Camera, CameraInv, const float* __restrict__, const double* __restrict__, float* __restrict__, int* __restrict__, int* __restrict__, unsigned long long* __restrict__, int, int, int* __restrict__, int* __restrict__, int* __restrict__, float* __restrict__, float* __restrict__, float* __restrict__, int2, uint32_t* __restrict__, uint32_t* __restrict__, const int* __restrict__);
-extern template __global__ void k_prepare<false>(const uint16_t* __restrict__, uint32_t* __restrict__, int, int, int, Camera, CameraInv, const float* __restrict__, const double* __restrict__, float* __restrict__, int* __restrict__, int* __restrict__, unsigned long long* __restrict__, int, int, int* __restrict__, int* __restrict__, int* __restrict__, float* __restrict__, float* __restrict__, float* __restrict__, int2, uint32_t* __restrict__, uint32_t* __restrict__, const int* __restrict__);
+    uint32_t* __restrict__ lastzero, uint32_t* __restrict__ zfix, const int* __restrict__ zero_flag, uint32_t ztag);
+extern template __global__ void k_prepare<true>(const uint16_t* __restrict__, uint32_t* __restrict__, int, int, int, Camera, CameraInv, const float* __restrict__, const double* __restrict__, float* __restrict__, int* __restrict__, int* __restrict__, unsigned long long* __restrict__, int, int, int* __restrict__, int* __restrict__, int* __restrict__, float* __restrict__, float* __restrict__, float* __restrict__, int2, uint32_t* __restrict__, uint32_t* __restrict__, const int* __restrict__, uint32_t);
+extern template __global__ void k_prepare<false>(const uint16_t* __restrict__, uint32_t* __restrict__, int, int, int, Camera, CameraInv, const float* __restrict__, const double* __restrict__, float* __restrict__, int* __restrict__, int* __restrict__, unsigned long long* __restrict__, int, int, int* __restrict__, int* __restrict__, int* __restrict__, float* __restrict__, float* __restrict__, float* __restrict__, int2, uint32_t* __restrict__, uint32_t* __restrict__, const int* __restrict__, uint32_t);
 
 constexpr int kRows = 4;
 constexpr int kItemsPerUnit = 256;
@@ -127,11 +130,11 @@
   int ctr_parity = 0, ctr_cur = 0;
   uint16_t* depth_stage[er_tsdf_k::kDepth] = {};
   uint32_t *zbuf[er_tsdf_k::kAux] = {}, *lastzero[er_tsdf_k::kAux] = {}, *zfix[er_tsdf_k::kAux] = {};
+  uint32_t zepoch[er_tsdf_k::kAux + 1] = {};
   double *T12 = nullptr, *seg12 = nullptr, *madj12 = nullptr, *dsum = nullptr;
   int *grid_index = nullptr, *key_scratch = nullptr, *slot_scratch = nullptr;
   er_tsdf_k::PlanRec* plan_rec[er_tsdf_k::kDepth] = {};
   er_tsdf_k::Plan* plan[er_tsdf_k::kDepth] = {};
-  bool reset_pending[er_tsdf_k::kDepth] = {};
   size_t key_scratch_cap = 0;
   int prof_stride = 0;
   long prof_tick = 0;
@@ -150,6 +153,7 @@
 __attribute__((visibility("hidden"))) int check_flags(er_tsdf_t h);
 __attribute__((visibility("hidden"))) int resolve_slots(er_tsdf_t h, const int* keys_host, int n, bool allocate);
 __attribute__((visibility("hidden"))) int sorted_units(er_tsdf_t h, std::vector<int>& keys, std::vector<int>& slots);
+__attribute__((visibility("hidden"))) int next_ztag(er_tsdf_t h, int which, uint32_t* zbuf, size_t cells, hipStream_t X, uint32_t* ztag);
 __attribute__((visibility("hidden"))) int reproject_single(er_tsdf_t h, const ReprojArgs& RA, uint16_t* z_dev, hipStream_t X);
 __attribute__((visibility("hidden"))) int color_zero_slots(er_tsdf_t h, int n);
 }
diff --git a/elasticreconstruction_amd/csrc/er_tsdf.hip b/elasticreconstruction_amd/csrc/er_tsdf.hip
--- a/elasticreconstruction_amd/csrc/er_tsdf.hip
+++ b/elasticreconstruction_amd/csrc/er_tsdf.hip
@@ -30,12 +30,11 @@
   }
 }
 
-__global__ void k_zbuf_to_depth(uint32_t* __restrict__ zbuf, uint16_t* __restrict__ depth, long total, uint32_t* __restrict__ lastzero,
-                                uint32_t* __restrict__ zfix, const int* __restrict__ zero_flag) {
+__global__ void k_zbuf_to_depth(const uint32_t* __restrict__ zbuf, uint16_t* __restrict__ depth, long total, uint32_t* __restrict__ lastzero,
+                                uint32_t* __restrict__ zfix, const int* __restrict__ zero_flag, uint32_t ztag) {
   long t = (long)blockIdx.x * blockDim.x + threadIdx.x;
   if (t >= total) return;
-  uint32_t z = zbuf[t];
-  zbuf[t] = kZEmpty;
+  uint32_t z = z_of_epoch(zbuf[t], ztag);
   if (zero_flag[0] & 1) z = take_z(z, (size_t)t, lastzero, zfix);
   depth[t] = (z == kZEmpty) ? (uint16_t)0 : (uint16_t)z;
 }
@@ -66,11 +65,11 @@
   return slot;
 }
 
-__global__ __launch_bounds__(256) void k_plan(const int* __restrict__ batch, const int* __restrict__ nbatch,
-                                              const unsigned long long* __restrict__ ht_mask, const int* __restrict__ ht_key,
+__global__ __launch_bounds__(256) void k_plan(const int* __restrict__ batch, int* nbatch,
+                                              unsigned long long* __restrict__ ht_mask, const int* __restrict__ ht_key,
                                               int* __restrict__ ht_slot, int* __restrict__ unit_key, int max_units,
                                               int* __restrict__ counters, PlanRec* __restrict__ plan_rec, Plan* __restrict__ plan,
-                                              int* __restrict__ zero_flag) {
+                                              int* __restrict__ zero_flag, unsigned long long* __restrict__ stats) {
   __shared__ int hist[65];
   __shared__ int start[66];
   const int n = *nbatch;
@@ -89,9 +88,13 @@
     if (zero_flag) zero_flag[0] = zero_flag[1] = 0;
   }
   __syncthreads();
+  if (threadIdx.x == 0) *nbatch = 0;
+  unsigned long long visits = 0;
   for (int t = threadIdx.x; t < n; t += blockDim.x) {
     const int e = batch[t];
     const unsigned long long mask = ht_mask[e];
+    ht_mask[e] = 0ull;
+    visits += (unsigned long long)__popcll(mask);
     const int key = ht_key[e];
     PlanRec r;
     r.key = key;
@@ -99,20 +102,7 @@
     r.mask = mask;
     plan_rec[atomicAdd(&start[__popcll(mask)], 1)] = r;
   }
-}
-
-__global__ void k_reset(const int* __restrict__ batch, int* __restrict__ nbatch, unsigned long long* __restrict__ ht_mask,
-                        unsigned long long* __restrict__ stats) {
-  const int n = *nbatch;
-  unsigned long long visits = 0;
-  for (int t = threadIdx.x; t < n; t += blockDim.x) {
-    const int e = batch[t];
-    visits += (unsigned long long)__popcll(ht_mask[e]);
-    ht_mask[e] = 0ull;
-  }
   if (visits) atomicAdd(&stats[0], visits);
-  __syncthreads();
-  if (threadIdx.x == 0) *nbatch = 0;
 }
 
 __global__ void k_sum_weight(const float2* __restrict__ pool, long n_vox, double* __restrict__ out) {
@@ -224,6 +214,16 @@
   return 0;
 }
 
+int next_ztag(er_tsdf_t h, int which, uint32_t* zbuf, size_t cells, hipStream_t X, uint32_t* ztag) {
+  if (h->zepoch[which] >= kZEpochMax) {
+    ER_HIP_TRY(hipMemsetAsync(zbuf, 0xFF, cells * sizeof(uint32_t), X));
+    h->zepoch[which] = 0;
+  }
+  h->zepoch[which]++;
+  *ztag = (kZEpochMax - h->zepoch[which]) << 16;
+  return 0;
+}
+
 int resolve_slots(er_tsdf_t h, const int* keys_host, int n, bool allocate) {
   if (join_voxel(h) || ensure_key_scratch(h, (size_t)n)) return 1;
   ER_HIP_TRY(hipMemcpyAsync(h->key_scratch, keys_host, (size_t)n * sizeof(int), hipMemcpyHostToDevice, h->stream));
@@ -269,20 +269,7 @@
   int gi[ER_MAX_BATCH];
 };
 
-int flush_resets(er_tsdf_t h) {
-  if (join_voxel(h)) return 1;
-  for (int q = 0; q < kDepth; q++)
-    if (h->reset_pending[q]) {
-      hipLaunchKernelGGL(k_reset, dim3(1), dim3(kBlock), 0, h->stream, h->batch[q], h->counters + kNbatchSlot[q], h->ht_mask[q], h->stats);
-      ER_HIP_TRY(hipGetLastError());
-      ER_HIP_TRY(hipEventRecord(h->int_done[q], h->stream));
-      h->reset_pending[q] = false;
-    }
-  return 0;
-}
-
 int sync_all(er_tsdf_t h) {
-  if (flush_resets(h)) return 1;
   if (h->copy_stream) ER_HIP_TRY(hipStreamSynchronize(h->copy_stream));
   for (int a = 0; a < kAux; a++) ER_HIP_TRY(hipStreamSynchronize(h->aux_stream[a]));
   if (h->stream != h->own_stream) ER_HIP_TRY(hipStreamSynchronize(h->own_stream));
@@ -336,18 +323,15 @@
     }
   }
   if (h->used[p]) ER_HIP_TRY(hipStreamWaitEvent(X, h->int_done[p], 0));
-  if (h->reset_pending[p]) {
-    hipLaunchKernelGGL(k_reset, dim3(1), dim3(kBlock), 0, X, h->batch[p], nbatch, h->ht_mask[p], h->stats);
-    ER_HIP_TRY(hipGetLastError());
-    h->reset_pending[p] = false;
-  }
   ER_HIP_TRY(hipMemcpyAsync(h->dstage[p], st, sizeof(Staging), hipMemcpyHostToDevice, X));
   ER_HIP_TRY(hipEventRecord(h->consts_done[p], X));
+  uint32_t ztag = 0;
   if (warp) {
+    if (next_ztag(h, a, h->zbuf[a], (size_t)ER_MAX_BATCH * (size_t)h->pixels, X, &ztag)) return 1;
     const int verts = (warp->resolution + 1) * (warp->resolution + 1) * (warp->resolution + 1);
     const float grid_ul = warp->length / (float)warp->resolution;
     const ReprojArgs RA{depth_dev, n, h->cols, h->rows, h->cam, h->cami, dev_seg, dev_madj, dev_gi, h->ctr, warp->resolution, grid_ul,
-                        verts * 3, h->zbuf[a], h->lastzero[a], h->zfix[a], h->counters + kZeroFlagSlot[a]};
+                        verts * 3, h->zbuf[a], h->lastzero[a], h->zfix[a], h->counters + kZeroFlagSlot[a], ztag};
     if (launch_reproject(h, RA, n, X)) return 1;
     zsrc = h->zbuf[a];
   }
@@ -357,9 +341,9 @@
                      depth_dev, zsrc, n, h->cols, h->rows, h->cam, h->cami, h->lambda, dev_t12, h->scaled[p], h->ht_key, h->ht_slot,
                      h->ht_mask[p], h->ht_cap - 1, h->ht_shift, h->batch[p], nbatch, h->counters,
                      h->tile_max[p], h->tile_lo[p], h->tile_lo_fine[p], make_int2(h->shard_rank, h->shard_world), h->lastzero[a], h->zfix[a],
-                     h->counters + kZeroFlagSlot[a]);
+                     h->counters + kZeroFlagSlot[a], ztag);
   hipLaunchKernelGGL(k_plan, dim3(1), dim3(256), 0, X, h->batch[p], nbatch, h->ht_mask[p], h->ht_key, h->ht_slot, h->unit_key, h->max_units,
-                     h->counters, h->plan_rec[p], h->plan[p], warp ? h->counters + kZeroFlagSlot[a] : (int*)nullptr);
+                     h->counters, h->plan_rec[p], h->plan[p], warp ? h->counters + kZeroFlagSlot[a] : (int*)nullptr, h->stats);
   ER_HIP_TRY(hipGetLastError());
   ER_HIP_TRY(hipEventRecord(h->pre_done[p], X));
 
@@ -381,7 +365,6 @@
   }
   ER_HIP_TRY(hipGetLastError());
   ER_HIP_TRY(hipEventRecord(h->int_done[p], S));
-  h->reset_pending[p] = true;
   h->used[p] = true;
   h->frames_done += n;
   return 0;
@@ -658,11 +641,13 @@
   ER_HIP_TRY(hipMemcpyAsync(h->grid_index, &gi, sizeof(int), hipMemcpyHostToDevice, h->stream));
   const float grid_ul = length / (float)resolution;
   const long total = (long)px;
+  uint32_t ztag = 0;
+  if (next_ztag(h, 0, h->zbuf[0], (size_t)ER_MAX_BATCH * px, h->stream, &ztag)) return 1;
   const ReprojArgs RA{h->depth_stage[0], 1, h->cols, h->rows, h->cam, h->cami, h->seg12, h->madj12, h->grid_index, h->ctr, resolution, grid_ul,
-                      verts * 3, h->zbuf[0], h->lastzero[0], h->zfix[0], h->counters + kZeroFlagSlot[0]};
+                      verts * 3, h->zbuf[0], h->lastzero[0], h->zfix[0], h->counters + kZeroFlagSlot[0], ztag};
   if (launch_reproject(h, RA, 1, h->stream)) return 1;
   hipLaunchKernelGGL(k_zbuf_to_depth, dim3((int)((total + kBlock - 1) / kBlock)), dim3(kBlock), 0, h->stream, h->zbuf[0],
-                     h->depth_stage[0], total, h->lastzero[0], h->zfix[0], h->counters + kZeroFlagSlot[0]);
+                     h->depth_stage[0], total, h->lastzero[0], h->zfix[0], h->counters + kZeroFlagSlot[0], ztag);
   ER_HIP_TRY(hipGetLastError());
   ER_HIP_TRY(hipMemsetAsync(h->counters + kZeroFlagSlot[0], 0, 2 * sizeof(int), h->stream));
   ER_HIP_TRY(hipMemcpyAsync(depth_inout_host, h->depth_stage[0], px * sizeof(uint16_t), hipMemcpyDeviceToHost, h->stream));
@@ -756,6 +741,20 @@
   return 0;
 }
 
+int er_tsdf_set_zbuf_epoch(er_tsdf_t h, int which, unsigned epoch) {
+  if (!h) return er::fail("er_tsdf_set_zbuf_epoch: NULL handle");
+  if (which < 0 || which > kZColor) return er::fail("er_tsdf_set_zbuf_epoch: no z-buffer %d (0, 1: the pre-pass streams'; %d: the colour calls')", which, kZColor);
+  if (epoch > kZEpochMax) return er::fail("er_tsdf_set_zbuf_epoch: epoch %u above %u", epoch, kZEpochMax);
+  ER_HIP_TRY(hipSetDevice(h->device));
+  if (sync_all(h)) return 1;
+  if (which < kAux && epoch < h->zepoch[which]) {
+    ER_HIP_TRY(hipMemsetAsync(h->zbuf[which], 0xFF, (size_t)ER_MAX_BATCH * (size_t)h->pixels * sizeof(uint32_t), h->stream));
+    ER_HIP_TRY(hipStreamSynchronize(h->stream));
+  }
+  h->zepoch[which] = epoch;
+  return 0;
+}
+
 int er_tsdf_wait_event(er_tsdf_t h, void* hip_event) {
   if (!h || !hip_event) return er::fail("er_tsdf_wait_event: NULL argument");
   ER_HIP_TRY(hipSetDevice(h->device));
@@ -778,8 +777,12 @@
   ER_HIP_TRY(hipMemsetAsync(h->ht_slot, 0xFF, (size_t)h->ht_cap * sizeof(int), s));
   for (int q = 0; q < kDepth; q++) ER_HIP_TRY(hipMemsetAsync(h->ht_mask[q], 0, (size_t)h->ht_cap * sizeof(unsigned long long), s));
   ER_HIP_TRY(hipMemsetAsync(h->counters, 0, C_COUNT * sizeof(int), s));
+  for (int q = 0; q < kAux; q++) {
+    ER_HIP_TRY(hipMemsetAsync(h->zbuf[q], 0xFF, (size_t)ER_MAX_BATCH * (size_t)h->pixels * sizeof(uint32_t), s));
+    h->zepoch[q] = 0;
+  }
   ER_HIP_TRY(hipStreamSynchronize(s));
-  for (int q = 0; q < kDepth; q++) h->used[q] = h->reset_pending[q] = false;
+  for (int q = 0; q < kDepth; q++) h->used[q] = false;
   h->batch_no = 0;
   h->dropped.clear();
   return 0;
@@ -867,7 +870,7 @@
 int er_tsdf_set_profiling(er_tsdf_t h, int enable) {
   if (!h) return er::fail("er_tsdf_set_profiling: NULL handle");
   ER_HIP_TRY(hipSetDevice(h->device));
-  if (flush_resets(h) || drain_events(h)) return 1;
+  if (join_voxel(h) || drain_events(h)) return 1;
   h->prof_stride = enable > 0 ? enable : 0;
   h->prof_tick = 0;
   h->ms_total = 0.0;
@@ -881,7 +884,7 @@
                         long* unit_visits) {
   if (!h) return er::fail("er_tsdf_get_profile: NULL handle");
   ER_HIP_TRY(hipSetDevice(h->device));
-  if (flush_resets(h)) return 1;
+  if (join_voxel(h)) return 1;
   ER_HIP_TRY(hipStreamSynchronize(h->stream));
   if (drain_events(h)) return 1;
   unsigned long long st[4] = {0, 0, 0, 0};
@@ -902,7 +905,7 @@
   if (launch_reproject(h, RA, 1, X)) return 1;
   const long total = (long)RA.cols * RA.rows;
   hipLaunchKernelGGL(k_zbuf_to_depth, dim3((int)((total + kBlock - 1) / kBlock)), dim3(kBlock), 0, X, RA.zbuf, z_dev, total, RA.lastzero, RA.zfix,
-                     RA.zero_flag);
+                     RA.zero_flag, RA.ztag);
   ER_HIP_TRY(hipGetLastError());
   ER_HIP_TRY(hipMemsetAsync(RA.zero_flag, 0, 2 * sizeof(int), X));
   return 0;
diff --git a/elasticreconstruction_amd/csrc/er_tsdf_color.hip b/elasticreconstruction_amd/csrc/er_tsdf_color.hip
--- a/elasticreconstruction_amd/csrc/er_tsdf_color.hip
+++ b/elasticreconstruction_amd/csrc/er_tsdf_color.hip
@@ -244,11 +244,13 @@
     uint32_t* win = reinterpret_cast<uint32_t*>(S + o_win);
     for (int f = 0; f < nb; f++) {
       const size_t F = (size_t)(start + f);
+      uint32_t ztag = 0;
+      if (next_ztag(h, kZColor, reinterpret_cast<uint32_t*>(S + o_zbuf), px, X, &ztag)) return 1;
       const ReprojArgs RA{dd + (size_t)f * px, 1, h->cols, h->rows, h->cam, h->cami, reinterpret_cast<const double*>(S + o_seg) + F * 16,
                           reinterpret_cast<const double*>(S + o_madj) + F * 12, reinterpret_cast<const int*>(S + o_gi) + F,
                           reinterpret_cast<const float*>(S + o_ctr), warp->resolution, warp->length / (float)warp->resolution, (int)(verts * 3),
                           reinterpret_cast<uint32_t*>(S + o_zbuf), reinterpret_cast<uint32_t*>(S + o_lz), reinterpret_cast<uint32_t*>(S + o_zfix),
-                          reinterpret_cast<int*>(S + o_flag)};
+                          reinterpret_cast<int*>(S + o_flag), ztag};
       if (reproject_single(h, RA, Z, X)) return 1;
       hipLaunchKernelGGL(k_color_warp, dim3(blocks), dim3(kBlock), 0, X, RA, Z, win);
       hipLaunchKernelGGL(k_color_gather, dim3(blocks), dim3(kBlock), 0, X, dc + (size_t)f * px * 3, win, Cw, h->pixels);
diff --git a/elasticreconstruction_amd/csrc/er_tsdf_dev.h b/elasticreconstruction_amd/csrc/er_tsdf_dev.h
--- a/elasticreconstruction_amd/csrc/er_tsdf_dev.h
+++ b/elasticreconstruction_amd/csrc/er_tsdf_dev.h
@@ -36,7 +36,7 @@
   const size_t o = (size_t)f * ((size_t)A.cols * A.rows) + cell;
   if (!replay) {
     if (dd != 0) {
-      atomicMin(&A.zbuf[o], (uint32_t)dd);
+      atomicMin(&A.zbuf[o], A.ztag | (uint32_t)dd);
     } else {
       atomicMax(&A.lastzero[o], (uint32_t)p + 1u);
       atomicOr(&A.zero_flag[f >> 5], 1 << (f & 31));
@@ -60,6 +60,11 @@
   scatter_px(A, f, p, cell, dd, replay);
 }
 
+__device__ __forceinline__ uint32_t z_of_epoch(uint32_t z, uint32_t ztag) {
+  const uint32_t x = z ^ ztag;
+  return x < 0x10000u ? x : kZEmpty;
+}
+
 __device__ __forceinline__ uint32_t take_z(uint32_t z, size_t o, uint32_t* __restrict__ lastzero, uint32_t* __restrict__ zfix) {
   if (lastzero[o] == 0) return z;
   const uint32_t r = zfix[o];
diff --git a/elasticreconstruction_amd/csrc/er_tsdf_pre.hip b/elasticreconstruction_amd/csrc/er_tsdf_pre.hip
--- a/elasticreconstruction_amd/csrc/er_tsdf_pre.hip
+++ b/elasticreconstruction_amd/csrc/er_tsdf_pre.hip
@@ -93,7 +93,7 @@
     int* __restrict__ ht_key, int* __restrict__ ht_slot, unsigned long long* __restrict__ ht_mask, int cap_mask,
     int hash_shift, int* __restrict__ batch, int* __restrict__ nbatch,
     int* __restrict__ counters, float* __restrict__ tile_max, float* __restrict__ tile_lo, float* __restrict__ tile_lo_fine, int2 shard,
-    uint32_t* __restrict__ lastzero, uint32_t* __restrict__ zfix, const int* __restrict__ zero_flag) {
+    uint32_t* __restrict__ lastzero, uint32_t* __restrict__ zfix, const int* __restrict__ zero_flag, uint32_t ztag) {
   __shared__ int s_keys[kTileKeys];
   __shared__ int s_n;
   __shared__ float s_wmax[kPrepThreads / 64], s_wlo[kLoSub][kLoSub][kPrepSubWaves];
@@ -120,8 +120,7 @@
     if (in[0]) {
       if (zbuf) {
         const uint4 zv = *reinterpret_cast<const uint4*>(zbuf + o);
-        *reinterpret_cast<uint4*>(zbuf + o) = make_uint4(kZEmpty, kZEmpty, kZEmpty, kZEmpty);
-        uint32_t z[kPrepPix] = {zv.x, zv.y, zv.z, zv.w};
+        uint32_t z[kPrepPix] = {z_of_epoch(zv.x, ztag), z_of_epoch(zv.y, ztag), z_of_epoch(zv.z, ztag), z_of_epoch(zv.w, ztag)};
         if (replayed) {
 #pragma unroll
           for (int j = 0; j < kPrepPix; j++) z[j] = take_z(z[j], o + j, lastzero, zfix);
@@ -147,8 +146,7 @@
     for (int j = 0; j < kPrepPix; j++) {
       if (in[j]) {
         if (zbuf) {
-          uint32_t z = zbuf[o + j];
-          zbuf[o + j] = kZEmpty;
+          uint32_t z = z_of_epoch(zbuf[o + j], ztag);
           if (replayed) z = take_z(z, o + j, lastzero, zfix);
           d[j] = (z == kZEmpty) ? (uint16_t)0 : (uint16_t)z;
         } else {
@@ -227,7 +225,7 @@
                                         const double* __restrict__, float* __restrict__, int* __restrict__, int* __restrict__,                             \
                                         unsigned long long* __restrict__, int, int, int* __restrict__, int* __restrict__, int* __restrict__,               \
                                         float* __restrict__, float* __restrict__, float* __restrict__, int2, uint32_t* __restrict__,                       \
-                                        uint32_t* __restrict__, const int* __restrict__);
+                                        uint32_t* __restrict__, const int* __restrict__, uint32_t);
 ER_PREPARE_INST(true)
 ER_PREPARE_INST(false)
 #undef ER_PREPARE_INST
diff --git a/elasticreconstruction_amd/tsdf.py b/elasticreconstruction_amd/tsdf.py
--- a/elasticreconstruction_amd/tsdf.py
+++ b/elasticreconstruction_amd/tsdf.py
@@ -145,6 +145,9 @@
         assert pad.value == pad_floats and nk.value <= cap
         return dict(scaled=scaled, pad=pad.value, tile_max=tmax[:, :, :n].copy(), tile_lo=tlo[:, :, :n].copy(),
                     tile_lo_fine=fine[:, :, :n].copy(), keys=keys[:nk.value].copy(), masks=masks[:nk.value].copy())
+
+    def set_zbuf_epoch(self, which, epoch):
+        _ffi.check(self._lib.er_tsdf_set_zbuf_epoch(self._h, int(which), int(epoch)), "er_tsdf_set_zbuf_epoch")
 
     def unit_count(self):
         n = C.c_int(0)
diff --git a/include/er_hip.h b/include/er_hip.h
--- a/include/er_hip.h
+++ b/include/er_hip.h
@@ -55,6 +55,8 @@
 int er_tsdf_prepass_trace(er_tsdf_t h, int n, const uint16_t* depth, int depth_on_device, const double* T, const er_warp* warp,
                           float* scaled, int* scaled_pad, float* tile_max, float* tile_lo, float* tile_lo_fine,
                           int* keys, unsigned long long* masks, int keys_cap, int* n_keys);
+
+int er_tsdf_set_zbuf_epoch(er_tsdf_t h, int which, unsigned epoch);
 
 int er_tsdf_wait_event(er_tsdf_t h, void* hip_event);
 
```
